# tpy001/VFMSeg

Measured on AMD Instinct MI355X. Metric: train images/sec @512x512 DINOv2-L+LoRA (dg_lora_dinov2_ms_masked, 1024^2 sample = LR+HR 512^2 passes), higher is better.
Workload: dtype bf16; 1 GPU; configs[1]: dg_lora_dinov2_ms_masked.py, synthetic 1024^2 19-class samples -> 2x512^2 passes, bs=2/GPU, full train step (fwd+bwd+allreduce+AdamW), LoRA dropout on; global_batch=2, parallelism=dp1

## Files before the change

include/vfmseg_hip.h:

```cpp
#ifndef VFMSEG_HIP_H
#define VFMSEG_HIP_H
#include <stdint.h>

#ifdef __cplusplus
extern "C" {
#endif

enum { VFM_F32 = 0, VFM_BF16 = 1, VFM_U8 = 2, VFM_I64 = 3,
       VFM_SPLIT3 = 4  };
enum { VFM_OK = 0, VFM_E_INVAL = -1, VFM_E_SHAPE = -2, VFM_E_ALIGN = -3, VFM_E_HIP = -4, VFM_E_UNSUPPORTED = -5 };
enum { VFM_EP_NONE = 0, VFM_EP_GELU = 1, VFM_EP_RELU = 2, VFM_EP_MUL_GELU_GRAD = 3, VFM_EP_MUL = 4,
       VFM_EP_QGELU = 5 , VFM_EP_MUL_QGELU_GRAD = 6,
       VFM_EP_GELU_DGELU = 7  };
enum { VFM_ACT_NONE = 0, VFM_ACT_GELU = 1, VFM_ACT_RELU = 2, VFM_ACT_QGELU = 3 };

const char* vfm_last_error(void);
int vfm_abi_version(void);
int vfm_half_kind(void);

int vfm_cast(const void* src, int src_dt, long ld_src, void* dst, int dst_dt, long ld_dst, long rows, long cols,
             const float* colscale, void* stream);
int vfm_split3(const float* src, long stride_r, long stride_c, void* dst, long ld_dst, long rows, long K, int pattern, void* stream);
int vfm_transpose(const void* src, int src_dt, long ld_src, void* dst, int dst_dt, long ld_dst, long rows, long cols,
                  long pad_rows, void* stream);
int vfm_strided_copy(const void* src, int src_dt, void* dst, int dst_dt, long n0, long n1, long n2, long n3, long s0,
                     long s1, long s2, long s3, long d0, long d1, long d2, long d3, int accumulate, void* stream);
typedef struct vfm_copy_job {
  const float* src; void* dst; long dst_dt; long accumulate;
  long n[4], s[4], d[4];
  long nsum, sum_stride;
} vfm_copy_job;
int vfm_strided_copy_batch(const vfm_copy_job* table_dev, int njobs, long max_elems, void* stream);
int vfm_axpby(const float* x, float a, float* y, float b, long n, void* stream);
int vfm_scale_by_device_scalar(float* y, const float* scalar, long n, void* stream);
int vfm_colsum(const void* x, int dt, long ld, long rows, long cols, float* out, int accumulate, float* ws, void* stream);
typedef struct vfm_lora_site {
  const float* A; const float* B;
  void* a; void* at; void* w; void* wt;
  long r, K, N, Kw, ld_a, ld_at, ld_w, ld_wt;
} vfm_lora_site;
int vfm_lora_pack(const vfm_lora_site* table_dev, int nsites, long max_elems, int dt, void* stream);
int vfm_slab_reduce(const float* slabs, int kch, long P, long Q, long rows_used, float alpha, float* dst, long sp, long sq,
                    int accumulate, void* stream);
int vfm_dropout_mask(void* out, int dt, long n, float p, uint64_t seed, uint64_t offset, void* stream);
int vfm_mul_mask(const void* src, int src_dt, long ld_src, const void* mask, int mask_dt, long mask_ld,
                 long rows_per_group, void* dst, int dst_dt, long ld_dst, long rows, long cols, void* stream);
int vfm_geglu_fwd(const void* h, int h_dt, long ld_h, void* out, int out_dt, long ld_out, long rows, long C, void* stream);
int vfm_geglu_bwd(const void* h, int h_dt, long ld_h, const void* dout, int do_dt, long ld_do, void* dh, int dh_dt,
                  long ld_dh, long rows, long C, void* stream);
int vfm_swiglu_fwd(const void* h, int h_dt, long ld_h, void* out, int out_dt, long ld_out, long rows, long C, void* stream);
int vfm_swiglu_bwd(const void* h, int h_dt, long ld_h, const void* dout, int do_dt, long ld_do, void* dh, int dh_dt,
                   long ld_dh, long rows, long C, void* stream);
int vfm_rope(void* x, int dt, long ld, long rows, int np, int ncols, int d, const float* cos_t, const float* sin_t,
             int inverse, void* stream);
int vfm_act_grad_mul(const void* dy, int dy_dt, long ld_dy, const void* pre, int pre_dt, long ld_pre, void* out, int out_dt,
                     long ld_out, long rows, long cols, int act, void* stream);
int vfm_mask_token_fwd(const float* x, const uint8_t* keep, const float* token, float* out, long rows, long C, void* stream);
int vfm_mask_token_bwd(const float* dout, const uint8_t* keep, float* dx, float* dtoken, float* ws ,
                       long rows, long C, void* stream);

int vfm_layernorm_fwd(const float* x, long ld_x, const float* w, const float* b, float eps, void* y, int y_dt, long ld_y,
                      float* stats, long rows, long C, void* stream);
int vfm_layernorm_fwd_split3(const float* x, long ld_x, const float* w, const float* b, float eps, float* y, long ld_y, void* y3, long ld3,
                             long plane, float* stats, long rows, long C, void* stream);
int vfm_layernorm_dropout_fwd(const float* x, long ld_x, const float* w, const float* b, float eps, void* y, long ld_y,
                              float* stats, void* y_drop, long ld_yd, void* mask, long ld_mask, float p, uint64_t seed,
                              uint64_t offset, long rows, long C, void* stream);
int vfm_layernorm_bwd_scaled(const void* dy, int dy_dt, long ld_dy, const float* x, long ld_x, const float* w,
                             const float* stats, float* dx, long ld_dx, int accumulate_dx, void* t_out, long ld_t,
                             const float* t_scale, long rows, long C, void* stream);
int vfm_layernorm_bwd(const void* dy, int dy_dt, long ld_dy, const float* x, long ld_x, const float* w,
                      const float* stats, float* dx, long ld_dx, int accumulate_dx, float* dw, float* db, float* ws,
                      long rows, long C, void* stream);
int vfm_groupnorm_fwd(const float* x, const float* w, const float* b, float eps, int G, int act, void* y, int y_dt,
                      float* stats, float* ws, long B, long P, long C, void* stream);
int vfm_groupnorm_bwd(const void* dy, int dy_dt, const float* x, const float* w, const float* b, const float* stats,
                      int G, int act, float* dx, float* dw, float* db, float* ws, long B, long P, long C, void* stream);
int vfm_groupnorm_tile_ok(long P, long C, int G);
int vfm_groupnorm_tile_fwd(const float* x, const float* w, const float* b, float eps, int G, int act, void* y, int y_dt,
                           float* stats, long B, long P, long C, void* stream);
int vfm_groupnorm_tile_bwd(const void* dy, int dy_dt, const float* x, const float* w, const float* b, const float* stats,
                           int G, int act, float* dx, float* dw, float* db, float* ws, long B, long P, long C, void* stream);
int vfm_bn_moments(const float* x, long rows, long C, float* sums, float* ws, void* stream);
int vfm_bn_finalize(const float* sums, float count, float* mean_var, float* running_mean, float* running_var,
                    float momentum, long C, void* stream);
int vfm_bn_apply(const float* x, const float* mean_var, const float* w, const float* b, float eps, int act, void* y,
                 int y_dt, long rows, long C, void* stream);
int vfm_bn_bwd_reduce(const void* dy, int dy_dt, const float* x, const float* mean_var, const float* w, const float* b,
                      float eps, int act, float* sums_dy, float* ws, long rows, long C, void* stream);
int vfm_bn_bwd_apply(const void* dy, int dy_dt, const float* x, const float* mean_var, const float* w, const float* b,
                     float eps, int act, const float* sums_dy, float total_rows, float* dx, long rows, long C,
                     void* stream);

typedef struct vfm_gemm_desc {
  const void* A; const void* B; void* C;
  int in_dt; int c_dt;
  long M, N, K;
  long sa_m, sa_k, sb_n, sb_k, ldc;
  float alpha;
  const float* bias; long bias_mod;
  const float* colscale;
  const void* residual; int r_dt; long ldr;
  int ep_mode; const void* aux; int aux_dt; long ld_aux;
  void* C2; int c2_dt; long ldc2;
  long batch, stride_a, stride_b, stride_c;
  long c_plane;
  long kb_rows;
} vfm_gemm_desc;
int vfm_gemm(const vfm_gemm_desc* d, void* stream);
int vfm_tune(const char* key, int value);

typedef struct vfm_attn_desc {
  const void* q; const void* k; const void* v; void* o;
  int dt; long ldq, ldk, ldv, ldo;
  int B, H, d;
  int nq_main, nq_extra, nk_main, nk_extra;
  float scale;
  float* lse;
  const void* dout; long ld_do;
  void* dq; void* dk; void* dv; long ld_dq, ld_dk, ld_dv;
  float* delta;
} vfm_attn_desc;
int vfm_attn_fwd(const vfm_attn_desc* d, void* stream);
int vfm_attn_bwd(const vfm_attn_desc* d, void* stream);
int vfm_attn_fwd_x3(const vfm_attn_desc* d, long lo_off, void* stream);
int vfm_attn_fwd_x3_split(const vfm_attn_desc* d, long lo_off, void* o3, long ld3, long plane, void* stream);
int vfm_attn_bwd_x3(const vfm_attn_desc* d, const void* q3, const void* k3, const void* v3, long ld3, long lo_off, const void* do3,
                    long ld_do3, long lo_off_do3, void* stream);

int vfm_sam_relpos_table(const float* rel_pos, int L, int d, int S, float* out, void* stream);
int vfm_sam_attn_prep(const void* qkv, int dt, long ld, const float* bias, const float* rh, const float* rw, void* q_aug,
                      void* k_aug, void* v_win, int nimg, int G, int S, int H, int d, int Dq, int NP,
                      int rows_per_batch , float scale, void* stream);
int vfm_softmax_rows(const float* scores, long ld_s, void* out, int out_dt, long ld_o, long rows, int n, int npad, void* stream);
int vfm_sam_attn_merge(const void* o_win, int dt, void* out, long ld, int nimg, int G, int S, int H, int d, int NP, void* stream);
int vfm_sam_attn_bwd_prep(const void* dao, long ld_dao, const void* qkv, long ld_qkv, const float* bias, int dt, void* dow,
                          void* dowT, void* vp, void* qsT, int nimg, int G, int S, int H, int d, int dp, int NP, float scale,
                          void* stream);
int vfm_softmax_rows_batched(const float* scores, long ld_s, void* out, int out_dt, long ld_o, long rows, int n, int npad,
                             int rows_per_batch, int valid_rows, void* stream);
int vfm_softmax_rows_bwd(const void* p, const float* dp, long ld_dp, void* ds, int dt, long ld_p, long rows, int n, int npad,
                         int rows_per_batch, int valid_rows, void* stream);
int vfm_sam_attn_bwd_merge(const void* dqa, const void* dkT, const void* dvT, int dt, const float* rh, const float* rw, void* dqkv,
                           long ld, int nimg, int G, int S, int H, int d, int dp, int NP, int Dq, float scale, void* stream);

int vfm_rein_mix_fwd(const float* x, long ld_x, const void* t, const void* vt, void* u, long ld_u, void* p, long ld_p, void* x16,
                     long ld_x16, long rows, int D, int m, float c, void* stream);
int vfm_rein_mix_bwd(const void* du, long ld_du, const void* p, long ld_p, const void* v, const void* tt, void* ds, long ld_ds,
                     float* dx, long ld_dx, long rows, int D, int m, float c, void* stream);

int vfm_sam_attn_flash_fwd(const void* qkv, long ld, const float* bias, const void* tbl_h, const void* tbl_w, void* out, long ldo,
                           int nimg, int G, int S, int H, int d, float scale, void* stream);
int vfm_sam_attn_flash_fwd_train(const void* qkv, long ld, const float* bias, const void* tbl_h, const void* tbl_w, void* out, long ldo,
                                 int nimg, int G, int S, int H, int d, float scale, float* lse, void* qext, void* stream);
long vfm_sam_attn_flash_stat_rows(int nimg, int G, int S, int H);
int vfm_sam_attn_flash_bwd(const void* qkv, long ld, const float* bias, const void* tbl_h, const void* tbl_w, const void* out,
                           const void* dout, long ldo, const float* lse, const void* qext, float* dsum, void* dqkv, long ldg,
                           int nimg, int G, int S, int H, int d, float scale, void* stream);

int vfm_patchify(const float* img, long stride_b, long stride_c, long stride_y, int y0, int x0, int h, int w, int P,
                 void* out, int out_dt, long ld_out, int B, void* stream);
int vfm_assemble_tokens(const float* patch_tok, const float* cls, const float* pos, float* x, int B, int np, int C,
                        void* stream);

int vfm_resize_bilinear(const void* in, int in_dt, int in_nchw, int B, int Hi, int Wi, int C, long in_ld_c, void* out,
                        int out_dt, int out_mode, long out_ld_c, int Hv, int Wv, int y0, int x0, int hc, int wc,
                        float scale_y, float scale_x, void* stream);
int vfm_resize_bicubic(const float* in, int Hi, int Wi, int C, float* out, int Ho, int Wo, double scale_y, double scale_x,
                       void* stream);
int vfm_label_resize(const int64_t* in, int B, int Hi, int Wi, int64_t* out, int Hv, int Wv, int y0, int x0, int hc,
                     int wc, void* stream);
int vfm_unblock(const float* x, float* y, int B, int H, int W, int C, int levels, int inverse, void* stream);
int vfm_upsample_ce(const float* logits_low, const int64_t* label, int B, int h, int w, int C, int H, int W,
                    int ignore_index, float* loss_parts, int32_t* counts, float* dlogits, void* stream);
int vfm_upsample_ce_w(const float* logits_low, const int64_t* label, const float* weight, int B, int h, int w, int C, int H, int W,
                      int ignore_index, float* loss_parts, int32_t* counts, float* dlogits, void* stream);
int vfm_pseudo_label(const float* logits_low, int B, int h, int w, int C, int H, int W, float thr, int64_t* pseudo_label,
                     float* pseudo_prob, int32_t* count, void* stream);
int vfm_class_presence(const int64_t* label, int B, long n, uint32_t* bits, void* stream);
int vfm_class_mix(const float* src_img, const float* tgt_img, const int64_t* src_label, const int64_t* pseudo_label,
                  const uint32_t* chosen, const int32_t* count, long total, int ignore_top, int ignore_bottom, int B, int H, int W,
                  float* mixed_img, int64_t* mixed_label, float* mix_weight, uint8_t* mask, void* stream);
#define VFM_OHEM_STATE_INTS 3080
#define VFM_OHEM_N 0
#define VFM_OHEM_NLT 1
#define VFM_OHEM_K 2
#define VFM_OHEM_T 6
#define VFM_LABEL_COUNT_INTS 33
int vfm_ohem_prob(const float* logits_low, const int64_t* label, int B, int h, int w, int C, int H, int W, int ignore_index,
                  float thresh, float* p, int32_t* state, void* stream);
int vfm_ohem_threshold(const float* p, long n_pix, long k_request, float thresh, int32_t* state, void* stream);
int vfm_label_weight(const int64_t* label, const float* p, const int32_t* state, const float* class_weight, const float* pix_weight,
                     int C, long n_pix, int ignore_index, int avg_non_ignore, float* weight, int32_t* counts, float* norm, void* stream);
int vfm_ce_finish(const float* loss_parts, long n, float scale, int32_t* counts, float eps, float* loss, float* acc, void* stream);
int vfm_hrda_fuse_fwd(const float* lr, const float* a, const float* hr, int B, int h, int w, int C, int ha, int wa, int hc, int wc,
                      int Y0, int X0, int my0, int my1, int mx0, int mx1, float* fused, float* att_out, float* lr_scaled_out,
                      void* stream);
int vfm_hrda_fuse_bwd(const float* d_fused, const float* lr, const float* a, const float* hr, const float* att, int B, int h, int w,
                      int C, int ha, int wa, int hc, int wc, int Y0, int X0, int my0, int my1, int mx0, int mx1, float* d_lr,
                      float* d_a, float* d_hr, float* d_att_ws, void* stream);
int vfm_reduce_sum(const float* x, long n, float scale, float* out, void* stream);

int vfm_preprocess_u8(const uint8_t* img, int H, int W, float* out, int Hp, int Wp, const float* mean3, const float* std3,
                      int bgr_to_rgb, float pad_val, void* stream);
typedef struct vfm_augment_plan {
  int resize_h, resize_w;
  int crop_y, crop_x, crop_h, crop_w;
  int flip;
  int wide;
  int brightness_on, contrast_on;
  int saturation_on, hue_on, hue_delta;
  double brightness_beta, contrast_alpha, saturation_alpha;
} vfm_augment_plan;
int vfm_augment_u8(const uint8_t* img, int Hs, int Ws, const vfm_augment_plan* plan, float* out, int Hp, int Wp, const float* mean3,
                   const float* std3, int bgr_to_rgb, float pad_val, void* stream);
int vfm_conf_gate(const float* logits, int B, int C, int H, int W, int y0, int x0, int hc, int wc, float thr,
                  int32_t* count, void* stream);
int vfm_slide_accumulate(const float* crop, int crop_nchw, int B, int h, int w, int C, float* preds, float* count,
                         int H, int W, int y0, int x0, int hc, int wc, void* stream);
typedef struct vfm_slide_win {
  const float* crop;
  int nchw, h, w;
  int y0, x0, hc, wc;
} vfm_slide_win;
int vfm_slide_gather(const vfm_slide_win* wins, int nwin, int B, int C, float* preds, int H, int W, void* stream);
int vfm_conf_gate_windows(const float* logits, int B, int C, int H, int W, const int* boxes, int nwin, float thr, int32_t* counts,
                          void* stream);
int vfm_slide_finalize(float* preds, const float* count, uint8_t* argmax, int B, int C, int H, int W, void* stream);

int vfm_confusion_hist(const uint8_t* pred, const void* label, int label_dt, long n, int num_classes, int ignore_index,
                       int64_t* hist, void* stream);
int vfm_postprocess_argmax(const float* logits, int C, long plane_stride, long row_stride, int Hm, int Wm, int y0, int x0,
                           int h, int w, int flip, uint8_t* pred, int oh, int ow, const void* label, int label_dt,
                           int num_classes, int ignore_index, int64_t* hist, void* stream);

int vfm_adamw(float* p, float* g, float* m, float* v, long n, const long* seg_start, const float* seg_lr_mult,
              const float* seg_wd, int n_seg, float lr, float beta1, float beta2, float eps, int step, float grad_scale,
              int zero_grad, int vec4, void* stream);
int vfm_adamw_guarded(float* p, float* g, float* m, float* v, long n, const long* seg_start, const float* seg_lr_mult,
                      const float* seg_wd, int n_seg, float lr, float beta1, float beta2, float eps, int step, float grad_scale,
                      int zero_grad, int vec4, const int* skip, const float* amp_state, void* stream);
int vfm_amp_update(const int* flag, float* amp_state, float growth, float backoff, int interval, int dynamic, void* stream);

enum { VFM_OP_GEMM = 0, VFM_OP_LN_FWD = 1, VFM_OP_LN_DROPOUT_FWD = 2, VFM_OP_LN_BWD_SCALED = 3, VFM_OP_ATTN_FWD = 4, VFM_OP_ATTN_BWD = 5,
       VFM_OP_CAST = 6, VFM_OP_STRIDED_COPY = 7 };
enum { VFM_PROF_NONE = 0, VFM_PROF_GEMM = 1, VFM_PROF_GEMM_TN = 2, VFM_PROF_ATTN_FWD = 3, VFM_PROF_ATTN_BWD = 4 };
typedef struct vfm_plan_op {
  int kind;
  int prof_kind;
  double flops;
  union {
    vfm_gemm_desc gemm;
    vfm_attn_desc attn;
    struct { const float* x; long ld_x; const float* w; const float* b; float eps; void* y; int y_dt; long ld_y; float* stats;
             long rows, C; } ln_fwd;
    struct { const float* x; long ld_x; const float* w; const float* b; float eps; void* y; long ld_y; float* stats; void* y_drop;
             long ld_yd; void* mask; long ld_mask; float p; uint64_t offset; long rows, C; } ln_drop;
    struct { const void* dy; int dy_dt; long ld_dy; const float* x; long ld_x; const float* w; const float* stats; float* dx;
             long ld_dx; int accumulate_dx; void* t_out; long ld_t; const float* t_scale; long rows, C; } ln_bwd;
    struct { const void* src; int src_dt; long ld_src; void* dst; int dst_dt; long ld_dst; long rows, cols; const float* colscale; } cast;
    struct { const void* src; int src_dt; void* dst; int dst_dt; long n[4]; long ss[4]; long ds[4]; int accumulate; } copy;
  } u;
} vfm_plan_op;
int vfm_run_plan(const vfm_plan_op* ops, int n, uint64_t seed, uint64_t rng_base, void* stream);
int vfm_prof_config(int every);
int vfm_prof_read(double* out, int cap);

#ifdef __cplusplus
}
#endif
#endif
```

vfmseg_amd/backbones.py:

```python
import math

import os

import torch
import torch.nn as nn

from .precision import is_half
from . import ops
from .precision import compute_dtype
from .registry import MODELS

R_PAD = 64

BACKWARD_EVENTS = {"heads_done": None, "block_done": None, "backbone_done": None}
_PENDING_BACKWARD = [0]


class _Lin(nn.Module):
    def __init__(self, i, o, bias=True):
        super().__init__()
        self.in_features, self.out_features = i, o
        self.weight = nn.Parameter(torch.empty(o, i))
        self.bias = nn.Parameter(torch.zeros(o)) if bias else None
        nn.init.trunc_normal_(self.weight, std=0.02)
# ... 169 lines not shown
        if ck is not None:
            if init_cfg.get("type", "Pretrained") != "Pretrained":
                raise NotImplementedError(f"init_cfg type {init_cfg.get('type')!r}: only dict(type='Pretrained', checkpoint=...) is read")
            self.load_pretrained_base(ck)

    def load_pretrained_base(self, checkpoint):
        sd = torch.load(checkpoint, map_location="cpu") if isinstance(checkpoint, (str, os.PathLike)) else checkpoint
        sd = sd.get("state_dict", sd) if isinstance(sd, dict) else sd
        missing, _ = self.load_state_dict(sd, strict=False)
        missing = [k for k in missing if not k.startswith("reins.")]
        if missing:
            raise RuntimeError(f"pretrained backbone {checkpoint if isinstance(checkpoint, (str, os.PathLike)) else '<state dict>'}: "
                               f"{len(missing)} base parameters not found (first: {missing[:3]}; the file holds e.g. {list(sd)[:3]})")
        self.pretrained = checkpoint if isinstance(checkpoint, (str, os.PathLike)) else "<state dict>"
        self.engine().invalidate()

    def train(self, mode=True):
        nn.Module.train(self, False)
        self._rein_train = bool(mode)
        if mode:
            for n, p in self.named_parameters():
                p.requires_grad = "reins" in n
            for p in self.reins.inert_params():
                p.requires_grad = False
            self.reins.train(True)
        return self

    def adapter_training(self):
        return self._rein_train

    def state_dict(self, *args, destination=None, prefix="", keep_vars=False):
        if args:
            args = list(args) + [None] * (3 - len(args))
            destination, prefix, keep_vars = args[0], args[1] or "", bool(args[2])
        state = super().state_dict(destination=destination, prefix=prefix, keep_vars=keep_vars)
        for k in [k for k in state.keys() if k.startswith(prefix) and "rein" not in k[len(prefix):]]:
            state.pop(k)
        return state

    def forward(self, x):
        xcat, (hp, wp) = self.forward_tokens([(x, None)], training=self._rein_train)
        b, d = x.shape[0], self.embed_dim
        v = xcat.view(b, hp, wp, len(self.out_indices), d)
        return tuple(v[:, :, :, i].permute(0, 3, 1, 2) for i in range(len(self.out_indices)))


class _Holder(nn.Module):
    def __init__(self, m):
        super().__init__()
        self.model = m


class _PeftModel(nn.Module):
    def __init__(self, m):
        super().__init__()
        self.base_model = _Holder(m)


@MODELS.register_module()
class LoRABackbone(nn.Module):

    def __init__(self, backbone, checkpoint=None, Lora_config=None, init_cfg=None, **kw):
        super().__init__()
        vit = MODELS.build(backbone)
        cfg = Lora_config or {}
        self.lora_targets = list(cfg.get("target_modules", ["qkv"]))
        for name, mod in list(vit.named_modules()):
            if isinstance(mod, _Lin) and any(name == t or name.endswith("." + t) for t in self.lora_targets):
                parent = vit
                parts = name.split(".")
                for p_ in parts[:-1]:
                    parent = getattr(parent, p_)
                setattr(parent, parts[-1], LoraLinear(mod, cfg.get("r", 32), cfg.get("lora_alpha", 32), cfg.get("lora_dropout", 0.0)))
        if not vit.engine().lora_on():
            raise NotImplementedError(f"target_modules={self.lora_targets}: no adapter site the {type(vit).__name__} HIP engine fuses")
        self.model = _PeftModel(vit)
        self._lora_train = False
        if checkpoint is not None:
            self.load_pretrained_backbone(checkpoint, self.lora_targets)
        self.train(True)

    @property
    def vit(self):
        return self.model.base_model.model

    def load_pretrained_backbone(self, checkpoint, target_modules):
        sd = torch.load(checkpoint, map_location="cpu") if isinstance(checkpoint, str) else checkpoint
        new = {}
        for name, w in sd.items():
            for t in target_modules:
                if t in name:
                    name = name.replace(t, t + ".base_layer")
            new[name] = w
        self.vit.load_state_dict(new, strict=False)
        self.vit.engine().invalidate()

    def train(self, mode=True):
        super().train(False)
        self._lora_train = bool(mode)
        for n, p in self.named_parameters():
            p.requires_grad = ("lora" in n) if mode else p.requires_grad
        if mode:
            for p in getattr(self.vit.engine(), "inert_params", lambda: [])():
                p.requires_grad = False
        return self

    def forward_tokens(self, jobs, seed=None):
        return self.vit.forward_tokens(jobs, training=self._lora_train, seed=seed)

    def forward(self, x):
        xcat, (hp, wp) = self.forward_tokens([(x, None)])
        b, d, nt = x.shape[0], self.vit.embed_dim, len(self.vit.out_indices)
        v = xcat.view(b, hp, wp, nt, d)
        return tuple(v[:, :, :, i].permute(0, 3, 1, 2) for i in range(nt))


class Packed:

    def __init__(self, w_f32, cd, k_pad=None):
        n, k = w_f32.shape
        k_pad = k_pad or k
        self.n, self.k = n, k_pad
        self.w = ops.empty_ld(n, k_pad, cd, w_f32.device, zero=True)
        ops.cast(w_f32, self.w[:, :k])
        self.wt = None
        if is_half(cd):
            self.wt = ops.empty_ld(k_pad, n, cd, w_f32.device, zero=True)
            ops.transpose(w_f32, self.wt[:k], pad_rows=n)

    def fwd(self, a, out, **epi):
        return ops.gemm(a, self.w, out, **epi)

    def dgrad(self, dy, out, **epi):
        if self.wt is not None:
            return ops.gemm(dy, self.wt, out, **epi)
        return ops.gemm(dy, self.w, out, trans_b=True, **epi)


def wgrad(dy, x, grad_out, alpha=1.0, n_rows=None, accumulate=True):
    M = dy.shape[0]
    res = grad_out if accumulate else None
    if is_half(dy.dtype):
        mp = (M + 63) // 64 * 64
        dyt = torch.empty(dy.shape[1], mp, dtype=dy.dtype, device=dy.device)
        xt = torch.empty(x.shape[1], mp, dtype=x.dtype, device=x.device)
        ops.transpose(dy, dyt, pad_rows=mp)
        ops.transpose(x, xt, pad_rows=mp)
        ops.gemm(dyt, xt, grad_out, alpha=alpha, residual=res)
    else:
        ops.gemm(dy, x, grad_out, alpha=alpha, residual=res, trans_a=True, trans_b=True)
    return grad_out


class _DinoTrainPlan:

    def __init__(self, eng, P, nimg, Np):
        v = eng.vit
        cd, dev = P["cd"], P["dev"]
        D, H = v.embed_dim, v.num_heads
        nL = len(v.blocks)
        M, Mp = nimg * Np + nimg, nimg * Np
        Lp0 = P["layers"][0]
        kq, hid = Lp0["qkv"].k, Lp0["fc1"].n
        q0 = v.blocks[0].attn.qkv
        self.eng, self.P, self.nimg, self.Np, self.M, self.Mp, self.nL, self.D, self.H = eng, P, nimg, Np, M, Mp, nL, D, H
        self.busy = False
        e = lambda *sh, dt=cd: torch.empty(*sh, dtype=dt, device=dev)
        f32 = torch.float32
        self.X = e(nL + 1, M, D, dt=f32)
        self.A1, self.XD, self.MASK = e(nL, M, kq), e(nL, M, D), e(nL, M, D)
        self.ST1, self.ST2 = e(nL, M, 2, dt=f32), e(nL, M, 2, dt=f32)
        self.QKV, self.AO = e(nL, M, 3 * D), e(nL, M, D)
        self.LSE = e(nL, nimg, H, Np + 1, dt=f32)
        self.XMID, self.A2 = e(nL, M, D, dt=f32), e(nL, M, D)
        hld = hid + ops.ld_pad(hid, cd)
        self.HPRE = e(nL, M, hld)[:, :, :hid]
        self.G = e(M, hld)[:, :hid]
        self.hid, self.kq = hid, kq
        hd = D // H
        scale = hd ** -0.5
        f = self.fwd = ops.Plan("backbone")
        self.tap_ops = []
        self.nt = len(v.out_indices)
        xcat0 = e(Mp, self.nt * D)
        for li, (blk, Lp) in enumerate(zip(v.blocks, P["layers"])):
            q = blk.attn.qkv
            x, a1 = self.X[li], self.A1[li]
            f.layernorm_dropout_fwd(x, Lp["n1w"], Lp["n1b"], 1e-6, a1[:, :D], self.ST1[li], self.XD[li], self.MASK[li], q.p, li * M * D)
            f.gemm(self.XD[li], Lp["a"], a1[:, D:D + R_PAD], alpha=q.scaling)
            f.gemm(a1, Lp["qkv"].w, self.QKV[li], bias=Lp["qkv_b"])
            qkv = self.QKV[li]
            f.attn_fwd(qkv[:, :D], qkv[:, D:2 * D], qkv[:, 2 * D:], self.AO[li], self.LSE[li], nimg, H, hd, Np, 1, Np, 1, scale)
            f.gemm(self.AO[li], Lp["proj"].w, self.XMID[li], bias=Lp["proj_b"], colscale=Lp["g1"], residual=x)
            f.layernorm_fwd(self.XMID[li], Lp["n2w"], Lp["n2b"], 1e-6, self.A2[li], self.ST2[li])
            f.gemm(self.A2[li], Lp["fc1"].w, self.G, bias=Lp["fc1_b"], ep_mode=ops.EP_GELU_DGELU, c2=self.HPRE[li])
            f.gemm(self.G, Lp["fc2"].w, self.X[li + 1], bias=Lp["fc2_b"], colscale=Lp["g2"], residual=self.XMID[li])
            for i, oi in enumerate(v.out_indices):
                if oi == li:
                    self.tap_ops.append((f.cast(self.X[li + 1][:Mp], xcat0[:, i * D:(i + 1) * D]), i * D))
        self.bwd = None

    def eligible_backward(self):
        from .functional import direct_grad_target
        v = self.eng.vit
        return (os.environ.get("VFMSEG_LORA_WGRAD_BATCHED", "1") != "0" and
                all(direct_grad_target(b.attn.qkv.lora_A["default"].weight) is not None and
                    direct_grad_target(b.attn.qkv.lora_B["default"].weight) is not None for b in v.blocks))

    def run_forward(self, xcat, seed, rng0):
        esz = xcat.element_size()
        for idx, col in self.tap_ops:
            self.fwd.entry(idx).u.cast.dst = xcat.data_ptr() + col * esz
        self.fwd.run(seed, rng0)

    def _build_backward(self, dxcat):
        v, P = self.eng.vit, self.P
        cd, dev = P["cd"], P["dev"]
        D, H, nL, M, Mp, nimg, Np = self.D, self.H, self.nL, self.M, self.Mp, self.nimg, self.Np
        hd = D // H
        scale = hd ** -0.5
        e = lambda *sh, dt=cd: torch.empty(*sh, dtype=dt, device=dev)
        self.DX = e(M, D, dt=torch.float32)
        self.T, self.DN, self.DAO = e(M, D), e(M, D), e(M, D)
        self.DH = e(M, self.hid + ops.ld_pad(self.hid, cd))[:, :self.hid]
        self.DQKV, self.DA1 = e(nL, M, 3 * D), e(nL, M, self.kq)
        half = nL // 2
        skip_l0 = os.environ.get("VFMSEG_PLAN_SKIP_L0", "1") != "0"
        self.half = half
        self.dx_sig = (tuple(dxcat.shape), tuple(dxcat.stride()), dxcat.dtype)
        plans, self.tap_src = [], []

        def add_tap(pl, pn, li):
            for i, oi in enumerate(v.out_indices):
                if oi == li:
                    src = dxcat[:, i * D:(i + 1) * D]
                    self.tap_src.append((pn, pl.strided_copy(src, self.DX, (Mp, D), (src.stride(0), 1), (D, 1), accumulate=True), i * D))

        for pn, (hi, lo) in enumerate(((nL, half), (half, 0)) if half > 0 else ((nL, 0),)):
            pl = ops.Plan("backbone")
            for li in range(hi - 1, lo - 1, -1):
                blk, Lp = v.blocks[li], P["layers"][li]
                q = blk.attn.qkv
                if li == nL - 1:
                    add_tap(pl, pn, li)
                    pl.cast(self.DX, self.T, Lp["g2"])
                pl.gemm(self.T, Lp["fc2"].wt, self.DH, ep_mode=ops.EP_MUL, aux=self.HPRE[li])
                pl.gemm(self.DH, Lp["fc1"].wt, self.DN)
                pl.layernorm_bwd_scaled(self.DN, self.XMID[li], Lp["n2w"], self.ST2[li], self.DX, self.T, Lp["g1"], accumulate_dx=True)
                pl.gemm(self.T, Lp["proj"].wt, self.DAO)
                qkv, dqkv, da1 = self.QKV[li], self.DQKV[li], self.DA1[li]
                pl.attn_bwd(qkv[:, :D], qkv[:, D:2 * D], qkv[:, 2 * D:], self.AO[li], self.LSE[li], self.DAO, dqkv[:, :D], dqkv[:, D:2 * D],
                            dqkv[:, 2 * D:], nimg, H, hd, Np, 1, Np, 1, scale)
                if li == 0 and skip_l0:
                    pl.gemm(dqkv, Lp["qkv"].wt[D:D + R_PAD], da1[:, D:D + R_PAD])
                    continue
                pl.gemm(dqkv, Lp["qkv"].wt, da1)
                pl.gemm(da1[:, D:D + R_PAD], Lp["at"], da1[:, :D], alpha=q.scaling, residual=da1[:, :D], ep_mode=ops.EP_MUL, aux=self.MASK[li])
                if li > 0:
                    add_tap(pl, pn, li - 1)
                    pl.layernorm_bwd_scaled(da1[:, :D], self.X[li], Lp["n1w"], self.ST1[li], self.DX, self.T, P["layers"][li - 1]["g2"],
                                            accumulate_dx=True)
                else:
                    pl.layernorm_bwd_scaled(da1[:, :D], self.X[li], Lp["n1w"], self.ST1[li], self.DX, self.T, Lp["g2"], accumulate_dx=True)
            plans.append((pl, lo, hi))
        self.bwd = plans

    def run_backward(self, ctx, dxcat):
        sig = (tuple(dxcat.shape), tuple(dxcat.stride()), dxcat.dtype)
        if self.bwd is None or self.dx_sig != sig:
            self._build_backward(dxcat)
        esz = dxcat.element_size()
        for pn, idx, col in self.tap_src:
            self.bwd[pn][0].entry(idx).u.copy.src = dxcat.data_ptr() + col * esz
        self.DX.zero_()
        for pl, lo, hi in self.bwd:
            pl.run()
            self.eng._lora_wgrads_batched(self.P, ctx, self.DA1, self.DQKV, lo, hi, self.M, self.D)
            if BACKWARD_EVENTS["block_done"] is not None:
                for lj in range(hi - 1, lo - 1, -1):
                    BACKWARD_EVENTS["block_done"](lj)


class DinoEngine:
    def __init__(self, vit):
        self.vit = vit
        self._packed = None
        self._pos_cache = {}

    def invalidate(self):
        self._packed = None
        self._pos_cache = {}

    def lora_on(self):
        return isinstance(self.vit.blocks[0].attn.qkv, LoraLinear)

    def rein_on(self):
        return getattr(self.vit, "reins", None) is not None

    def trainable(self):
        out = []
        if self.lora_on():
            for blk in self.vit.blocks:
                out += [blk.attn.qkv.lora_A["default"].weight, blk.attn.qkv.lora_B["default"].weight]
        if self.rein_on():
            out += self.vit.reins.live_params()
        return out

    def packed(self):
        cd = compute_dtype()
        dev = self.vit.pos_embed.device
        if self._packed is not None and self._packed["cd"] == cd and self._packed["dev"] == dev:
            return self._packed
        v = self.vit
        D = v.embed_dim
        P = dict(cd=cd, dev=dev, layers=[])
        with torch.no_grad():
            pw = v.patch_embed.proj.weight.detach().reshape(D, -1)
            P["pe"] = Packed(pw, cd)
            P["pe_b"] = v.patch_embed.proj.bias.detach().float().contiguous()
            P["cls"] = v.cls_token.detach().reshape(D).float().contiguous()
            for blk in v.blocks:
                qkv = blk.attn.qkv
                base = qkv.base_layer if isinstance(qkv, LoraLinear) else qkv
                kq = D + (R_PAD if isinstance(qkv, LoraLinear) else 0)
                Lp = dict(
                    qkv=Packed(base.weight.detach(), cd, k_pad=kq),
                    qkv_b=base.bias.detach().float().contiguous() if base.bias is not None else None,
                    proj=Packed(blk.attn.proj.weight.detach(), cd),
                    proj_b=blk.attn.proj.bias.detach().float().contiguous() if blk.attn.proj.bias is not None else None,
                    fc1=Packed(blk.mlp.fc1.weight.detach(), cd),
                    fc1_b=blk.mlp.fc1.bias.detach().float().contiguous() if blk.mlp.fc1.bias is not None else None,
                    fc2=Packed(blk.mlp.fc2.weight.detach(), cd),
                    fc2_b=blk.mlp.fc2.bias.detach().float().contiguous() if blk.mlp.fc2.bias is not None else None,
                    g1=blk.ls1.gamma.detach().float().contiguous(), g2=blk.ls2.gamma.detach().float().contiguous(),
                    n1w=blk.norm1.weight.detach().float().contiguous(), n1b=blk.norm1.bias.detach().float().contiguous(),
                    n2w=blk.norm2.weight.detach().float().contiguous(), n2b=blk.norm2.bias.detach().float().contiguous(),
                )
                if isinstance(qkv, LoraLinear):
                    Lp["a"] = torch.zeros(R_PAD, D, dtype=cd, device=dev)
                    Lp["at"] = torch.zeros(D, R_PAD, dtype=cd, device=dev)
                P["layers"].append(Lp)
        self._packed = P
        return P

    def refresh_lora(self, P):
        D = self.vit.embed_dim
        sites = []
        for blk, Lp in zip(self.vit.blocks, P["layers"]):
            q = blk.attn.qkv
            if isinstance(q, LoraLinear):
                A, Bm = q.lora_A["default"].weight.detach(), q.lora_B["default"].weight.detach()
                sites.append((A, Bm, Lp["a"], Lp["at"], Lp["qkv"].w, Lp["qkv"].wt, q.r, A.shape[1], Bm.shape[0], D))
        _refresh_sites(P, sites)

    def merged_qkv(self, P):
        from .optim import PARAM_EPOCH
        key = [PARAM_EPOCH[0]]
        for blk in self.vit.blocks:
            q = blk.attn.qkv
            A, Bm = q.lora_A["default"].weight, q.lora_B["default"].weight
            key += [A._version, Bm._version, A.data_ptr(), Bm.data_ptr()]
        key = tuple(key)
        if P.get("merged_key") == key:
            return P["merged"]
        D, cd, dev = self.vit.embed_dim, P["cd"], P["dev"]
        merged = []
        with torch.no_grad():
            for blk in self.vit.blocks:
                q = blk.attn.qkv
                A, Bm = q.lora_A["default"].weight.detach().float(), q.lora_B["default"].weight.detach().float()
                w = q.base_layer.weight.detach().float()
                weff = torch.empty_like(w)
                ops.gemm(Bm.contiguous(), A.contiguous(), weff, alpha=q.scaling, residual=w, trans_b=True)
                wp = ops.empty_ld(w.shape[0], D, cd, dev)
                ops.cast(weff, wp)
                merged.append(wp)
        P["merged"], P["merged_key"] = merged, key
        return merged

    def pos_tokens(self, hp, wp):
        v = self.vit
        n = v.pos_embed.shape[1] - 1
        s = int(math.sqrt(n))
        if hp == s and wp == s:
            return v.pos_embed.detach().reshape(n + 1, -1).float().contiguous()
        key = (hp, wp)
        if key not in self._pos_cache:
            D = v.embed_dim
            pe = v.pos_embed.detach().reshape(n + 1, D).float().contiguous()
            out = torch.empty(1 + hp * wp, D, dtype=torch.float32, device=pe.device)
            ops.cast(pe[:1], out[:1])
            sy, sx = s / (hp + 0.1), s / (wp + 0.1)
            assert int(s * ((hp + 0.1) / s)) == hp and int(s * ((wp + 0.1) / s)) == wp
            ops.resize_bicubic(pe[1:], s, s, D, out[1:], hp, wp, sy, sx)
            self._pos_cache[key] = out
        return self._pos_cache[key]

    def forward(self, jobs, training, seed, need_grad=False):
        v, P = self.vit, self.packed()
        cd = P["cd"]
        dev = P["dev"]
        D, H, ps = v.embed_dim, v.num_heads, v.patch_size
        lora = self.lora_on()
        rein = self._rein_pack(P) if self.rein_on() else None
        merged = None
        from .precision import split3 as _x3_mode
        x3 = _x3_mode() and not is_half(cd)
        if (lora and not training and not torch.is_grad_enabled() and (is_half(cd) or x3)
                and os.environ.get("VFMSEG_MERGE_LORA_EVAL", "1") != "0"):
            merged = self.merged_qkv(P)
        elif lora:
            self.refresh_lora(P)
        sizes = []
        for img, box in jobs:
            y0, y1, x0, x1 = box if box is not None else (0, img.shape[2], 0, img.shape[3])
            sizes.append(((y1 - y0) // ps, (x1 - x0) // ps))
        hp, wp = sizes[0]
        assert all(s == (hp, wp) for s in sizes), "all jobs of one backbone call must share the token grid"
        Np = hp * wp
        nimg = sum(j[0].shape[0] for j in jobs)
        Mp, M = nimg * Np, nimg * Np + nimg
        kpe = 3 * ps * ps
        A0 = torch.empty(Mp, kpe, dtype=cd, device=dev)
        r0 = 0
        for img, box in jobs:
            b = img.shape[0]
            ops.patchify(img, A0[r0 * Np:(r0 + b) * Np], box=box, patch=ps)
            r0 += b
        ptok = torch.empty(Mp, D, dtype=torch.float32, device=dev)
        P["pe"].fwd(A0, ptok, bias=P["pe_b"])
        plan = self._train_plan(P, nimg, Np, training, merged) if need_grad else None
        x = plan.X[0] if plan is not None else torch.empty(M, D, dtype=torch.float32, device=dev)
        ops.assemble_tokens(ptok, P["cls"], self.pos_tokens(hp, wp), x, nimg, Np, D)
        del ptok, A0
        nt = len(v.out_indices)
        from .precision import eval_heads_fp32
        tap_dt = torch.float32 if (not training and not need_grad and eval_heads_fp32()) else cd
        xcat = torch.empty(Mp, nt * D, dtype=tap_dt, device=dev)
        saved = []
        if lora and training:
            from .functional import draw_seed
            seed, rng0 = draw_seed(seed, len(v.blocks) * M * D)
        else:
            seed, rng0 = 0, 0
        if plan is not None:
            plan.run_forward(xcat, seed, rng0)
            plan.busy = True
            ctx = dict(saved=None, plan=plan, nimg=nimg, Np=Np, M=M, Mp=Mp, P=P, training=training, A1all=plan.A1, XDall=plan.XD)
            return xcat, (hp, wp), ctx
        nL = len(v.blocks)
        batched = lora and training and is_half(cd) and merged is None
        A1all = torch.empty(nL, M, P["layers"][0]["qkv"].k, dtype=cd, device=dev) if batched else None
        XDall = None
        hd = D // H
        scale = hd ** -0.5
        for li, (blk, Lp) in enumerate(zip(v.blocks, P["layers"])):
            S = {"x_in": x}
            kq = D if merged is not None else Lp["qkv"].k
            a1 = A1all[li] if batched else torch.empty(M, kq, dtype=cd, device=dev)
            st1 = torch.empty(M, 2, dtype=torch.float32, device=dev)
            q = blk.attn.qkv if lora else None
            fused_drop = lora and training and q.p > 0 and is_half(cd) and D % 256 == 0
            if fused_drop:
                mask = torch.empty(M, D, dtype=cd, device=dev)
                if batched and XDall is None:
                    XDall = torch.empty(nL, M, D, dtype=cd, device=dev)
                xd = XDall[li] if batched else torch.empty(M, D, dtype=cd, device=dev)
                ops.layernorm_dropout_fwd(x, Lp["n1w"], Lp["n1b"], 1e-6, a1[:, :D], st1, xd, mask, q.p, seed, offset=rng0 + li * M * D)
            else:
                so = "only" if (x3 and not training and not need_grad and kq == D) else None
                ops.layernorm_fwd(x, Lp["n1w"], Lp["n1b"], 1e-6, a1 if kq == D else a1[:, :D], st1, split_out=so)
            if lora and merged is None:
                if not fused_drop:
                    xd, mask = a1[:, :D], None
                    if training and q.p > 0:
                        mask = torch.empty(M, D, dtype=cd, device=dev)
                        ops.dropout_mask(mask, q.p, seed, offset=rng0 + li * M * D)
                        xd = torch.empty(M, D, dtype=cd, device=dev)
                        ops.mul_mask(a1[:, :D], mask, xd)
                ops.gemm(xd, Lp["a"], a1[:, D:D + R_PAD], alpha=q.scaling)
                S.update(xd=xd if mask is not None else None, mask=mask)
            qkv = torch.empty(M, 3 * D, dtype=cd, device=dev)
            if merged is not None:
                ops.gemm(a1, merged[li], qkv, bias=Lp["qkv_b"])
            else:
                Lp["qkv"].fwd(a1, qkv, bias=Lp["qkv_b"])
            ao = torch.empty(M, D, dtype=cd, device=dev)
            lse = torch.empty(nimg, H, Np + 1, dtype=torch.float32, device=dev)
            so = "only" if (x3 and not training and not need_grad) else None
            ops.attn_fwd(qkv[:, :D], qkv[:, D:2 * D], qkv[:, 2 * D:], ao, lse, nimg, H, hd, Np, 1, Np, 1, scale, keep_split=training, o_split=so)
            xm = torch.empty(M, D, dtype=torch.float32, device=dev)
            Lp["proj"].fwd(ao, xm, bias=Lp["proj_b"], colscale=Lp["g1"], residual=x)
            a2 = torch.empty(M, D, dtype=cd, device=dev)
            st2 = torch.empty(M, 2, dtype=torch.float32, device=dev)
            ops.layernorm_fwd(xm, Lp["n2w"], Lp["n2b"], 1e-6, a2, st2, split_out=so)
            hid = Lp["fc1"].n
            g = ops.empty_ld(M, hid, cd, dev)
            if training and (lora or (rein is not None and need_grad)):
                hpre = torch.empty(M, hid, dtype=cd, device=dev)
                Lp["fc1"].fwd(a2, g, bias=Lp["fc1_b"], ep_mode=ops.EP_GELU_DGELU, c2=hpre)
            else:
                hpre = None
                Lp["fc1"].fwd(a2, g, bias=Lp["fc1_b"], ep_mode=ops.EP_GELU, **({"c_split": so} if so else {}))
            xo = torch.empty(M, D, dtype=torch.float32, device=dev)
            Lp["fc2"].fwd(g, xo, bias=Lp["fc2_b"], colscale=Lp["g2"], residual=xm)
            S.update(a1=a1, st1=st1, qkv=qkv, ao=ao, lse=lse, x_mid=xm, a2=a2, st2=st2, hpre=hpre, g=g)
            saved.append(S)
            x = xo
            if rein is not None:
                x = self._rein_forward(rein, li, x, Mp, S if (training and need_grad) else None)
            for i, oi in enumerate(v.out_indices):
                if oi == li:
                    ops.cast(x[:Mp], xcat[:, i * D:(i + 1) * D])
        ctx = dict(saved=saved, nimg=nimg, Np=Np, M=M, Mp=Mp, P=P, training=training, A1all=A1all, XDall=XDall, rein=rein)
        return xcat, (hp, wp), ctx

    def _train_plan(self, P, nimg, Np, training, merged):
        v = self.vit
        if (not training or merged is not None or not self.lora_on() or self.rein_on() or not is_half(P["cd"])
                or os.environ.get("VFMSEG_PLAN", "1") == "0" or v.embed_dim % 256 != 0):
            return None
        q0 = v.blocks[0].attn.qkv
        if not all(isinstance(b.attn.qkv, LoraLinear) and b.attn.qkv.p > 0 and b.attn.qkv.p == q0.p and b.attn.qkv.scaling == q0.scaling
                   for b in v.blocks):
            return None
        plans = P.setdefault("plans", {})
        pl = plans.get((nimg, Np))
        if pl is None:
            pl = plans[(nimg, Np)] = _DinoTrainPlan(self, P, nimg, Np)
        if pl.busy or not pl.eligible_backward():
            return None
        return pl

    def backward(self, ctx, dxcat):
        if ctx.get("plan") is not None:
            plan = ctx["plan"]
            try:
                plan.run_backward(ctx, dxcat)
            finally:
                plan.busy = False
            return [None] * (2 * len(self.vit.blocks))
        v, P = self.vit, ctx["P"]
        cd, dev = P["cd"], P["dev"]
        D, H = v.embed_dim, v.num_heads
        hd = D // H
        scale = hd ** -0.5
        M, Mp, nimg, Np = ctx["M"], ctx["Mp"], ctx["nimg"], ctx["Np"]
        dx = torch.zeros(M, D, dtype=torch.float32, device=dev)
        grads = [None] * (2 * len(v.blocks) if self.lora_on() else 0)
        nL = len(v.blocks)
        rein = ctx.get("rein")
        rein_acc = self._rein_backward_begin(rein) if rein is not None else None
        from .functional import direct_grad_target
        wg_batched = (ctx.get("A1all") is not None and self.lora_on() and os.environ.get("VFMSEG_LORA_WGRAD_BATCHED", "1") != "0" and
                      all(direct_grad_target(b.attn.qkv.lora_A["default"].weight) is not None and
                          direct_grad_target(b.attn.qkv.lora_B["default"].weight) is not None for b in v.blocks) and
                      (ctx.get("XDall") is not None or all(S_["mask"] is None for S_ in ctx["saved"])))
        if wg_batched:
            kq_all = ctx["A1all"].shape[2]
            DA1all = torch.empty(nL, M, kq_all, dtype=cd, device=dev)
            DQKVall = torch.empty(nL, M, 3 * D, dtype=cd, device=dev)
        half = nL // 2
        fuse_t = is_half(cd) and D % 256 == 0
        fuse_t1 = fuse_t and rein is None
        def add_tap(li):
            for i, oi in enumerate(v.out_indices):
                if oi == li:
                    src = dxcat[:, i * D:(i + 1) * D]
                    ops.strided_copy(src, dx, (Mp, D), (src.stride(0), 1), (D, 1), accumulate=True)
        t = None
        for li in range(len(v.blocks) - 1, -1, -1):
            blk, Lp, S = v.blocks[li], P["layers"][li], ctx["saved"][li]
            q = blk.attn.qkv
            if t is None:
                add_tap(li)
                if rein is not None:
                    self._rein_backward(rein, rein_acc, li, dx, Mp, S)
                t = torch.empty(M, D, dtype=cd, device=dev)
                ops.cast(dx, t, Lp["g2"])
            hid = Lp["fc1"].n
            dh = ops.empty_ld(M, hid, cd, dev)
            Lp["fc2"].dgrad(t, dh, ep_mode=ops.EP_MUL, aux=S["hpre"])
            dn = torch.empty(M, D, dtype=cd, device=dev)
            Lp["fc1"].dgrad(dh, dn)
            if fuse_t:
                ops.layernorm_bwd_scaled(dn, S["x_mid"], Lp["n2w"], S["st2"], dx, t, Lp["g1"], accumulate_dx=True)
            else:
                ops.layernorm_bwd(dn, S["x_mid"], Lp["n2w"], S["st2"], dx, accumulate_dx=True)
                ops.cast(dx, t, Lp["g1"])
            del dh
            dao = torch.empty(M, D, dtype=cd, device=dev)
            Lp["proj"].dgrad(t, dao)
            dqkv = DQKVall[li] if wg_batched else torch.empty(M, 3 * D, dtype=cd, device=dev)
            qkv = S["qkv"]
            ops.attn_bwd(qkv[:, :D], qkv[:, D:2 * D], qkv[:, 2 * D:], S["ao"], S["lse"], dao, dqkv[:, :D], dqkv[:, D:2 * D],
                         dqkv[:, 2 * D:], nimg, H, hd, Np, 1, Np, 1, scale)
            kq = Lp["qkv"].k
            da1 = DA1all[li] if wg_batched else torch.empty(M, kq, dtype=cd, device=dev)
            Lp["qkv"].dgrad(dqkv, da1)
            if isinstance(q, LoraLinear) and wg_batched:
                ep = dict(ep_mode=ops.EP_MUL, aux=S["mask"]) if S["mask"] is not None else {}
                ops.gemm(da1[:, D:D + R_PAD], Lp["at"], da1[:, :D], alpha=q.scaling, residual=da1[:, :D], **ep)
            elif isinstance(q, LoraLinear):
                r = q.r
                A, Bm = q.lora_A["default"].weight, q.lora_B["default"].weight
                a1 = S["a1"]
                xd = S["xd"] if S["xd"] is not None else a1[:, :D]
                from .functional import direct_grad_target
                tB, tA = direct_grad_target(Bm), direct_grad_target(A)
                gBt = torch.empty(R_PAD, Bm.shape[0], dtype=torch.float32, device=dev)
                gAp = torch.empty(R_PAD, A.shape[1], dtype=torch.float32, device=dev)
                doneB = _wgrad_small_t(a1[:, D:D + R_PAD], dqkv, gBt, scatter=None if tB is None else (tB, r, 1, r))
                doneA = _wgrad_small_t(da1[:, D:D + R_PAD], xd, gAp, alpha=q.scaling,
                                       scatter=None if tA is None else (tA, r, A.shape[1], 1))
                if doneB is True:
                    pass
                elif tB is not None:
                    ops.strided_copy(gBt, tB, (Bm.shape[0], r), (1, gBt.stride(0)), (r, 1), accumulate=True)
                else:
                    gB = torch.empty_like(Bm, dtype=torch.float32)
                    ops.strided_copy(gBt, gB, (Bm.shape[0], r), (1, gBt.stride(0)), (r, 1))
                    grads[2 * li + 1] = gB
                if doneA is True:
                    pass
                elif tA is not None:
                    ops.axpby(gAp[:r].reshape(-1), 1.0, tA.view(-1), 1.0)
                else:
                    grads[2 * li] = gAp[:r]
                ep = dict(ep_mode=ops.EP_MUL, aux=S["mask"]) if S["mask"] is not None else {}
                ops.gemm(da1[:, D:D + R_PAD], Lp["at"], da1[:, :D], alpha=q.scaling, residual=da1[:, :D], **ep)
            if fuse_t1 and li > 0:
                add_tap(li - 1)
                ops.layernorm_bwd_scaled(da1[:, :D], S["x_in"], Lp["n1w"], S["st1"], dx, t, P["layers"][li - 1]["g2"],
                                         accumulate_dx=True)
            else:
                ops.layernorm_bwd(da1[:, :D], S["x_in"], Lp["n1w"], S["st1"], dx, accumulate_dx=True)
                t = None
            ctx["saved"][li] = None
            if wg_batched:
                if li == half or li == 0:
                    lo, hi = (half, nL) if li == half and half > 0 else (0, half if half > 0 else nL)
                    self._lora_wgrads_batched(P, ctx, DA1all, DQKVall, lo, hi, M, D)
                    if BACKWARD_EVENTS["block_done"] is not None:
                        for lj in range(hi - 1, lo - 1, -1):
                            BACKWARD_EVENTS["block_done"](lj)
            elif BACKWARD_EVENTS["block_done"] is not None:
                BACKWARD_EVENTS["block_done"](li)
        if rein is not None:
            grads += self._rein_backward_end(rein, rein_acc)
        return grads

    def _rein_fused(self, P):
        r = self.vit.reins
        return (is_half(P["cd"]) and os.environ.get("VFMSEG_REIN_FUSED", "0") == "1" and self.vit.embed_dim % 256 == 0
                and r.token_length <= ops.REIN_TOK)

    def _rein_pack(self, P):
        from .optim import PARAM_EPOCH
        r = self.vit.reins
        cd, dev = P["cd"], P["dev"]
        D, nL, m = self.vit.embed_dim, r.num_layers, r.token_length
        live = r.live_params()
        key = (PARAM_EPOCH[0], self._rein_fused(P)) + tuple(x for p_ in live for x in (p_._version, p_.data_ptr()))
        R = P.get("rein")
        if R is not None and R["key"] == key:
            return R
        TP = (max(m, ops.REIN_TOK) + 63) // 64 * 64
        if R is None or R["TP"] != TP:
            z = lambda *sh, dt=cd: torch.zeros(*sh, dtype=dt, device=dev)
            R = P["rein"] = dict(TP=TP, T32=z(nL, TP, D, dt=torch.float32), T=z(nL, TP, D), V=z(nL, TP, D), TT=None, VT=None,
                                 scalevec=torch.empty(D, dtype=torch.float32, device=dev))
        R["key"], R["m"], R["c"], R["fused"] = key, m, float(D) ** -0.5, self._rein_fused(P)
        with torch.no_grad():
            T32 = R["T32"]
            toks = [p_.detach() for p_ in r.token_params()]
            if len(toks) == 2:
                ops.gemm(toks[0], toks[1], T32[:, :m], trans_b=True)
            else:
                ops.strided_copy(toks[0], T32, (nL, m, D), (m * D, D, 1), (TP * D, D, 1))
            if cd != torch.float32:
                ops.cast(T32.view(nL * TP, D), R["T"].view(nL * TP, D))
            else:
                R["T"] = T32
            Wt, Wd = r.mlp_token2feat, r.mlp_delta_f
            R["wt"], R["wd"] = Packed(Wt.weight.detach(), cd), Packed(Wd.weight.detach(), cd)
            R["bt"], R["bd"] = Wt.bias.detach(), Wd.bias.detach()
            vtmp = torch.empty(nL * TP, D, dtype=torch.float32, device=dev)
            R["wt"].fwd(R["T"].view(nL * TP, D), vtmp, bias=R["bt"])
            vt3 = vtmp.view(nL, TP, D)
            ops.strided_copy(vt3[:, 1:m], R["V"][:, 1:m], (nL, m - 1, D), (TP * D, D, 1), (TP * D, D, 1))
            if R["fused"]:
                if R["TT"] is None:
                    R["TT"], R["VT"] = torch.zeros(nL, D, TP, dtype=cd, device=dev), torch.zeros(nL, D, TP, dtype=cd, device=dev)
                ops.strided_copy(T32, R["TT"], (nL, D, m), (TP * D, 1, D), (D * TP, TP, 1))
                ops.strided_copy(vt3[:, 1:m], R["VT"][:, :, 1:m], (nL, D, m - 1), (TP * D, 1, D), (D * TP, TP, 1))
            ops.strided_copy(r.scale.detach().reshape(1), R["scalevec"], (D,), (0,), (1,))
        return R

    def _rein_forward(self, R, li, x, Mp, S):
        cd, dev = R["T"].dtype, x.device
        D, m, TP = x.shape[1], R["m"], R["TP"]
        xp = x[:Mp]
        u = torch.empty(Mp, D, dtype=cd, device=dev)
        p = torch.empty(Mp, TP, dtype=cd, device=dev) if S is not None else None
        x16 = None
        if R["fused"]:
            x16 = torch.empty(Mp, D, dtype=cd, device=dev) if S is not None else None
            ops.rein_mix_fwd(xp, R["T"][li], R["VT"][li], u, m, R["c"], p=p, x16=x16)
        else:
            if cd != torch.float32:
                x16 = torch.empty(Mp, D, dtype=cd, device=dev)
                ops.cast(xp, x16)
            sc = torch.empty(Mp, TP, dtype=torch.float32, device=dev)
            ops.gemm(x16 if x16 is not None else xp, R["T"][li], sc, alpha=R["c"])
            if p is None:
                p = torch.empty(Mp, TP, dtype=cd, device=dev)
            ops.softmax_rows(sc, p, m)
            ops.gemm(p, R["V"][li], u, residual=xp, trans_b=True)
        if S is None:
            xn = x
        else:
            xn = torch.empty_like(x)
            ops.cast(x[Mp:], xn[Mp:])
            S.update(rein_u=u, rein_p=p, rein_x=x16 if x16 is not None else xp)
        R["wd"].fwd(u, xn[:Mp], bias=R["bd"], colscale=R["scalevec"], residual=xp)
        return xn

    def _rein_backward_begin(self, R):
        dev = R["T"].device
        nL, TP, D = R["T"].shape
        z = lambda *sh: torch.zeros(*sh, dtype=torch.float32, device=dev)
        return dict(dT=z(nL, TP, D), dV=z(nL, TP, D), Gm=z(D, D), gb=z(D))

    @staticmethod
    def _tn(xs, y, out, alpha=1.0, accumulate=False):
        if is_half(xs.dtype):
            ops.gemm_tn_batched(xs.unsqueeze(0), y.unsqueeze(0), out.unsqueeze(0), xs.shape[0], alpha=alpha, accumulate=accumulate)
        else:
            ops.gemm(xs, y, out, alpha=alpha, residual=out if accumulate else None, trans_a=True, trans_b=True)

    def _rein_backward(self, R, acc, li, dx, Mp, S):
        cd, dev = R["T"].dtype, dx.device
        D, m, TP, c = dx.shape[1], R["m"], R["TP"], R["c"]
        u, p, xs = S["rein_u"], S["rein_p"], S["rein_x"]
        g = torch.empty(Mp, D, dtype=cd, device=dev)
        ops.cast(dx[:Mp], g)
        self._tn(g, u, acc["Gm"], accumulate=True)
        ops.colsum(g, acc["gb"], accumulate=True)
        du = torch.empty(Mp, D, dtype=cd, device=dev)
        R["wd"].dgrad(g, du, colscale=R["scalevec"])
        ds = torch.empty(Mp, TP, dtype=cd, device=dev)
        if R["fused"]:
            ops.rein_mix_bwd(du, p, R["V"][li], R["TT"][li], ds, dx[:Mp], m, c)
            a = 1.0
        else:
            dp = torch.empty(Mp, TP, dtype=torch.float32, device=dev)
            ops.gemm(du, R["V"][li], dp)
            ops.softmax_rows_bwd(p, dp, ds, m, 1, 1)
            ops.gemm(ds, R["T"][li], dx[:Mp], alpha=c, residual=dx[:Mp], trans_b=True)
            ops.strided_copy(du, dx[:Mp], (Mp, D), (du.stride(0), 1), (dx.stride(0), 1), accumulate=True)
            a = c
        self._tn(ds, xs, acc["dT"][li], alpha=a)
        self._tn(p, du, acc["dV"][li])
        S["rein_u"] = S["rein_p"] = S["rein_x"] = None

    def _rein_backward_end(self, R, acc):
        from .functional import direct_grad_target
        r = self.vit.reins
        cd, dev = R["T"].dtype, R["T"].device
        nL, TP, D = R["T"].shape
        m = R["m"]
        z = lambda *sh, dt=torch.float32: torch.zeros(*sh, dtype=dt, device=dev)
        dvz = z(nL, TP, D, dt=cd)
        ops.strided_copy(acc["dV"][:, 1:m], dvz[:, 1:m], (nL, m - 1, D), (TP * D, D, 1), (TP * D, D, 1))
        dvz2, T2 = dvz.view(nL * TP, D), R["T"].view(nL * TP, D)
        gWt, gbt = z(D, D), z(D)
        self._tn(dvz2, T2, gWt)
        ops.colsum(dvz2, gbt)
        back = torch.empty(nL * TP, D, dtype=torch.float32, device=dev)
        R["wt"].dgrad(dvz2, back)
        dT = acc["dT"]
        ops.strided_copy(back.view(nL, TP, D)[:, 1:m], dT[:, 1:m], (nL, m - 1, D), (TP * D, D, 1), (TP * D, D, 1), accumulate=True)
        toks = r.token_params()
# ... 169 lines not shown
```

vfmseg_amd/csrc/elementwise.hip:

```cpp
#include "common.h"

thread_local char g_vfm_err[512] = {0};

extern "C" const char* vfm_last_error(void) { return g_vfm_err; }
extern "C" int vfm_abi_version(void) { return 9; }
extern "C" int vfm_half_kind(void) { return VFM_HALF_KIND; }

template <typename TI, typename TO>
__global__ void k_cast(const TI* __restrict__ src, long ld_src, TO* __restrict__ dst, long ld_dst, long rows, long cols,
                       const float* __restrict__ colscale) {
  const long cols4 = cols >> 2;
  const long total = rows * cols4;
  for (long i = blockIdx.x * (long)blockDim.x + threadIdx.x; i < total; i += (long)gridDim.x * blockDim.x) {
    const long r = i / cols4, c = (i - r * cols4) << 2;
    float v[4];
#pragma unroll
    for (int j = 0; j < 4; ++j) v[j] = ld_f32(src + r * ld_src + c + j);
    if (colscale) {
#pragma unroll
      for (int j = 0; j < 4; ++j) v[j] *= colscale[c + j];
    }
#pragma unroll
    for (int j = 0; j < 4; ++j) st_f32(dst + r * ld_dst + c + j, v[j]);
  }
  const long tail0 = cols4 << 2;
  const long ntail = cols - tail0;
  if (ntail) {
    for (long i = blockIdx.x * (long)blockDim.x + threadIdx.x; i < rows * ntail; i += (long)gridDim.x * blockDim.x) {
      const long r = i / ntail, c = tail0 + (i - r * ntail);
      float v = ld_f32(src + r * ld_src + c);
      if (colscale) v *= colscale[c];
      st_f32(dst + r * ld_dst + c, v);
    }
  }
}

extern "C" int vfm_cast(const void* src, int src_dt, long ld_src, void* dst, int dst_dt, long ld_dst, long rows, long cols,
                        const float* colscale, void* stream) {
  VFM_CHECK(rows >= 0 && cols >= 0 && ld_src >= cols && ld_dst >= cols, VFM_E_SHAPE, "vfm_cast: bad shape");
  if (rows == 0 || cols == 0) return VFM_OK;
  hipStream_t s = (hipStream_t)stream;
  const long total = rows * ((cols + 3) / 4);
  const int grid = (int)((total + 255) / 256 > 4096 ? 4096 : (total + 255) / 256);
#define L(TI, TO) hipLaunchKernelGGL((k_cast<TI, TO>), dim3(grid), dim3(256), 0, s, (const TI*)src, ld_src, (TO*)dst, ld_dst, rows, cols, colscale)
  if (src_dt == VFM_F32 && dst_dt == VFM_F32) L(float, float);
  else if (src_dt == VFM_F32 && dst_dt == VFM_BF16) L(float, bf16_t);
  else if (src_dt == VFM_BF16 && dst_dt == VFM_F32) L(bf16_t, float);
  else if (src_dt == VFM_BF16 && dst_dt == VFM_BF16) L(bf16_t, bf16_t);
  else VFM_FAIL(VFM_E_INVAL, "vfm_cast: dtype");
#undef L
  VFM_LAUNCH_CHECK();
  return VFM_OK;
}

__global__ void k_split3(const float* __restrict__ src, long sr, long sc, bf16_t* __restrict__ dst, long ld_dst, long rows, long K, long Kp,
                         int pattern) {
  const long per_row = Kp / 4;
  const long total = rows * per_row;
  for (long i = (long)blockIdx.x * blockDim.x + threadIdx.x; i < total; i += (long)gridDim.x * blockDim.x) {
    const long r = i / per_row, c = (i % per_row) * 4;
    float v[4];
    if (sc == 1 && c + 3 < K && ((reinterpret_cast<uintptr_t>(src + r * sr + c) & 15) == 0)) {
      const float4 f = *reinterpret_cast<const float4*>(src + r * sr + c);
      v[0] = f.x, v[1] = f.y, v[2] = f.z, v[3] = f.w;
    } else {
#pragma unroll
      for (int e = 0; e < 4; ++e) v[e] = (c + e < K) ? src[r * sr + (c + e) * sc] : 0.f;
    }
    ushort4 hi, lo;
    bf16_t* ph = &hi.x;
    bf16_t* pl = &lo.x;
#pragma unroll
    for (int e = 0; e < 4; ++e) {
      ph[e] = f32_to_bf16(v[e]);
      pl[e] = f32_to_bf16(v[e] - bf16_to_f32(ph[e]));
    }
    bf16_t* d = dst + r * ld_dst + c;
    *reinterpret_cast<ushort4*>(d) = hi;
    *reinterpret_cast<ushort4*>(d + Kp) = pattern == 0 ? hi : lo;
    *reinterpret_cast<ushort4*>(d + 2 * Kp) = pattern == 0 ? lo : hi;
  }
}

extern "C" int vfm_split3(const float* src, long stride_r, long stride_c, void* dst, long ld_dst, long rows, long K, int pattern, void* stream) {
  const long Kp = (K + 63) / 64 * 64;
  VFM_CHECK(rows >= 0 && K > 0 && ld_dst >= 3 * Kp && ld_dst % 4 == 0 && ((uintptr_t)dst % 8) == 0 && (pattern == 0 || pattern == 1), VFM_E_SHAPE,
            "vfm_split3: dst must hold rows x 3 ceil64(K) bf16 (ld %% 4 == 0, 8-byte aligned)");
  if (rows == 0) return VFM_OK;
  const long total = rows * (Kp / 4);
  const int grid = (int)((total + 255) / 256 > 8192 ? 8192 : (total + 255) / 256);
  hipLaunchKernelGGL(k_split3, dim3(grid), dim3(256), 0, (hipStream_t)stream, src, stride_r, stride_c, (bf16_t*)dst, ld_dst, rows, K, Kp, pattern);
  VFM_LAUNCH_CHECK();
  return VFM_OK;
}

template <typename TI, typename TO>
__global__ void k_transpose(const TI* __restrict__ src, long ld_src, TO* __restrict__ dst, long ld_dst, long rows, long cols,
                            long pad_rows) {
  __shared__ float tile[64][65];
  const long r0 = (long)blockIdx.y * 64, c0 = (long)blockIdx.x * 64;
  const int tx = threadIdx.x & 63, ty = threadIdx.x >> 6;
  for (int i = ty; i < 64; i += 4) {
    const long r = r0 + i, c = c0 + tx;
    tile[i][tx] = (r < rows && c < cols) ? ld_f32(src + r * ld_src + c) : 0.f;
  }
  __syncthreads();
  for (int i = ty; i < 64; i += 4) {
    const long c = c0 + i, r = r0 + tx;
    if (c < cols && r < pad_rows) st_f32(dst + c * ld_dst + r, tile[tx][i]);
  }
}

extern "C" int vfm_transpose(const void* src, int src_dt, long ld_src, void* dst, int dst_dt, long ld_dst, long rows, long cols,
                             long pad_rows, void* stream) {
  VFM_CHECK(pad_rows >= rows && ld_dst >= pad_rows && ld_src >= cols, VFM_E_SHAPE, "vfm_transpose: bad shape");
  if (cols == 0 || pad_rows == 0) return VFM_OK;
  hipStream_t s = (hipStream_t)stream;
  dim3 grid(cdiv(cols, 64), cdiv(pad_rows, 64));
#define L(TI, TO) hipLaunchKernelGGL((k_transpose<TI, TO>), grid, dim3(256), 0, s, (const TI*)src, ld_src, (TO*)dst, ld_dst, rows, cols, pad_rows)
  if (src_dt == VFM_F32 && dst_dt == VFM_F32) L(float, float);
  else if (src_dt == VFM_F32 && dst_dt == VFM_BF16) L(float, bf16_t);
  else if (src_dt == VFM_BF16 && dst_dt == VFM_F32) L(bf16_t, float);
  else if (src_dt == VFM_BF16 && dst_dt == VFM_BF16) L(bf16_t, bf16_t);
  else VFM_FAIL(VFM_E_INVAL, "vfm_transpose: dtype");
#undef L
  VFM_LAUNCH_CHECK();
  return VFM_OK;
}

template <typename TI, typename TO>
__global__ void k_strided_copy(const TI* __restrict__ src, TO* __restrict__ dst, long n0, long n1, long n2, long n3, long s0,
                               long s1, long s2, long s3, long d0, long d1, long d2, long d3, int accumulate) {
  const long total = n0 * n1 * n2 * n3;
  for (long i = blockIdx.x * (long)blockDim.x + threadIdx.x; i < total; i += (long)gridDim.x * blockDim.x) {
    long t = i;
    const long i3 = t % n3; t /= n3;
    const long i2 = t % n2; t /= n2;
    const long i1 = t % n1; t /= n1;
    const float v = ld_f32(src + t * s0 + i1 * s1 + i2 * s2 + i3 * s3);
    TO* q = dst + t * d0 + i1 * d1 + i2 * d2 + i3 * d3;
    st_f32(q, accumulate ? ld_f32(q) + v : v);
  }
}

extern "C" int vfm_strided_copy(const void* src, int src_dt, void* dst, int dst_dt, long n0, long n1, long n2, long n3,
                                long s0, long s1, long s2, long s3, long d0, long d1, long d2, long d3, int accumulate,
                                void* stream) {
  const long total = n0 * n1 * n2 * n3;
  if (total == 0) return VFM_OK;
  hipStream_t s = (hipStream_t)stream;
  const int grid = (int)((total + 255) / 256 > 4096 ? 4096 : (total + 255) / 256);
#define L(TI, TO) hipLaunchKernelGGL((k_strided_copy<TI, TO>), dim3(grid), dim3(256), 0, s, (const TI*)src, (TO*)dst, n0, n1, n2, n3, s0, s1, s2, s3, d0, d1, d2, d3, accumulate)
  if (src_dt == VFM_F32 && dst_dt == VFM_F32) L(float, float);
  else if (src_dt == VFM_F32 && dst_dt == VFM_BF16) L(float, bf16_t);
  else if (src_dt == VFM_BF16 && dst_dt == VFM_F32) L(bf16_t, float);
  else if (src_dt == VFM_BF16 && dst_dt == VFM_BF16) L(bf16_t, bf16_t);
  else VFM_FAIL(VFM_E_INVAL, "vfm_strided_copy: dtype");
#undef L
// ... 674 lines not shown
```

vfmseg_amd/csrc/norm.hip:

```cpp
#include "common.h"

__device__ __forceinline__ float act_f(float v, int act) {
  return act == VFM_ACT_GELU ? gelu_f(v) : (act == VFM_ACT_RELU ? fmaxf(v, 0.f) : v);
}
__device__ __forceinline__ float act_grad_f(float v, int act) {
  return act == VFM_ACT_GELU ? gelu_grad_f(v) : (act == VFM_ACT_RELU ? (v > 0.f ? 1.f : 0.f) : 1.f);
}

template <typename TO, int MAXPL>
__global__ void k_ln_fwd(const float* __restrict__ x, long ld_x, const float* __restrict__ w, const float* __restrict__ b,
                         float eps, TO* __restrict__ y, long ld_y, float* __restrict__ stats, long rows, int C) {
  const int lane = threadIdx.x & 63;
  const long row = (long)blockIdx.x * (blockDim.x >> 6) + (threadIdx.x >> 6);
  if (row >= rows) return;
  const float* xr = x + row * ld_x;
  float v[MAXPL];
  float s = 0.f;
#pragma unroll
  for (int i = 0; i < MAXPL; ++i) {
    const int c = i * 64 + lane;
    v[i] = c < C ? xr[c] : 0.f;
    s += v[i];
  }
  const float mean = wave_sum(s) / C;
  float q = 0.f;
#pragma unroll
  for (int i = 0; i < MAXPL; ++i) {
    const int c = i * 64 + lane;
    const float d = c < C ? v[i] - mean : 0.f;
    q += d * d;
  }
  const float rstd = rsqrtf(wave_sum(q) / C + eps);
  if (stats && lane == 0) {
    stats[row * 2] = mean;
    stats[row * 2 + 1] = rstd;
  }
#pragma unroll
  for (int i = 0; i < MAXPL; ++i) {
    const int c = i * 64 + lane;
    if (c < C) st_f32(y + row * ld_y + c, (v[i] - mean) * rstd * w[c] + b[c]);
  }
}


struct LnDrop {
  void* yd; long ld_yd; void* mask; long ld_mask; float p, keep_scale; uint64_t seed, offset;
};
struct Split3Out {
  bf16_t* y3; long ld3; long plane;
};
__device__ __forceinline__ void store_split4(const Split3Out& so, long row, int c0, float4 o) {
  const bf16_t h0 = f32_to_bf16(o.x), h1 = f32_to_bf16(o.y), h2 = f32_to_bf16(o.z), h3 = f32_to_bf16(o.w);
  const ushort4 hi = {h0, h1, h2, h3};
  const ushort4 lo = {f32_to_bf16(o.x - bf16_to_f32(h0)), f32_to_bf16(o.y - bf16_to_f32(h1)), f32_to_bf16(o.z - bf16_to_f32(h2)),
                      f32_to_bf16(o.w - bf16_to_f32(h3))};
  bf16_t* p = so.y3 + row * so.ld3 + c0;
  *reinterpret_cast<ushort4*>(p) = hi;
  *reinterpret_cast<ushort4*>(p + so.plane) = hi;
  *reinterpret_cast<ushort4*>(p + 2 * so.plane) = lo;
}
template <typename TO, int NV, bool DROP = false, bool SPLIT = false>
__global__ void k_ln_fwd_v4(const float* __restrict__ x, long ld_x, const float* __restrict__ w, const float* __restrict__ b,
                            float eps, TO* __restrict__ y, long ld_y, float* __restrict__ stats, long rows, int C, LnDrop dr = LnDrop(),
                            Split3Out so = Split3Out()) {
  const int lane = threadIdx.x & 63;
  const long row = (long)blockIdx.x * (blockDim.x >> 6) + (threadIdx.x >> 6);
  if (row >= rows) return;
  const float* xr = x + row * ld_x;
  float4 v[NV];
  float s = 0.f;
#pragma unroll
  for (int i = 0; i < NV; ++i) {
    v[i] = *reinterpret_cast<const float4*>(xr + (i * 64 + lane) * 4);
    s += (v[i].x + v[i].y) + (v[i].z + v[i].w);
  }
  const float mean = wave_sum(s) / C;
  float q = 0.f;
#pragma unroll
  for (int i = 0; i < NV; ++i) {
    const float a = v[i].x - mean, bb = v[i].y - mean, c = v[i].z - mean, d = v[i].w - mean;
    q += (a * a + bb * bb) + (c * c + d * d);
  }
  const float rstd = rsqrtf(wave_sum(q) / C + eps);
  if (stats && lane == 0) {
    stats[row * 2] = mean;
    stats[row * 2 + 1] = rstd;
  }
#pragma unroll
  for (int i = 0; i < NV; ++i) {
    const int c0 = (i * 64 + lane) * 4;
    const float4 ww = *reinterpret_cast<const float4*>(w + c0);
    const float4 bv = *reinterpret_cast<const float4*>(b + c0);
    float4 o;
    o.x = (v[i].x - mean) * rstd * ww.x + bv.x;
    o.y = (v[i].y - mean) * rstd * ww.y + bv.y;
    o.z = (v[i].z - mean) * rstd * ww.z + bv.z;
    o.w = (v[i].w - mean) * rstd * ww.w + bv.w;
    if constexpr (sizeof(TO) == 2) {
      ushort4 p = {f32_to_bf16(o.x), f32_to_bf16(o.y), f32_to_bf16(o.z), f32_to_bf16(o.w)};
      *reinterpret_cast<ushort4*>(y + row * ld_y + c0) = p;
      if constexpr (DROP) {
        const uint64_t e0 = dr.offset + (uint64_t)row * C + c0;
        const bf16_t ks = f32_to_bf16(dr.keep_scale);
        const float ksf = bf16_to_f32(ks);
        ushort4 mk, yd;
        const bool k0 = (hash_u32(dr.seed, e0) >> 8) * (1.0f / 16777216.0f) >= dr.p;
        const bool k1 = (hash_u32(dr.seed, e0 + 1) >> 8) * (1.0f / 16777216.0f) >= dr.p;
        const bool k2 = (hash_u32(dr.seed, e0 + 2) >> 8) * (1.0f / 16777216.0f) >= dr.p;
        const bool k3 = (hash_u32(dr.seed, e0 + 3) >> 8) * (1.0f / 16777216.0f) >= dr.p;
        mk.x = k0 ? ks : 0, mk.y = k1 ? ks : 0, mk.z = k2 ? ks : 0, mk.w = k3 ? ks : 0;
        yd.x = k0 ? f32_to_bf16(bf16_to_f32(p.x) * ksf) : f32_to_bf16(bf16_to_f32(p.x) * 0.f);
        yd.y = k1 ? f32_to_bf16(bf16_to_f32(p.y) * ksf) : f32_to_bf16(bf16_to_f32(p.y) * 0.f);
        yd.z = k2 ? f32_to_bf16(bf16_to_f32(p.z) * ksf) : f32_to_bf16(bf16_to_f32(p.z) * 0.f);
        yd.w = k3 ? f32_to_bf16(bf16_to_f32(p.w) * ksf) : f32_to_bf16(bf16_to_f32(p.w) * 0.f);
        *reinterpret_cast<ushort4*>((bf16_t*)dr.mask + row * dr.ld_mask + c0) = mk;
        *reinterpret_cast<ushort4*>((bf16_t*)dr.yd + row * dr.ld_yd + c0) = yd;
      }
    } else {
      if (!SPLIT || y != nullptr) *reinterpret_cast<float4*>(y + row * ld_y + c0) = o;
      if constexpr (SPLIT) store_split4(so, row, c0, o);
    }
  }
}

template <typename TD, int NV>
__global__ void k_ln_bwd_v4(const TD* __restrict__ dy, long ld_dy, const float* __restrict__ x, long ld_x,
                            const float* __restrict__ w, const float* __restrict__ stats, float* __restrict__ dx, long ld_dx,
                            int accumulate_dx, long rows, int C, bf16_t* __restrict__ t_out = nullptr, long ld_t = 0,
                            const float* __restrict__ t_scale = nullptr) {
  const int lane = threadIdx.x & 63;
  const long row = (long)blockIdx.x * (blockDim.x >> 6) + (threadIdx.x >> 6);
  if (row >= rows) return;
  const float mean = stats[row * 2], rstd = stats[row * 2 + 1];
  float4 g[NV], xh[NV];
  float s1 = 0.f, s2 = 0.f;
#pragma unroll
  for (int i = 0; i < NV; ++i) {
    const int c0 = (i * 64 + lane) * 4;
    float4 d;
    if constexpr (sizeof(TD) == 2) {
      const ushort4 p = *reinterpret_cast<const ushort4*>(dy + row * ld_dy + c0);
      d = make_float4(bf16_to_f32(p.x), bf16_to_f32(p.y), bf16_to_f32(p.z), bf16_to_f32(p.w));
    } else {
      d = *reinterpret_cast<const float4*>(dy + row * ld_dy + c0);
    }
    const float4 xv = *reinterpret_cast<const float4*>(x + row * ld_x + c0);
    const float4 ww = *reinterpret_cast<const float4*>(w + c0);
    xh[i] = make_float4((xv.x - mean) * rstd, (xv.y - mean) * rstd, (xv.z - mean) * rstd, (xv.w - mean) * rstd);
    g[i] = make_float4(d.x * ww.x, d.y * ww.y, d.z * ww.z, d.w * ww.w);
    s1 += (g[i].x + g[i].y) + (g[i].z + g[i].w);
    s2 += (g[i].x * xh[i].x + g[i].y * xh[i].y) + (g[i].z * xh[i].z + g[i].w * xh[i].w);
  }
  s1 = wave_sum(s1) / C;
  s2 = wave_sum(s2) / C;
#pragma unroll
  for (int i = 0; i < NV; ++i) {
    const int c0 = (i * 64 + lane) * 4;
    float4 o = make_float4(rstd * (g[i].x - s1 - xh[i].x * s2), rstd * (g[i].y - s1 - xh[i].y * s2),
                           rstd * (g[i].z - s1 - xh[i].z * s2), rstd * (g[i].w - s1 - xh[i].w * s2));
    float4* p = reinterpret_cast<float4*>(dx + row * ld_dx + c0);
    if (accumulate_dx) {
      const float4 old = *p;
      o.x += old.x, o.y += old.y, o.z += old.z, o.w += old.w;
    }
    *p = o;
    if (t_out) {
      const float4 ts = *reinterpret_cast<const float4*>(t_scale + c0);
      const ushort4 tv = {f32_to_bf16(o.x * ts.x), f32_to_bf16(o.y * ts.y), f32_to_bf16(o.z * ts.z), f32_to_bf16(o.w * ts.w)};
      *reinterpret_cast<ushort4*>(t_out + row * ld_t + c0) = tv;
    }
  }
}

template <typename TO, int MAXP2>
__global__ void k_ln_fwd_v2(const float* __restrict__ x, long ld_x, const float* __restrict__ w, const float* __restrict__ b, float eps,
                            TO* __restrict__ y, long ld_y, float* __restrict__ stats, long rows, int C) {
  const int lane = threadIdx.x & 63;
  const long row = (long)blockIdx.x * (blockDim.x >> 6) + (threadIdx.x >> 6);
  if (row >= rows) return;
  const float* xr = x + row * ld_x;
  float2 v[MAXP2];
  float s = 0.f;
#pragma unroll
  for (int i = 0; i < MAXP2; ++i) {
    const int c = (i * 64 + lane) * 2;
    v[i] = c < C ? *reinterpret_cast<const float2*>(xr + c) : make_float2(0.f, 0.f);
    s += v[i].x + v[i].y;
  }
  const float mean = wave_sum(s) / C;
  float q = 0.f;
#pragma unroll
  for (int i = 0; i < MAXP2; ++i) {
    const int c = (i * 64 + lane) * 2;
    if (c < C) {
      const float a = v[i].x - mean, bb = v[i].y - mean;
      q += a * a + bb * bb;
    }
  }
  const float rstd = rsqrtf(wave_sum(q) / C + eps);
  if (stats && lane == 0) {
    stats[row * 2] = mean;
    stats[row * 2 + 1] = rstd;
  }
#pragma unroll
  for (int i = 0; i < MAXP2; ++i) {
    const int c = (i * 64 + lane) * 2;
    if (c < C) {
      const float2 ww = *reinterpret_cast<const float2*>(w + c), bv = *reinterpret_cast<const float2*>(b + c);
      const float o0 = (v[i].x - mean) * rstd * ww.x + bv.x, o1 = (v[i].y - mean) * rstd * ww.y + bv.y;
      if constexpr (sizeof(TO) == 2) {
        const ushort2 pk = {f32_to_bf16(o0), f32_to_bf16(o1)};
        *reinterpret_cast<ushort2*>(y + row * ld_y + c) = pk;
      } else {
        *reinterpret_cast<float2*>(y + row * ld_y + c) = make_float2(o0, o1);
      }
    }
  }
}

template <typename TO, int MAXP4>
__global__ void k_ln_fwd_v4t(const float* __restrict__ x, long ld_x, const float* __restrict__ w, const float* __restrict__ b, float eps,
                             TO* __restrict__ y, long ld_y, float* __restrict__ stats, long rows, int C) {
  const int lane = threadIdx.x & 63;
  const long row = (long)blockIdx.x * (blockDim.x >> 6) + (threadIdx.x >> 6);
  if (row >= rows) return;
  const float* xr = x + row * ld_x;
  float v[MAXP4][4];
  float s = 0.f;
#pragma unroll
  for (int i = 0; i < MAXP4; ++i) {
    const int c = (i * 64 + lane) * 4;
    const float4 t = c < C ? *reinterpret_cast<const float4*>(xr + c) : make_float4(0.f, 0.f, 0.f, 0.f);
    v[i][0] = t.x, v[i][1] = t.y, v[i][2] = t.z, v[i][3] = t.w;
#pragma unroll
    for (int e = 0; e < 4; ++e)
      if (c + e < C) s += v[i][e];
  }
  const float mean = wave_sum(s) / C;
  float q = 0.f;
#pragma unroll
  for (int i = 0; i < MAXP4; ++i) {
    const int c = (i * 64 + lane) * 4;
#pragma unroll
    for (int e = 0; e < 4; ++e)
      if (c + e < C) q += (v[i][e] - mean) * (v[i][e] - mean);
  }
  const float rstd = rsqrtf(wave_sum(q) / C + eps);
  if (stats && lane == 0) {
    stats[row * 2] = mean;
    stats[row * 2 + 1] = rstd;
  }
#pragma unroll
  for (int i = 0; i < MAXP4; ++i) {
    const int c = (i * 64 + lane) * 4;
    if (c < C) {
      if (c + 4 <= C) {
        const float4 ww = *reinterpret_cast<const float4*>(w + c), bv = *reinterpret_cast<const float4*>(b + c);
        const float o0 = (v[i][0] - mean) * rstd * ww.x + bv.x, o1 = (v[i][1] - mean) * rstd * ww.y + bv.y;
        const float o2 = (v[i][2] - mean) * rstd * ww.z + bv.z, o3 = (v[i][3] - mean) * rstd * ww.w + bv.w;
        if constexpr (sizeof(TO) == 2) {
          const ushort4 pk = {f32_to_bf16(o0), f32_to_bf16(o1), f32_to_bf16(o2), f32_to_bf16(o3)};
          *reinterpret_cast<ushort4*>(y + row * ld_y + c) = pk;
        } else {
          *reinterpret_cast<float4*>(y + row * ld_y + c) = make_float4(o0, o1, o2, o3);
        }
      } else {
#pragma unroll
        for (int e = 0; e < 4; ++e)
          if (c + e < C) {
            const float o = (v[i][e] - mean) * rstd * w[c + e] + b[c + e];
            if constexpr (sizeof(TO) == 2) y[row * ld_y + c + e] = f32_to_bf16(o);
            else y[row * ld_y + c + e] = o;
          }
      }
    }
  }
}

extern "C" int vfm_layernorm_fwd_split3(const float* x, long ld_x, const float* w, const float* b, float eps, float* y, long ld_y, void* y3,
                                        long ld3, long plane, float* stats, long rows, long C, void* stream) {
  const int nv = (int)(C / 256);
  VFM_CHECK(C > 0 && C % 256 == 0 && (nv == 1 || nv == 2 || nv == 4 || nv == 5 || nv == 8) && ld_x >= C && ld_x % 4 == 0 && (uintptr_t)x % 16 == 0 &&
                (uintptr_t)w % 16 == 0 && (uintptr_t)b % 16 == 0,
            VFM_E_SHAPE, "vfm_layernorm_fwd_split3: C=%ld must be 256, 512, 1024, 1280 or 2048 with 16-byte aligned rows", C);
  VFM_CHECK(y3 && (uintptr_t)y3 % 8 == 0 && plane >= C && plane % 4 == 0 && ld3 >= 3 * plane && ld3 % 4 == 0 && (!y || (ld_y >= C && ld_y % 4 == 0 && (uintptr_t)y % 16 == 0)),
            VFM_E_ALIGN, "vfm_layernorm_fwd_split3: y3 [rows, >= 3 plane] bf16 with plane >= C, 8-byte aligned; y (optional fp32 copy) 16-byte aligned");
  if (rows == 0) return VFM_OK;
  hipStream_t s = (hipStream_t)stream;
  dim3 grid(cdiv(rows, 4)), blk(256);
  Split3Out so;
  so.y3 = (bf16_t*)y3, so.ld3 = ld3, so.plane = plane;
#define LVS(NV) hipLaunchKernelGGL((k_ln_fwd_v4<float, NV, false, true>), grid, blk, 0, s, x, ld_x, w, b, eps, y, ld_y, stats, rows, (int)C, LnDrop(), so)
  if (nv == 1) LVS(1); else if (nv == 2) LVS(2); else if (nv == 4) LVS(4); else if (nv == 5) LVS(5); else LVS(8);
#undef LVS
  VFM_LAUNCH_CHECK();
  return VFM_OK;
}

extern "C" int vfm_layernorm_fwd(const float* x, long ld_x, const float* w, const float* b, float eps, void* y, int y_dt,
                                 long ld_y, float* stats, long rows, long C, void* stream) {
  VFM_CHECK(C > 0 && C <= 3072 && ld_x >= C && ld_y >= C, VFM_E_SHAPE, "vfm_layernorm_fwd: C=%ld unsupported", C);
  if (rows == 0) return VFM_OK;
  hipStream_t s = (hipStream_t)stream;
  dim3 grid(cdiv(rows, 4)), blk(256);
  const int nvq = (int)(C / 256);
  const bool v4 = (C % 256 == 0) && (nvq == 1 || nvq == 2 || nvq == 4 || nvq == 5 || nvq == 8) && (ld_x % 4 == 0) && (ld_y % 4 == 0) && ((uintptr_t)x % 16 == 0) &&
                  ((uintptr_t)y % 8 == 0) && ((uintptr_t)w % 16 == 0) && ((uintptr_t)b % 16 == 0);
  if (v4) {
#define LV(TO, NV) hipLaunchKernelGGL((k_ln_fwd_v4<TO, NV>), grid, blk, 0, s, x, ld_x, w, b, eps, (TO*)y, ld_y, stats, rows, (int)C)
    const int nv = (int)(C / 256);
    if (y_dt == VFM_BF16) { if (nv == 1) LV(bf16_t, 1); else if (nv == 4) LV(bf16_t, 4); else if (nv == 5) LV(bf16_t, 5); else if (nv == 2) LV(bf16_t, 2); else LV(bf16_t, 8); }
    else if (y_dt == VFM_F32) { if (nv == 1) LV(float, 1); else if (nv == 4) LV(float, 4); else if (nv == 5) LV(float, 5); else if (nv == 2) LV(float, 2); else LV(float, 8); }
    else VFM_FAIL(VFM_E_INVAL, "vfm_layernorm_fwd: dtype");
#undef LV
    if (!(nv == 1 || nv == 2 || nv == 4 || nv == 5 || nv == 8)) VFM_FAIL(VFM_E_SHAPE, "vfm_layernorm_fwd: C=%ld", C);
    VFM_LAUNCH_CHECK();
    return VFM_OK;
  }
  if (C > 1024 && C <= 2816 && ld_x % 4 == 0 && ld_y % 4 == 0 && ld_x >= (C + 3) / 4 * 4 && ld_y >= (C + 3) / 4 * 4 && (uintptr_t)x % 16 == 0 &&
      (uintptr_t)y % 16 == 0 && (uintptr_t)w % 16 == 0 && (uintptr_t)b % 16 == 0) {
    if (y_dt == VFM_BF16) hipLaunchKernelGGL((k_ln_fwd_v4t<bf16_t, 11>), grid, blk, 0, s, x, ld_x, w, b, eps, (bf16_t*)y, ld_y, stats, rows, (int)C);
    else if (y_dt == VFM_F32) hipLaunchKernelGGL((k_ln_fwd_v4t<float, 11>), grid, blk, 0, s, x, ld_x, w, b, eps, (float*)y, ld_y, stats, rows, (int)C);
    else VFM_FAIL(VFM_E_INVAL, "vfm_layernorm_fwd: dtype");
    VFM_LAUNCH_CHECK();
    return VFM_OK;
  }
  if (C > 1024 && C % 2 == 0 && ld_x % 2 == 0 && ld_y % 2 == 0 && (uintptr_t)x % 8 == 0 && (uintptr_t)y % 8 == 0 && (uintptr_t)w % 8 == 0 &&
      (uintptr_t)b % 8 == 0) {
    if (y_dt == VFM_BF16) hipLaunchKernelGGL((k_ln_fwd_v2<bf16_t, 24>), grid, blk, 0, s, x, ld_x, w, b, eps, (bf16_t*)y, ld_y, stats, rows, (int)C);
    else if (y_dt == VFM_F32) hipLaunchKernelGGL((k_ln_fwd_v2<float, 24>), grid, blk, 0, s, x, ld_x, w, b, eps, (float*)y, ld_y, stats, rows, (int)C);
    else VFM_FAIL(VFM_E_INVAL, "vfm_layernorm_fwd: dtype");
    VFM_LAUNCH_CHECK();
    return VFM_OK;
  }
#define L(TO, PL) hipLaunchKernelGGL((k_ln_fwd<TO, PL>), grid, blk, 0, s, x, ld_x, w, b, eps, (TO*)y, ld_y, stats, rows, (int)C)
  const int pl = (int)((C + 63) / 64);
  if (y_dt == VFM_BF16) { if (pl <= 4) L(bf16_t, 4); else if (pl <= 16) L(bf16_t, 16); else if (pl <= 32) L(bf16_t, 32); else L(bf16_t, 48); }
  else if (y_dt == VFM_F32) { if (pl <= 4) L(float, 4); else if (pl <= 16) L(float, 16); else if (pl <= 32) L(float, 32); else L(float, 48); }
  else VFM_FAIL(VFM_E_INVAL, "vfm_layernorm_fwd: dtype");
#undef L
  VFM_LAUNCH_CHECK();
  return VFM_OK;
}

extern "C" int vfm_layernorm_dropout_fwd(const float* x, long ld_x, const float* w, const float* b, float eps, void* y, long ld_y,
                                         float* stats, void* y_drop, long ld_yd, void* mask, long ld_mask, float p, uint64_t seed,
                                         uint64_t offset, long rows, long C, void* stream) {
  VFM_CHECK(p >= 0.f && p < 1.f, VFM_E_INVAL, "vfm_layernorm_dropout_fwd: p");
  const long nv = C / 256;
  VFM_CHECK(C % 256 == 0 && (nv == 1 || nv == 2 || nv == 4 || nv == 5 || nv == 8), VFM_E_SHAPE, "vfm_layernorm_dropout_fwd: C=%ld", C);
  VFM_CHECK(ld_x % 4 == 0 && ld_y % 4 == 0 && ld_yd % 4 == 0 && ld_mask % 4 == 0 && (uintptr_t)x % 16 == 0 && (uintptr_t)y % 8 == 0 &&
                (uintptr_t)y_drop % 8 == 0 && (uintptr_t)mask % 8 == 0 && (uintptr_t)w % 16 == 0 && (uintptr_t)b % 16 == 0,
            VFM_E_ALIGN, "vfm_layernorm_dropout_fwd: alignment");
  if (rows == 0) return VFM_OK;
  hipStream_t s = (hipStream_t)stream;
  dim3 blk(256), grid(cdiv(rows, 4));
  LnDrop dr{y_drop, ld_yd, mask, ld_mask, p, 1.0f / (1.0f - p), seed, offset};
#define LVD(NV) hipLaunchKernelGGL((k_ln_fwd_v4<bf16_t, NV, true>), grid, blk, 0, s, x, ld_x, w, b, eps, (bf16_t*)y, ld_y, stats, rows, (int)C, dr)
  if (nv == 1) LVD(1); else if (nv == 2) LVD(2); else if (nv == 4) LVD(4); else if (nv == 5) LVD(5); else LVD(8);
#undef LVD
  VFM_LAUNCH_CHECK();
  return VFM_OK;
}

template <typename TD, int MAXPL, bool NEED_W>
__global__ void k_ln_bwd(const TD* __restrict__ dy, long ld_dy, const float* __restrict__ x, long ld_x,
                         const float* __restrict__ w, const float* __restrict__ stats, float* __restrict__ dx, long ld_dx,
                         int accumulate_dx, float* __restrict__ ws, long rows, int C) {
  const int lane = threadIdx.x & 63, wv = threadIdx.x >> 6, nw = blockDim.x >> 6;
  float pdw[NEED_W ? MAXPL : 1], pdb[NEED_W ? MAXPL : 1];
#pragma unroll
  for (int i = 0; i < (NEED_W ? MAXPL : 1); ++i) pdw[i] = pdb[i] = 0.f;
  for (long row = (long)blockIdx.x * nw + wv; row < rows; row += (long)gridDim.x * nw) {
    const float mean = stats[row * 2], rstd = stats[row * 2 + 1];
    float g[MAXPL], xh[MAXPL];
    float s1 = 0.f, s2 = 0.f;
#pragma unroll
    for (int i = 0; i < MAXPL; ++i) {
      const int c = i * 64 + lane;
      if (c < C) {
        const float d = ld_f32(dy + row * ld_dy + c);
        xh[i] = (x[row * ld_x + c] - mean) * rstd;
        g[i] = d * w[c];
        s1 += g[i];
        s2 += g[i] * xh[i];
        if constexpr (NEED_W) {
          pdw[i] += d * xh[i];
          pdb[i] += d;
        }
      } else {
        g[i] = xh[i] = 0.f;
      }
    }
    s1 = wave_sum(s1) / C;
    s2 = wave_sum(s2) / C;
#pragma unroll
    for (int i = 0; i < MAXPL; ++i) {
      const int c = i * 64 + lane;
      if (c < C) {
        const float v = rstd * (g[i] - s1 - xh[i] * s2);
        float* p = dx + row * ld_dx + c;
        *p = accumulate_dx ? *p + v : v;
      }
    }
  }
  if constexpr (NEED_W) {
    extern __shared__ float sh[];
#pragma unroll
    for (int i = 0; i < MAXPL; ++i) {
      const int c = i * 64 + lane;
      if (c < C) {
        sh[(wv * 2 + 0) * C + c] = pdw[i];
        sh[(wv * 2 + 1) * C + c] = pdb[i];
      }
    }
    __syncthreads();
    for (int c = threadIdx.x; c < 2 * C; c += blockDim.x) {
      const int which = c / C, cc = c - which * C;
      float a = 0.f;
      for (int k = 0; k < nw; ++k) a += sh[(k * 2 + which) * C + cc];
      ws[((long)blockIdx.x * 2 + which) * C + cc] = a;
    }
  }
}
__global__ void k_ln_bwd_fin(const float* __restrict__ ws, int parts, int C, float* __restrict__ dw, float* __restrict__ db) {
  __shared__ float sh[2][4][64];
  const int tx = threadIdx.x & 63, ty = threadIdx.x >> 6;
  const int c = blockIdx.x * 64 + tx;
  float a = 0.f, b = 0.f;
  if (c < C) {
#pragma unroll 8
    for (int p = ty; p < parts; p += 4) {
      a += ws[((long)p * 2 + 0) * C + c];
      b += ws[((long)p * 2 + 1) * C + c];
    }
  }
  sh[0][ty][tx] = a, sh[1][ty][tx] = b;
  __syncthreads();
  if (ty == 0 && c < C) {
    if (dw) dw[c] += (sh[0][0][tx] + sh[0][1][tx]) + (sh[0][2][tx] + sh[0][3][tx]);
    if (db) db[c] += (sh[1][0][tx] + sh[1][1][tx]) + (sh[1][2][tx] + sh[1][3][tx]);
  }
}

template <typename TD, int MAXP4>
__global__ void k_ln_bwd_v4t(const TD* __restrict__ dy, long ld_dy, const float* __restrict__ x, long ld_x, const float* __restrict__ w,
                             const float* __restrict__ stats, float* __restrict__ dx, long ld_dx, int accumulate_dx, long rows, int C) {
  const int lane = threadIdx.x & 63;
  const long row = (long)blockIdx.x * (blockDim.x >> 6) + (threadIdx.x >> 6);
  if (row >= rows) return;
  const float mean = stats[row * 2], rstd = stats[row * 2 + 1];
  float g[MAXP4][4], xh[MAXP4][4];
  float s1 = 0.f, s2 = 0.f;
#pragma unroll
  for (int i = 0; i < MAXP4; ++i) {
    const int c = (i * 64 + lane) * 4;
#pragma unroll
    for (int e = 0; e < 4; ++e) g[i][e] = xh[i][e] = 0.f;
    if (c < C) {
      float d[4];
      if constexpr (sizeof(TD) == 2) {
        const ushort4 pp = *reinterpret_cast<const ushort4*>(dy + row * ld_dy + c);
        d[0] = bf16_to_f32(pp.x), d[1] = bf16_to_f32(pp.y), d[2] = bf16_to_f32(pp.z), d[3] = bf16_to_f32(pp.w);
      } else {
        const float4 t = *reinterpret_cast<const float4*>(dy + row * ld_dy + c);
        d[0] = t.x, d[1] = t.y, d[2] = t.z, d[3] = t.w;
      }
      const float4 xv4 = *reinterpret_cast<const float4*>(x + row * ld_x + c);
      const float xv[4] = {xv4.x, xv4.y, xv4.z, xv4.w};
      float wv[4] = {0.f, 0.f, 0.f, 0.f};
      if (c + 4 <= C) {
        const float4 ww = *reinterpret_cast<const float4*>(w + c);
        wv[0] = ww.x, wv[1] = ww.y, wv[2] = ww.z, wv[3] = ww.w;
      } else {
#pragma unroll
        for (int e = 0; e < 4; ++e)
          if (c + e < C) wv[e] = w[c + e];
      }
#pragma unroll
      for (int e = 0; e < 4; ++e)
        if (c + e < C) {
          xh[i][e] = (xv[e] - mean) * rstd;
          g[i][e] = d[e] * wv[e];
          s1 += g[i][e];
          s2 += g[i][e] * xh[i][e];
        }
    }
  }
  s1 = wave_sum(s1) / C;
  s2 = wave_sum(s2) / C;
#pragma unroll
  for (int i = 0; i < MAXP4; ++i) {
    const int c = (i * 64 + lane) * 4;
    if (c < C) {
      float o[4];
#pragma unroll
      for (int e = 0; e < 4; ++e) o[e] = rstd * (g[i][e] - s1 - xh[i][e] * s2);
      if (c + 4 <= C) {
        float4* pp = reinterpret_cast<float4*>(dx + row * ld_dx + c);
        if (accumulate_dx) {
          const float4 old = *pp;
          o[0] += old.x, o[1] += old.y, o[2] += old.z, o[3] += old.w;
        }
        *pp = make_float4(o[0], o[1], o[2], o[3]);
      } else {
#pragma unroll
        for (int e = 0; e < 4; ++e)
          if (c + e < C) dx[row * ld_dx + c + e] = accumulate_dx ? dx[row * ld_dx + c + e] + o[e] : o[e];
      }
    }
  }
// ... 615 lines not shown
```

vfmseg_amd/csrc/plan.hip:

```cpp
#include <vector>

#include "common.h"

namespace {
struct ProfRec {
  int kind;
  double flops;
  hipEvent_t e0, e1;
};
int g_prof_every = 0;
long g_prof_count = 0;
std::vector<ProfRec> g_prof_recs;
std::vector<hipEvent_t> g_prof_pool;

hipEvent_t prof_event() {
  if (!g_prof_pool.empty()) {
    hipEvent_t e = g_prof_pool.back();
    g_prof_pool.pop_back();
    return e;
  }
  hipEvent_t e = nullptr;
  if (hipEventCreate(&e) != hipSuccess) return nullptr;
  return e;
}

int run_one(const vfm_plan_op& o, uint64_t seed, uint64_t rng_base, void* s) {
  switch (o.kind) {
    case VFM_OP_GEMM: return vfm_gemm(&o.u.gemm, s);
    case VFM_OP_ATTN_FWD: return vfm_attn_fwd(&o.u.attn, s);
    case VFM_OP_ATTN_BWD: return vfm_attn_bwd(&o.u.attn, s);
    case VFM_OP_LN_FWD: {
      const auto& a = o.u.ln_fwd;
      return vfm_layernorm_fwd(a.x, a.ld_x, a.w, a.b, a.eps, a.y, a.y_dt, a.ld_y, a.stats, a.rows, a.C, s);
    }
    case VFM_OP_LN_DROPOUT_FWD: {
      const auto& a = o.u.ln_drop;
      return vfm_layernorm_dropout_fwd(a.x, a.ld_x, a.w, a.b, a.eps, a.y, a.ld_y, a.stats, a.y_drop, a.ld_yd, a.mask, a.ld_mask, a.p, seed,
                                       rng_base + a.offset, a.rows, a.C, s);
    }
    case VFM_OP_LN_BWD_SCALED: {
      const auto& a = o.u.ln_bwd;
      return vfm_layernorm_bwd_scaled(a.dy, a.dy_dt, a.ld_dy, a.x, a.ld_x, a.w, a.stats, a.dx, a.ld_dx, a.accumulate_dx, a.t_out, a.ld_t,
                                      a.t_scale, a.rows, a.C, s);
    }
    case VFM_OP_CAST: {
      const auto& a = o.u.cast;
      return vfm_cast(a.src, a.src_dt, a.ld_src, a.dst, a.dst_dt, a.ld_dst, a.rows, a.cols, a.colscale, s);
    }
    case VFM_OP_STRIDED_COPY: {
      const auto& a = o.u.copy;
      return vfm_strided_copy(a.src, a.src_dt, a.dst, a.dst_dt, a.n[0], a.n[1], a.n[2], a.n[3], a.ss[0], a.ss[1], a.ss[2], a.ss[3], a.ds[0],
                              a.ds[1], a.ds[2], a.ds[3], a.accumulate, s);
    }
    default: VFM_FAIL(VFM_E_INVAL, "vfm_run_plan: unknown op kind %d", o.kind);
  }
}
}

extern "C" int vfm_run_plan(const vfm_plan_op* ops, int n, uint64_t seed, uint64_t rng_base, void* stream) {
  VFM_CHECK(ops != nullptr || n == 0, VFM_E_INVAL, "vfm_run_plan: null plan");
  hipStream_t hs = (hipStream_t)stream;
  for (int i = 0; i < n; ++i) {
    const vfm_plan_op& o = ops[i];
    bool timed = false;
    ProfRec rec;
    if (g_prof_every > 0 && o.prof_kind != VFM_PROF_NONE && (++g_prof_count % g_prof_every) == 0 && g_prof_recs.size() < 65536) {
      rec.kind = o.prof_kind, rec.flops = o.flops, rec.e0 = prof_event(), rec.e1 = prof_event();
      timed = rec.e0 && rec.e1 && hipEventRecord(rec.e0, hs) == hipSuccess;
    }
    const int rc = run_one(o, seed, rng_base, stream);
    if (timed) {
      if (hipEventRecord(rec.e1, hs) == hipSuccess) g_prof_recs.push_back(rec);
    }
    if (rc != VFM_OK) {
      char msg[400];
      snprintf(msg, sizeof(msg), "%s", g_vfm_err);
      VFM_FAIL(rc, "vfm_run_plan: entry %d (kind %d) failed: %s", i, o.kind, msg);
    }
  }
  return VFM_OK;
}

extern "C" int vfm_prof_config(int every) {
  VFM_CHECK(every >= 0, VFM_E_INVAL, "vfm_prof_config: every >= 0");
  g_prof_every = every;
  g_prof_count = 0;
  return VFM_OK;
}

extern "C" int vfm_prof_read(double* out, int cap) {
  VFM_CHECK(out != nullptr || cap == 0, VFM_E_INVAL, "vfm_prof_read: null buffer");
  int n = 0;
  for (const ProfRec& r : g_prof_recs) {
    float ms = 0.f;
    if (hipEventSynchronize(r.e1) == hipSuccess && hipEventElapsedTime(&ms, r.e0, r.e1) == hipSuccess && n < cap) {
      out[3 * n] = (double)r.kind, out[3 * n + 1] = r.flops, out[3 * n + 2] = (double)ms;
      ++n;
    }
    g_prof_pool.push_back(r.e0), g_prof_pool.push_back(r.e1);
  }
  g_prof_recs.clear();
  return n;
}
```

vfmseg_amd/lib.py:

```python
import ctypes as C
import os

import torch

_HERE = os.path.dirname(os.path.abspath(__file__))
LIB_PATH = os.path.join(_HERE, "csrc", "libvfmseg_hip.so")
LIB_PATH_F16 = os.path.join(_HERE, "csrc", "libvfmseg_hip_f16.so")

F32, BF16, U8, I64, SPLIT3 = 0, 1, 2, 3, 4
ABI_VERSION = 9
EP_NONE, EP_GELU, EP_RELU, EP_MUL_GELU_GRAD, EP_MUL, EP_QGELU, EP_MUL_QGELU_GRAD, EP_GELU_DGELU = 0, 1, 2, 3, 4, 5, 6, 7
ACT_NONE, ACT_GELU, ACT_RELU, ACT_QGELU = 0, 1, 2, 3

vp, ci, cl, cf, u64 = C.c_void_p, C.c_int, C.c_long, C.c_float, C.c_uint64


class GemmDesc(C.Structure):
    _fields_ = [
        ("A", vp), ("B", vp), ("C", vp),
        ("in_dt", ci), ("c_dt", ci),
        ("M", cl), ("N", cl), ("K", cl),
        ("sa_m", cl), ("sa_k", cl), ("sb_n", cl), ("sb_k", cl), ("ldc", cl),
        ("alpha", cf),
        ("bias", vp), ("bias_mod", cl),
        ("colscale", vp),
        ("residual", vp), ("r_dt", ci), ("ldr", cl),
        ("ep_mode", ci), ("aux", vp), ("aux_dt", ci), ("ld_aux", cl),
        ("C2", vp), ("c2_dt", ci), ("ldc2", cl),
        ("batch", cl), ("stride_a", cl), ("stride_b", cl), ("stride_c", cl),
        ("c_plane", cl),
        ("kb_rows", cl),
    ]


class AttnDesc(C.Structure):
    _fields_ = [
        ("q", vp), ("k", vp), ("v", vp), ("o", vp),
        ("dt", ci), ("ldq", cl), ("ldk", cl), ("ldv", cl), ("ldo", cl),
        ("B", ci), ("H", ci), ("d", ci),
        ("nq_main", ci), ("nq_extra", ci), ("nk_main", ci), ("nk_extra", ci),
        ("scale", cf),
        ("lse", vp),
        ("dout", vp), ("ld_do", cl),
        ("dq", vp), ("dk", vp), ("dv", vp), ("ld_dq", cl), ("ld_dk", cl), ("ld_dv", cl),
        ("delta", vp),
    ]


class _LnFwd(C.Structure):
    _fields_ = [("x", vp), ("ld_x", cl), ("w", vp), ("b", vp), ("eps", cf), ("y", vp), ("y_dt", ci), ("ld_y", cl), ("stats", vp),
                ("rows", cl), ("C", cl)]


class _LnDrop(C.Structure):
    _fields_ = [("x", vp), ("ld_x", cl), ("w", vp), ("b", vp), ("eps", cf), ("y", vp), ("ld_y", cl), ("stats", vp), ("y_drop", vp),
                ("ld_yd", cl), ("mask", vp), ("ld_mask", cl), ("p", cf), ("offset", u64), ("rows", cl), ("C", cl)]


class _LnBwd(C.Structure):
    _fields_ = [("dy", vp), ("dy_dt", ci), ("ld_dy", cl), ("x", vp), ("ld_x", cl), ("w", vp), ("stats", vp), ("dx", vp), ("ld_dx", cl),
                ("accumulate_dx", ci), ("t_out", vp), ("ld_t", cl), ("t_scale", vp), ("rows", cl), ("C", cl)]


class _CastOp(C.Structure):
    _fields_ = [("src", vp), ("src_dt", ci), ("ld_src", cl), ("dst", vp), ("dst_dt", ci), ("ld_dst", cl), ("rows", cl), ("cols", cl),
                ("colscale", vp)]


class _CopyOp(C.Structure):
    _fields_ = [("src", vp), ("src_dt", ci), ("dst", vp), ("dst_dt", ci), ("n", cl * 4), ("ss", cl * 4), ("ds", cl * 4), ("accumulate", ci)]


class _PlanU(C.Union):
    _fields_ = [("gemm", GemmDesc), ("attn", AttnDesc), ("ln_fwd", _LnFwd), ("ln_drop", _LnDrop), ("ln_bwd", _LnBwd), ("cast", _CastOp),
                ("copy", _CopyOp)]


class PlanOp(C.Structure):
    _fields_ = [("kind", ci), ("prof_kind", ci), ("flops", C.c_double), ("u", _PlanU)]


OP_GEMM, OP_LN_FWD, OP_LN_DROPOUT_FWD, OP_LN_BWD_SCALED, OP_ATTN_FWD, OP_ATTN_BWD, OP_CAST, OP_STRIDED_COPY = range(8)
PROF_NONE, PROF_GEMM, PROF_GEMM_TN, PROF_ATTN_FWD, PROF_ATTN_BWD = range(5)
PROF_NAMES = {PROF_GEMM: "gemm", PROF_GEMM_TN: "gemm_tn", PROF_ATTN_FWD: "attn_fwd", PROF_ATTN_BWD: "attn_bwd"}


class SlideWin(C.Structure):
    _fields_ = [("crop", vp), ("nchw", ci), ("h", ci), ("w", ci), ("y0", ci), ("x0", ci), ("hc", ci), ("wc", ci)]


class AugmentPlan(C.Structure):
    _fields_ = [("resize_h", ci), ("resize_w", ci), ("crop_y", ci), ("crop_x", ci), ("crop_h", ci), ("crop_w", ci), ("flip", ci), ("wide", ci),
                ("brightness_on", ci), ("contrast_on", ci), ("saturation_on", ci), ("hue_on", ci), ("hue_delta", ci),
                ("brightness_beta", C.c_double), ("contrast_alpha", C.c_double), ("saturation_alpha", C.c_double)]


SIGNATURES = {
    "vfm_cast": [vp, ci, cl, vp, ci, cl, cl, cl, vp, vp],
    "vfm_split3": [vp, cl, cl, vp, cl, cl, cl, ci, vp],
    "vfm_transpose": [vp, ci, cl, vp, ci, cl, cl, cl, cl, vp],
    "vfm_strided_copy": [vp, ci, vp, ci] + [cl] * 12 + [ci, vp],
    "vfm_strided_copy_batch": [vp, ci, cl, vp],
    "vfm_axpby": [vp, cf, vp, cf, cl, vp],
    "vfm_scale_by_device_scalar": [vp, vp, cl, vp],
    "vfm_colsum": [vp, ci, cl, cl, cl, vp, ci, vp, vp],
    "vfm_preprocess_u8": [vp, ci, ci, vp, ci, ci, C.POINTER(C.c_float), C.POINTER(C.c_float), ci, cf, vp],
    "vfm_augment_u8": [vp, ci, ci, C.POINTER(AugmentPlan), vp, ci, ci, C.POINTER(C.c_float), C.POINTER(C.c_float), ci, cf, vp],
    "vfm_lora_pack": [vp, ci, cl, ci, vp],
    "vfm_slab_reduce": [vp, ci, cl, cl, cl, cf, vp, cl, cl, ci, vp],
    "vfm_dropout_mask": [vp, ci, cl, cf, u64, u64, vp],
    "vfm_mul_mask": [vp, ci, cl, vp, ci, cl, cl, vp, ci, cl, cl, cl, vp],
    "vfm_geglu_fwd": [vp, ci, cl, vp, ci, cl, cl, cl, vp],
    "vfm_geglu_bwd": [vp, ci, cl, vp, ci, cl, vp, ci, cl, cl, cl, vp],
    "vfm_swiglu_fwd": [vp, ci, cl, vp, ci, cl, cl, cl, vp],
    "vfm_swiglu_bwd": [vp, ci, cl, vp, ci, cl, vp, ci, cl, cl, cl, vp],
    "vfm_rope": [vp, ci, cl, cl, ci, ci, ci, vp, vp, ci, vp],
    "vfm_act_grad_mul": [vp, ci, cl, vp, ci, cl, vp, ci, cl, cl, cl, ci, vp],
    "vfm_mask_token_fwd": [vp, vp, vp, vp, cl, cl, vp],
    "vfm_mask_token_bwd": [vp, vp, vp, vp, vp, cl, cl, vp],
    "vfm_layernorm_fwd": [vp, cl, vp, vp, cf, vp, ci, cl, vp, cl, cl, vp],
    "vfm_layernorm_fwd_split3": [vp, cl, vp, vp, cf, vp, cl, vp, cl, cl, vp, cl, cl, vp],
    "vfm_layernorm_dropout_fwd": [vp, cl, vp, vp, cf, vp, cl, vp, vp, cl, vp, cl, cf, u64, u64, cl, cl, vp],
    "vfm_layernorm_bwd_scaled": [vp, ci, cl, vp, cl, vp, vp, vp, cl, ci, vp, cl, vp, cl, cl, vp],
    "vfm_layernorm_bwd": [vp, ci, cl, vp, cl, vp, vp, vp, cl, ci, vp, vp, vp, cl, cl, vp],
    "vfm_groupnorm_fwd": [vp, vp, vp, cf, ci, ci, vp, ci, vp, vp, cl, cl, cl, vp],
    "vfm_groupnorm_bwd": [vp, ci, vp, vp, vp, vp, ci, ci, vp, vp, vp, vp, cl, cl, cl, vp],
    "vfm_groupnorm_tile_ok": [cl, cl, ci],
    "vfm_groupnorm_tile_fwd": [vp, vp, vp, cf, ci, ci, vp, ci, vp, cl, cl, cl, vp],
    "vfm_groupnorm_tile_bwd": [vp, ci, vp, vp, vp, vp, ci, ci, vp, vp, vp, vp, cl, cl, cl, vp],
    "vfm_bn_moments": [vp, cl, cl, vp, vp, vp],
    "vfm_bn_finalize": [vp, cf, vp, vp, vp, cf, cl, vp],
    "vfm_bn_apply": [vp, vp, vp, vp, cf, ci, vp, ci, cl, cl, vp],
    "vfm_bn_bwd_reduce": [vp, ci, vp, vp, vp, vp, cf, ci, vp, vp, cl, cl, vp],
    "vfm_bn_bwd_apply": [vp, ci, vp, vp, vp, vp, cf, ci, vp, cf, vp, cl, cl, vp],
    "vfm_gemm": [C.POINTER(GemmDesc), vp],
    "vfm_tune": [C.c_char_p, ci],
    "vfm_attn_fwd": [C.POINTER(AttnDesc), vp],
    "vfm_attn_fwd_x3": [C.POINTER(AttnDesc), cl, vp],
    "vfm_attn_fwd_x3_split": [C.POINTER(AttnDesc), cl, vp, cl, cl, vp],
    "vfm_attn_bwd": [C.POINTER(AttnDesc), vp],
    "vfm_attn_bwd_x3": [C.POINTER(AttnDesc), vp, vp, vp, cl, cl, vp, cl, cl, vp],
    "vfm_sam_relpos_table": [vp, ci, ci, ci, vp, vp],
    "vfm_sam_attn_prep": [vp, ci, cl, vp, vp, vp, vp, vp, vp, ci, ci, ci, ci, ci, ci, ci, ci, cf, vp],
    "vfm_softmax_rows": [vp, cl, vp, ci, cl, cl, ci, ci, vp],
    "vfm_sam_attn_merge": [vp, ci, vp, cl, ci, ci, ci, ci, ci, ci, vp],
    "vfm_sam_attn_bwd_prep": [vp, cl, vp, cl, vp, ci, vp, vp, vp, vp, ci, ci, ci, ci, ci, ci, ci, cf, vp],
    "vfm_softmax_rows_batched": [vp, cl, vp, ci, cl, cl, ci, ci, ci, ci, vp],
    "vfm_softmax_rows_bwd": [vp, vp, cl, vp, ci, cl, cl, ci, ci, ci, ci, vp],
    "vfm_rein_mix_fwd": [vp, cl, vp, vp, vp, cl, vp, cl, vp, cl, cl, ci, ci, cf, vp],
    "vfm_rein_mix_bwd": [vp, cl, vp, cl, vp, vp, vp, cl, vp, cl, cl, ci, ci, cf, vp],
    "vfm_sam_attn_bwd_merge": [vp, vp, vp, ci, vp, vp, vp, cl, ci, ci, ci, ci, ci, ci, ci, ci, cf, vp],
    "vfm_sam_attn_flash_fwd": [vp, cl, vp, vp, vp, vp, cl, ci, ci, ci, ci, ci, cf, vp],
    "vfm_sam_attn_flash_fwd_train": [vp, cl, vp, vp, vp, vp, cl, ci, ci, ci, ci, ci, cf, vp, vp, vp],
    "vfm_sam_attn_flash_bwd": [vp, cl, vp, vp, vp, vp, vp, cl, vp, vp, vp, vp, cl, ci, ci, ci, ci, ci, cf, vp],
    "vfm_patchify": [vp, cl, cl, cl, ci, ci, ci, ci, ci, vp, ci, cl, ci, vp],
    "vfm_assemble_tokens": [vp, vp, vp, vp, ci, ci, ci, vp],
    "vfm_resize_bilinear": [vp, ci, ci, ci, ci, ci, ci, cl, vp, ci, ci, cl, ci, ci, ci, ci, ci, ci, cf, cf, vp],
    "vfm_resize_bicubic": [vp, ci, ci, ci, vp, ci, ci, C.c_double, C.c_double, vp],
    "vfm_label_resize": [vp, ci, ci, ci, vp, ci, ci, ci, ci, ci, ci, vp],
    "vfm_unblock": [vp, vp, ci, ci, ci, ci, ci, ci, vp],
    "vfm_upsample_ce": [vp, vp, ci, ci, ci, ci, ci, ci, ci, vp, vp, vp, vp],
    "vfm_upsample_ce_w": [vp, vp, vp, ci, ci, ci, ci, ci, ci, ci, vp, vp, vp, vp],
    "vfm_pseudo_label": [vp, ci, ci, ci, ci, ci, ci, cf, vp, vp, vp, vp],
    "vfm_ohem_prob": [vp, vp, ci, ci, ci, ci, ci, ci, ci, cf, vp, vp, vp],
    "vfm_ohem_threshold": [vp, cl, cl, cf, vp, vp],
    "vfm_label_weight": [vp, vp, vp, vp, vp, ci, cl, ci, ci, vp, vp, vp, vp],
    "vfm_class_presence": [vp, ci, cl, vp, vp],
    "vfm_class_mix": [vp, vp, vp, vp, vp, vp, cl, ci, ci, ci, ci, ci, vp, vp, vp, vp, vp],
    "vfm_hrda_fuse_fwd": [vp, vp, vp] + [ci] * 14 + [vp, vp, vp, vp],
    "vfm_hrda_fuse_bwd": [vp, vp, vp, vp, vp] + [ci] * 14 + [vp, vp, vp, vp, vp],
    "vfm_reduce_sum": [vp, cl, cf, vp, vp],
    "vfm_ce_finish": [vp, cl, cf, vp, cf, vp, vp, vp],
    "vfm_conf_gate": [vp, ci, ci, ci, ci, ci, ci, ci, ci, cf, vp, vp],
    "vfm_slide_accumulate": [vp, ci, ci, ci, ci, ci, vp, vp, ci, ci, ci, ci, ci, ci, vp],
    "vfm_slide_finalize": [vp, vp, vp, ci, ci, ci, ci, vp],
    "vfm_slide_gather": [vp, ci, ci, ci, vp, ci, ci, vp],
    "vfm_conf_gate_windows": [vp, ci, ci, ci, ci, vp, ci, cf, vp, vp],
    "vfm_confusion_hist": [vp, vp, ci, cl, ci, ci, vp, vp],
    "vfm_postprocess_argmax": [vp, ci, cl, cl] + [ci] * 7 + [vp, ci, ci, vp, ci, ci, ci, vp, vp],
    "vfm_adamw": [vp, vp, vp, vp, cl, vp, vp, vp, ci, cf, cf, cf, cf, ci, cf, ci, ci, vp],
    "vfm_adamw_guarded": [vp, vp, vp, vp, cl, vp, vp, vp, ci, cf, cf, cf, cf, ci, cf, ci, ci, vp, vp, vp],
    "vfm_amp_update": [vp, vp, cf, cf, ci, ci, vp],
    "vfm_run_plan": [C.POINTER(PlanOp), ci, u64, u64, vp],
    "vfm_prof_config": [ci],
    "vfm_prof_read": [C.POINTER(C.c_double), ci],
}

_lib = None
_libs = {}
_half = 0
HALF_DTYPES = (torch.bfloat16, torch.float16)


class HipLibraryMissing(RuntimeError):
    pass


def _open(kind):
    path = LIB_PATH_F16 if kind else LIB_PATH
    if not os.path.exists(path):
        raise HipLibraryMissing(
            f"{path} not found: build it with `python -m vfmseg_amd.csrc.build` (hipcc --offload-arch=gfx950)")
    lib = C.CDLL(path)
    lib.vfm_last_error.restype = C.c_char_p
    lib.vfm_abi_version.restype = ci
    lib.vfm_half_kind.restype = ci
    if lib.vfm_abi_version() < ABI_VERSION:
        raise HipLibraryMissing(f"{path} has ABI version {lib.vfm_abi_version()}, this binding needs {ABI_VERSION}: rebuild (python -m vfmseg_amd.csrc.build)")
    if lib.vfm_half_kind() != kind:
        raise HipLibraryMissing(f"{path} reports half kind {lib.vfm_half_kind()}, expected {kind}: stale build")
    for name, args in SIGNATURES.items():
        fn = getattr(lib, name)
        fn.argtypes = args
        fn.restype = ci
    return lib


def load():
    global _lib
    if _lib is not None:
        return _lib
    if _half not in _libs:
        _libs[_half] = _open(_half)
    _lib = _libs[_half]
    return _lib


def set_half(kind):
    global _half, _lib
    kind = {torch.bfloat16: 0, torch.float16: 1, "bf16": 0, "fp16": 1, "f16": 1}.get(kind, kind)
    assert kind in (0, 1)
    if kind != _half:
        _half, _lib = kind, None


def half_dtype():
    return torch.float16 if _half else torch.bfloat16


class HipError(RuntimeError):
    pass


def check(rc, name):
    if rc != 0:
        raise HipError(f"{name} failed ({rc}): {load().vfm_last_error().decode()}")


_raw_stream = getattr(torch._C, "_cuda_getCurrentRawStream", None)
_dev_index = None


def stream():
    global _dev_index
    if _raw_stream is not None:
        if _dev_index is None:
            _dev_index = torch.cuda.current_device()
        return _raw_stream(_dev_index)
    return torch.cuda.current_stream().cuda_stream


def set_device_index(i):
    global _dev_index
    _dev_index = i


def dt_of(t):
    if t.dtype == torch.float32:
        return F32
    if t.dtype == torch.bfloat16 or t.dtype == torch.float16:
        if (t.dtype == torch.float16) != bool(_half):
            raise TypeError(f"{t.dtype} tensor handed to the {'fp16' if _half else 'bf16'} library (precision mode and tensors disagree)")
        return BF16
    if t.dtype == torch.uint8 or t.dtype == torch.bool:
        return U8
# ... 16 lines not shown
```

vfmseg_amd/ops.py:

```python
import ctypes as C
import os

import torch

from .precision import is_half
from . import lib as L
from .lib import (ACT_GELU, ACT_NONE, ACT_QGELU, ACT_RELU, BF16, EP_GELU, EP_GELU_DGELU, EP_MUL, EP_MUL_GELU_GRAD,
                  EP_MUL_QGELU_GRAD, EP_NONE, EP_QGELU, EP_RELU, F32)

_ws_cache = {}

PROFILE = None
REGION = ["heads"]


class region:
    def __init__(self, name):
        self.name = name

    def __enter__(self):
        REGION.append(self.name)

    def __exit__(self, *a):
        REGION.pop()
# ... 64 lines not shown
        self.keep, self.max_elems, self.n = [], 0, len(jobs)
        for job in jobs:
            src, dst, shape, sstr, dstr = job[:5]
            acc = int(bool(job[5])) if len(job) > 5 else 0
            nsum, sstride = (int(job[6]), int(job[7])) if len(job) > 7 else (1, 0)
            assert src.dtype == torch.float32 and src.is_cuda and dst.is_cuda and (not acc or dst.dtype == torch.float32)
            k = 4 - len(shape)
            n, s_, d_ = [1] * k + list(shape), [0] * k + list(sstr), [0] * k + list(dstr)
            buf += struct.pack("2Q16q", src.data_ptr(), dst.data_ptr(), L.dt_of(dst), acc, *n, *s_, *d_, nsum, sstride)
            self.keep += [src, dst]
            e = 1
            for v in shape:
                e *= v
            self.max_elems = max(self.max_elems, e)
        self.table = torch.frombuffer(buf, dtype=torch.uint8).clone().to(jobs[0][1].device) if jobs else None

    def run(self):
        if self.n:
            lib = L.load()
            L.check(lib.vfm_strided_copy_batch(L.ptr(self.table), self.n, self.max_elems, L.stream()), "vfm_strided_copy_batch")


def permute_copy(src, perm, dst):
    v = src.permute(*perm)
    strided_copy(src, dst, list(v.shape), list(v.stride()), list(torch.empty(v.shape, device="meta").stride()))
    return dst


def axpby(x, a, y, b):
    lib = L.load()
    assert x.is_contiguous() and y.is_contiguous() and x.dtype == y.dtype == torch.float32 and x.numel() == y.numel()
    L.check(lib.vfm_axpby(L.ptr(x), float(a), L.ptr(y), float(b), x.numel(), L.stream()), "vfm_axpby")
    return y


def scale_by_device_scalar(y, scalar):
    lib = L.load()
    assert y.is_contiguous() and y.dtype == torch.float32
    L.check(lib.vfm_scale_by_device_scalar(L.ptr(y), L.ptr(scalar), y.numel(), L.stream()), "vfm_scale_by_device_scalar")
    return y


def colsum(x, out, accumulate=False):
    lib = L.load()
    rows, cols = x.shape
    ws = workspace(64 * cols, x.device)
    L.check(lib.vfm_colsum(L.ptr(x), L.dt_of(x), _ld(x), rows, cols, L.ptr(out), int(accumulate), L.ptr(ws), L.stream()),
            "vfm_colsum")
    return out


def dropout_mask(out, p, seed, offset=0):
    lib = L.load()
    assert out.is_contiguous()
    L.check(lib.vfm_dropout_mask(L.ptr(out), L.dt_of(out), out.numel(), float(p), int(seed), int(offset), L.stream()),
            "vfm_dropout_mask")
    return out


def mul_mask(src, mask, dst, rows_per_group=1):
    lib = L.load()
    L.check(lib.vfm_mul_mask(L.ptr(src), L.dt_of(src), _ld(src), L.ptr(mask), L.dt_of(mask), _ld(mask), rows_per_group,
                             L.ptr(dst), L.dt_of(dst), _ld(dst), src.shape[0], src.shape[1], L.stream()), "vfm_mul_mask")
    return dst


def geglu_fwd(h, out):
    lib = L.load()
    rows, c2 = h.shape
    L.check(lib.vfm_geglu_fwd(L.ptr(h), L.dt_of(h), _ld(h), L.ptr(out), L.dt_of(out), _ld(out), rows, c2 // 2, L.stream()),
            "vfm_geglu_fwd")
    return out


def geglu_bwd(h, dout, dh):
    lib = L.load()
    rows, c2 = h.shape
    L.check(lib.vfm_geglu_bwd(L.ptr(h), L.dt_of(h), _ld(h), L.ptr(dout), L.dt_of(dout), _ld(dout), L.ptr(dh), L.dt_of(dh),
                              _ld(dh), rows, c2 // 2, L.stream()), "vfm_geglu_bwd")
    return dh


def swiglu_fwd(h, out, C_):
    lib = L.load()
    L.check(lib.vfm_swiglu_fwd(L.ptr(h), L.dt_of(h), _ld(h), L.ptr(out), L.dt_of(out), _ld(out), h.shape[0], C_, L.stream()),
            "vfm_swiglu_fwd")
    return out


def swiglu_bwd(h, dout, dh, C_):
    lib = L.load()
    L.check(lib.vfm_swiglu_bwd(L.ptr(h), L.dt_of(h), _ld(h), L.ptr(dout), L.dt_of(dout), _ld(dout), L.ptr(dh), L.dt_of(dh),
                               _ld(dh), h.shape[0], C_, L.stream()), "vfm_swiglu_bwd")
    return dh


def rope(x, rows, np_, ncols, d, cos_t, sin_t, inverse=False):
    lib = L.load()
    L.check(lib.vfm_rope(L.ptr(x), L.dt_of(x), _ld(x), rows, np_, ncols, d, L.ptr(cos_t), L.ptr(sin_t), int(inverse), L.stream()),
            "vfm_rope")
    return x


def act_grad_mul(dy, pre, out, act):
    lib = L.load()
    L.check(lib.vfm_act_grad_mul(L.ptr(dy), L.dt_of(dy), _ld(dy), L.ptr(pre), L.dt_of(pre), _ld(pre), L.ptr(out),
                                 L.dt_of(out), _ld(out), dy.shape[0], dy.shape[1], act, L.stream()), "vfm_act_grad_mul")
    return out


def mask_token_fwd(x, keep, token, out):
    lib = L.load()
    L.check(lib.vfm_mask_token_fwd(L.ptr(x), L.ptr(keep), L.ptr(token), L.ptr(out), x.shape[0], x.shape[1], L.stream()),
            "vfm_mask_token_fwd")
    return out


def mask_token_bwd(dout, keep, dx, dtoken):
    lib = L.load()
    ws = workspace(64 * dout.shape[1], dout.device)
    L.check(lib.vfm_mask_token_bwd(L.ptr(dout), L.ptr(keep), L.ptr(dx), L.ptr(dtoken), L.ptr(ws), dout.shape[0], dout.shape[1],
                                   L.stream()), "vfm_mask_token_bwd")


def _split_key(t):
    return (t.data_ptr(), tuple(t.shape), tuple(t.stride()), t._version)


def _register_split_out(t, t3):
    try:
        t._vfm_split3_out = (_split_key(t), t3)
    except AttributeError:
        pass


def layernorm_fwd(x, w, b, eps, y, stats=None, split_out=None):
    lib = L.load()
    rows, c = x.shape
    if split_out and _split3_on() and y.dtype == torch.float32 and c % 256 == 0 and c // 256 in (1, 2, 4, 5, 8) and y.shape[1] == c:
        kp = (c + 63) // 64 * 64
        y3 = torch.empty(rows, 3 * kp, dtype=L.half_dtype(), device=x.device)
        L.check(lib.vfm_layernorm_fwd_split3(L.ptr(x), _ld(x), L.ptr(w), L.ptr(b), float(eps), None if split_out == "only" else L.ptr(y), _ld(y),
                                             L.ptr(y3), y3.stride(0), kp, L.ptr(stats), rows, c, L.stream()), "vfm_layernorm_fwd_split3")
        _register_split_out(y, y3)
        return y
    L.check(lib.vfm_layernorm_fwd(L.ptr(x), _ld(x), L.ptr(w), L.ptr(b), float(eps), L.ptr(y), L.dt_of(y), _ld(y),
                                  L.ptr(stats), rows, c, L.stream()), "vfm_layernorm_fwd")
    return y


def layernorm_dropout_fwd(x, w, b, eps, y, stats, y_drop, mask, p, seed, offset=0):
    lib = L.load()
    rows, c = x.shape
    assert is_half(y.dtype) and is_half(y_drop.dtype) and is_half(mask.dtype)
    L.check(lib.vfm_layernorm_dropout_fwd(L.ptr(x), _ld(x), L.ptr(w), L.ptr(b), float(eps), L.ptr(y), _ld(y), L.ptr(stats),
                                          L.ptr(y_drop), _ld(y_drop), L.ptr(mask), _ld(mask), float(p), int(seed), int(offset),
                                          rows, c, L.stream()), "vfm_layernorm_dropout_fwd")
    return y


def layernorm_bwd_scaled(dy, x, w, stats, dx, t_out, t_scale, accumulate_dx=False):
    lib = L.load()
    rows, c = x.shape
    assert is_half(t_out.dtype) and t_scale.dtype == torch.float32
    L.check(lib.vfm_layernorm_bwd_scaled(L.ptr(dy), L.dt_of(dy), _ld(dy), L.ptr(x), _ld(x), L.ptr(w), L.ptr(stats), L.ptr(dx),
                                         _ld(dx), int(accumulate_dx), L.ptr(t_out), _ld(t_out), L.ptr(t_scale), rows, c,
                                         L.stream()), "vfm_layernorm_bwd_scaled")
    return dx


def layernorm_bwd(dy, x, w, stats, dx, accumulate_dx=False, dw=None, db=None):
    lib = L.load()
    rows, c = x.shape
    ws = workspace(2 * 128 * c, x.device) if (dw is not None or db is not None) else None
    L.check(lib.vfm_layernorm_bwd(L.ptr(dy), L.dt_of(dy), _ld(dy), L.ptr(x), _ld(x), L.ptr(w), L.ptr(stats), L.ptr(dx),
                                  _ld(dx), int(accumulate_dx), L.ptr(dw), L.ptr(db), L.ptr(ws), rows, c, L.stream()),
            "vfm_layernorm_bwd")
    return dx


def groupnorm_fwd(x, w, b, eps, groups, act, y, stats, B, P):
    lib = L.load()
    c = x.shape[1]
    ws = workspace(B * groups * 2 + B * 64 * 2 * c, x.device)
    L.check(lib.vfm_groupnorm_fwd(L.ptr(x), L.ptr(w), L.ptr(b), float(eps), groups, act, L.ptr(y), L.dt_of(y), L.ptr(stats),
                                  L.ptr(ws), B, P, c, L.stream()), "vfm_groupnorm_fwd")
    return y


def groupnorm_bwd(dy, x, w, b, stats, groups, act, dx, dw, db, B, P):
    lib = L.load()
    c = x.shape[1]
    ws = workspace(B * groups * 2 + B * 64 * 2 * c, x.device)
    L.check(lib.vfm_groupnorm_bwd(L.ptr(dy), L.dt_of(dy), L.ptr(x), L.ptr(w), L.ptr(b), L.ptr(stats), groups, act, L.ptr(dx),
                                  L.ptr(dw), L.ptr(db), L.ptr(ws), B, P, c, L.stream()), "vfm_groupnorm_bwd")
    return dx


def groupnorm_tile_ok(P, C, groups):
    return bool(L.load().vfm_groupnorm_tile_ok(int(P), int(C), int(groups)))


def groupnorm_tile_fwd(x, w, b, eps, groups, act, y, stats, B, P):
    lib = L.load()
    L.check(lib.vfm_groupnorm_tile_fwd(L.ptr(x), L.ptr(w), L.ptr(b), float(eps), groups, act, L.ptr(y), L.dt_of(y), L.ptr(stats),
                                       B, P, x.shape[1], L.stream()), "vfm_groupnorm_tile_fwd")
    return y


def groupnorm_tile_bwd(dy, x, w, b, stats, groups, act, dx, dw, db, B, P):
    lib = L.load()
    c = x.shape[1]
    ws = workspace(B * 2 * c, x.device)
    L.check(lib.vfm_groupnorm_tile_bwd(L.ptr(dy), L.dt_of(dy), L.ptr(x), L.ptr(w), L.ptr(b), L.ptr(stats), groups, act, L.ptr(dx),
                                       L.ptr(dw), L.ptr(db), L.ptr(ws), B, P, c, L.stream()), "vfm_groupnorm_tile_bwd")
    return dx


def bn_moments(x, sums):
    lib = L.load()
    rows, c = x.shape
    ws = workspace(64 * 2 * c, x.device)
    L.check(lib.vfm_bn_moments(L.ptr(x), rows, c, L.ptr(sums), L.ptr(ws), L.stream()), "vfm_bn_moments")
    return sums


def bn_finalize(sums, count, mean_var, running_mean=None, running_var=None, momentum=0.1):
    lib = L.load()
    L.check(lib.vfm_bn_finalize(L.ptr(sums), float(count), L.ptr(mean_var), L.ptr(running_mean), L.ptr(running_var),
                                float(momentum), sums.shape[1], L.stream()), "vfm_bn_finalize")
    return mean_var


def bn_apply(x, mean_var, w, b, eps, act, y):
    lib = L.load()
    rows, c = x.shape
    L.check(lib.vfm_bn_apply(L.ptr(x), L.ptr(mean_var), L.ptr(w), L.ptr(b), float(eps), act, L.ptr(y), L.dt_of(y), rows, c,
                             L.stream()), "vfm_bn_apply")
    return y


def bn_bwd_reduce(dy, x, mean_var, w, b, eps, act, sums_dy):
    lib = L.load()
    rows, c = x.shape
    ws = workspace(64 * 2 * c, x.device)
    L.check(lib.vfm_bn_bwd_reduce(L.ptr(dy), L.dt_of(dy), L.ptr(x), L.ptr(mean_var), L.ptr(w), L.ptr(b), float(eps), act,
                                  L.ptr(sums_dy), L.ptr(ws), rows, c, L.stream()), "vfm_bn_bwd_reduce")
    return sums_dy


def bn_bwd_apply(dy, x, mean_var, w, b, eps, act, sums_dy, total_rows, dx):
    lib = L.load()
    rows, c = x.shape
    L.check(lib.vfm_bn_bwd_apply(L.ptr(dy), L.dt_of(dy), L.ptr(x), L.ptr(mean_var), L.ptr(w), L.ptr(b), float(eps), act,
                                 L.ptr(sums_dy), float(total_rows), L.ptr(dx), rows, c, L.stream()), "vfm_bn_bwd_apply")
    return dx


def split3(x, pattern, trans=False, cache=False):
    if pattern == 0 and not trans:
        hit = getattr(x, "_vfm_split3_out", None)
        if hit is not None and hit[0] == _split_key(x):
            return hit[1]
    if cache:
        from .optim import PARAM_EPOCH
        key = (PARAM_EPOCH[0], x._version, x.data_ptr(), pattern, trans, tuple(x.shape), tuple(x.stride()))
        hit = getattr(x, "_vfm_split3", None)
        if hit is not None and hit[0] == key:
            return hit[1]
    rows, K = (x.shape[1], x.shape[0]) if trans else (x.shape[0], x.shape[1])
    sr, sc = (x.stride(1), x.stride(0)) if trans else (x.stride(0), x.stride(1))
    kp = (K + 63) // 64 * 64
    out = torch.empty(rows, 3 * kp, dtype=L.half_dtype(), device=x.device)
    L.check(L.load().vfm_split3(L.ptr(x), sr, sc, L.ptr(out), out.stride(0), rows, K, pattern, L.stream()), "vfm_split3")
    if cache:
        try:
            x._vfm_split3 = (key, out)
        except AttributeError:
            pass
    return out


def gemm(a, b, c, *, alpha=1.0, bias=None, bias_mod=0, colscale=None, residual=None, ep_mode=EP_NONE, aux=None, c2=None,
         trans_a=False, trans_b=False, kb_rows=0, c_split=None):
    if a.dtype == torch.float32 and b.dtype == torch.float32 and a.dim() == 2 and not kb_rows and _split3_on():
        a3 = split3(a, 0, trans=trans_a)
        b3 = split3(b, 1, trans=trans_b, cache=not b.requires_grad)
        c3 = None
        if (c_split == "only" and c.dtype == torch.float32 and c.dim() == 2 and c.shape[1] % 64 == 0 and residual is None and c2 is None
                and ep_mode in (EP_NONE, EP_GELU)):
            c3 = torch.empty(c.shape[0], 3 * c.shape[1], dtype=L.half_dtype(), device=c.device)
        gemm(a3, b3, c, alpha=alpha, bias=bias, bias_mod=bias_mod, colscale=colscale, residual=residual, ep_mode=ep_mode, aux=aux, c2=c2, c_split=c3)
        if c3 is not None:
            _register_split_out(c, c3)
        return c
    lib = L.load()
    d = gemm_desc(a, b, c, alpha=alpha, bias=bias, bias_mod=bias_mod, colscale=colscale, residual=residual, ep_mode=ep_mode, aux=aux, c2=c2,
                  trans_a=trans_a, trans_b=trans_b, kb_rows=kb_rows)
    if torch.is_tensor(c_split):
        d.C, d.c_dt, d.ldc, d.c_plane = L.ptr(c_split), L.SPLIT3, c_split.stride(0), c.shape[1]
    fin = PROFILE("gemm", 2.0 * d.M * d.N * d.K * d.batch, REGION[-1]) if (PROFILE is not None and is_half(a.dtype)) else None
    L.check(lib.vfm_gemm(C.byref(d), L.stream()), "vfm_gemm")
    if fin is not None:
        fin()
    return c


def gemm_desc(a, b, c, *, alpha=1.0, bias=None, bias_mod=0, colscale=None, residual=None, ep_mode=EP_NONE, aux=None, c2=None,
              trans_a=False, trans_b=False, kb_rows=0, d=None):
    d = L.GemmDesc() if d is None else d
    batched = a.dim() == 3
    a2 = a[0] if batched else a
    b2 = b[0] if batched else b
    c2d = c[0] if batched else c
    if trans_a:
        K, M = a2.shape
        d.sa_m, d.sa_k = a2.stride(1), a2.stride(0)
    else:
        M, K = a2.shape
        d.sa_m, d.sa_k = a2.stride(0), a2.stride(1)
    if trans_b:
        Kb, N = b2.shape
        d.sb_n, d.sb_k = b2.stride(1), b2.stride(0)
    else:
        N, Kb = b2.shape
        d.sb_n, d.sb_k = b2.stride(0), b2.stride(1)
    if kb_rows:
        assert trans_b and Kb == kb_rows and K >= Kb, "kb_rows: b holds the first kb_rows of the K (token) dimension"
        d.kb_rows = int(kb_rows)
    else:
        assert K == Kb, f"gemm K mismatch {K} vs {Kb}"
    assert a.dtype == b.dtype
    assert c2d.shape[0] == M and c2d.shape[1] == N and c2d.stride(1) == 1
    d.A, d.B, d.C = L.ptr(a), L.ptr(b), L.ptr(c)
    d.in_dt, d.c_dt = L.dt_of(a), L.dt_of(c)
    d.M, d.N, d.K = M, N, K
    d.ldc = c2d.stride(0)
    d.alpha = float(alpha)
    d.bias, d.bias_mod = L.ptr(bias), int(bias_mod)
    d.colscale = L.ptr(colscale)
    if residual is not None:
        r2 = residual[0] if batched else residual
        d.residual, d.r_dt, d.ldr = L.ptr(residual), L.dt_of(residual), r2.stride(0)
    d.ep_mode = ep_mode
    if aux is not None:
        d.aux, d.aux_dt, d.ld_aux = L.ptr(aux), L.dt_of(aux), aux.stride(0)
    if c2 is not None:
        d.C2, d.c2_dt, d.ldc2 = L.ptr(c2), L.dt_of(c2), c2.stride(0)
    if batched:
        d.batch, d.stride_a, d.stride_b, d.stride_c = a.shape[0], a.stride(0), b.stride(0), c.stride(0)
    else:
        d.batch = 1
    return d


class Plan:

    def __init__(self, region="backbone"):
        self.ops, self.keep, self.arr, self.region = [], [], None, region

    def _new(self, kind, prof=L.PROF_NONE, flops=0.0, *tensors):
        op = L.PlanOp()
        op.kind, op.prof_kind, op.flops = kind, prof, float(flops)
        self.ops.append(op)
        self.keep.extend(t for t in tensors if t is not None)
        self.arr = None
        return op

    def gemm(self, a, b, c, **kw):
        op = self._new(L.OP_GEMM, L.PROF_GEMM if is_half(a.dtype) else L.PROF_NONE, 0.0, a, b, c, kw.get("bias"), kw.get("colscale"),
                       kw.get("residual"), kw.get("aux"), kw.get("c2"))
        d = gemm_desc(a, b, c, d=op.u.gemm, **kw)
        op.flops = 2.0 * d.M * d.N * d.K * d.batch
        return len(self.ops) - 1

    def layernorm_fwd(self, x, w, b, eps, y, stats):
        op = self._new(L.OP_LN_FWD, L.PROF_NONE, 0.0, x, w, b, y, stats)
        u = op.u.ln_fwd
        u.x, u.ld_x, u.w, u.b, u.eps, u.y, u.y_dt, u.ld_y, u.stats = L.ptr(x), _ld(x), L.ptr(w), L.ptr(b), float(eps), L.ptr(y), L.dt_of(y), _ld(y), L.ptr(stats)
        u.rows, u.C = x.shape
        return len(self.ops) - 1

    def layernorm_dropout_fwd(self, x, w, b, eps, y, stats, y_drop, mask, p, offset):
        assert is_half(y.dtype) and is_half(y_drop.dtype) and is_half(mask.dtype)
        op = self._new(L.OP_LN_DROPOUT_FWD, L.PROF_NONE, 0.0, x, w, b, y, stats, y_drop, mask)
        u = op.u.ln_drop
        u.x, u.ld_x, u.w, u.b, u.eps, u.y, u.ld_y, u.stats = L.ptr(x), _ld(x), L.ptr(w), L.ptr(b), float(eps), L.ptr(y), _ld(y), L.ptr(stats)
        u.y_drop, u.ld_yd, u.mask, u.ld_mask, u.p, u.offset = L.ptr(y_drop), _ld(y_drop), L.ptr(mask), _ld(mask), float(p), int(offset)
        u.rows, u.C = x.shape
        return len(self.ops) - 1

    def layernorm_bwd_scaled(self, dy, x, w, stats, dx, t_out, t_scale, accumulate_dx=False):
        assert is_half(t_out.dtype) and t_scale.dtype == torch.float32
        op = self._new(L.OP_LN_BWD_SCALED, L.PROF_NONE, 0.0, dy, x, w, stats, dx, t_out, t_scale)
        u = op.u.ln_bwd
        u.dy, u.dy_dt, u.ld_dy, u.x, u.ld_x, u.w, u.stats = L.ptr(dy), L.dt_of(dy), _ld(dy), L.ptr(x), _ld(x), L.ptr(w), L.ptr(stats)
        u.dx, u.ld_dx, u.accumulate_dx, u.t_out, u.ld_t, u.t_scale = L.ptr(dx), _ld(dx), int(accumulate_dx), L.ptr(t_out), _ld(t_out), L.ptr(t_scale)
        u.rows, u.C = x.shape
        return len(self.ops) - 1

    def attn_fwd(self, q, k, v, o, lse, B, H, d, nq_main, nq_extra, nk_main, nk_extra, scale):
        fl = 4.0 * B * H * (nq_main + nq_extra) * (nk_main + nk_extra) * d
        op = self._new(L.OP_ATTN_FWD, L.PROF_ATTN_FWD if is_half(q.dtype) else L.PROF_NONE, fl, q, k, v, o, lse)
        C.memmove(C.byref(op.u.attn), C.byref(_attn_desc(q, k, v, o, B, H, d, nq_main, nq_extra, nk_main, nk_extra, scale, lse)), C.sizeof(L.AttnDesc))
        return len(self.ops) - 1

    def attn_bwd(self, q, k, v, o, lse, dout, dq, dk, dv, B, H, d, nq_main, nq_extra, nk_main, nk_extra, scale):
        fl = 10.0 * B * H * (nq_main + nq_extra) * (nk_main + nk_extra) * d
        delta = _attn_bwd_delta(q, B, H, nq_main + nq_extra)
        op = self._new(L.OP_ATTN_BWD, L.PROF_ATTN_BWD if is_half(q.dtype) else L.PROF_NONE, fl, q, k, v, o, lse, dout, dq, dk, dv, delta)
        a = _attn_desc(q, k, v, o, B, H, d, nq_main, nq_extra, nk_main, nk_extra, scale, lse)
        a.dout, a.ld_do = L.ptr(dout), dout.stride(0)
        a.dq, a.dk, a.dv = L.ptr(dq), L.ptr(dk), L.ptr(dv)
        a.ld_dq, a.ld_dk, a.ld_dv = dq.stride(0), dk.stride(0), dv.stride(0)
        a.delta = L.ptr(delta)
        C.memmove(C.byref(op.u.attn), C.byref(a), C.sizeof(L.AttnDesc))
        return len(self.ops) - 1

    def cast(self, src, dst, colscale=None):
        op = self._new(L.OP_CAST, L.PROF_NONE, 0.0, src, dst, colscale)
        u = op.u.cast
        u.src, u.src_dt, u.ld_src, u.dst, u.dst_dt, u.ld_dst = L.ptr(src), L.dt_of(src), _ld(src), L.ptr(dst), L.dt_of(dst), _ld(dst)
        u.rows, u.cols = src.shape
        u.colscale = L.ptr(colscale)
        return len(self.ops) - 1

    def strided_copy(self, src, dst, shape, sstr, dstr, accumulate=False):
        op = self._new(L.OP_STRIDED_COPY, L.PROF_NONE, 0.0, src, dst)
        u = op.u.copy
        k = 4 - len(shape)
        u.src, u.src_dt, u.dst, u.dst_dt = L.ptr(src), L.dt_of(src), L.ptr(dst), L.dt_of(dst)
        for i, (n, s_, d_) in enumerate(zip([1] * k + list(shape), [0] * k + list(sstr), [0] * k + list(dstr))):
            u.n[i], u.ss[i], u.ds[i] = n, s_, d_
        u.accumulate = int(accumulate)
        return len(self.ops) - 1

    def _array(self):
        if self.arr is None:
            self.arr = (L.PlanOp * len(self.ops))()
            for i, op in enumerate(self.ops):
                C.memmove(C.byref(self.arr[i]), C.byref(op), C.sizeof(L.PlanOp))
        return self.arr

    def entry(self, i):
        return self._array()[i]

    def run(self, seed=0, rng_base=0, start=0, count=None):
        arr = self._array()
        n = len(self.ops) - start if count is None else count
        first = C.cast(C.byref(arr, start * C.sizeof(L.PlanOp)), C.POINTER(L.PlanOp))
        L.check(L.load().vfm_run_plan(first, n, int(seed), int(rng_base), L.stream()), "vfm_run_plan")

    def __len__(self):
        return len(self.ops)


def prof_config(every):
    L.check(L.load().vfm_prof_config(int(every)), "vfm_prof_config")


def prof_read(cap=65536):
    buf = (C.c_double * (3 * cap))()
    n = L.load().vfm_prof_read(buf, cap)
    if n < 0:
        L.check(n, "vfm_prof_read")
    return [(L.PROF_NAMES.get(int(buf[3 * i]), "other"), buf[3 * i + 1], buf[3 * i + 2]) for i in range(n)]


class LoraPackTable:

    def __init__(self, sites, dt_tensor):
        import struct
        buf = bytearray()
        self.max_elems = 0
        self.keep = []
        for (A, B, a, at, w, wt, r, K, N, Kw) in sites:
            assert A.dtype == torch.float32 and B.dtype == torch.float32 and A.is_contiguous() and B.is_contiguous()
            self.keep += [A, B, a, at, w, wt]
            buf += struct.pack("6Q8q", A.data_ptr(), B.data_ptr(), a.data_ptr(), at.data_ptr(), w.data_ptr(),
                               wt.data_ptr() if wt is not None else 0, r, K, N, Kw, a.stride(0), at.stride(0), w.stride(0),
                               wt.stride(0) if wt is not None else 0)
            self.max_elems = max(self.max_elems, r * (K + N))
        self.n = len(sites)
        self.dt = L.dt_of(dt_tensor)
        dev = sites[0][2].device
        self.table = torch.frombuffer(buf, dtype=torch.uint8).clone().to(dev)
        self.ptrs = [s_[0].data_ptr() for s_ in sites] + [s_[1].data_ptr() for s_ in sites]

    def valid_for(self, sites):
        return self.n == len(sites) and self.ptrs == [s_[0].data_ptr() for s_ in sites] + [s_[1].data_ptr() for s_ in sites]

    def run(self):
        lib = L.load()
        L.check(lib.vfm_lora_pack(L.ptr(self.table), self.n, self.max_elems, self.dt, L.stream()), "vfm_lora_pack")


def slab_reduce(slabs, rows_used, dst, sp, sq, alpha=1.0, accumulate=False):
    lib = L.load()
    kch, P, Q = slabs.shape
    assert slabs.is_contiguous() and slabs.dtype == torch.float32 and dst.dtype == torch.float32
    L.check(lib.vfm_slab_reduce(L.ptr(slabs), kch, P, Q, int(rows_used), float(alpha), L.ptr(dst), int(sp), int(sq), int(accumulate),
                                L.stream()), "vfm_slab_reduce")
    return dst


def gemm_splitk_bt(at, y, slabs, kch):
    lib = L.load()
    d = L.GemmDesc()
    P, mp = at.shape
    M, Q = y.shape
    ck = mp // kch
    assert ck * kch == mp and ck % 64 == 0 and slabs.shape == (kch, P, Q)
    d.A, d.B, d.C = L.ptr(at), L.ptr(y), L.ptr(slabs)
    d.in_dt, d.c_dt = L.dt_of(at), L.dt_of(slabs)
    d.M, d.N, d.K = P, Q, ck
    d.sa_m, d.sa_k = at.stride(0), 1
    d.sb_n, d.sb_k = 1, y.stride(0)
    d.ldc = slabs.stride(1)
    d.alpha = 1.0
    d.batch, d.stride_a, d.stride_b, d.stride_c = kch, ck, ck * y.stride(0), slabs.stride(0)
    d.kb_rows = int(M)
    fin = PROFILE("gemm_tn", 2.0 * P * Q * mp, REGION[-1]) if PROFILE is not None else None
    L.check(lib.vfm_gemm(C.byref(d), L.stream()), "vfm_gemm")
    if fin is not None:
        fin()
    return slabs


def gemm_splitk_tn(xs, y, slabs, kch):
    lib = L.load()
    d = L.GemmDesc()
    M, P = xs.shape
    M2, Q = y.shape
    assert M == M2 and xs.stride(1) == 1 and y.stride(1) == 1
    mp = (M + 63) // 64 * 64
    ck = mp // kch
    assert ck * kch == mp and ck % 64 == 0 and slabs.shape == (kch, P, Q)
    d.A, d.B, d.C = L.ptr(xs), L.ptr(y), L.ptr(slabs)
    d.in_dt, d.c_dt = L.dt_of(xs), L.dt_of(slabs)
    d.M, d.N, d.K = P, Q, ck
    d.sa_m, d.sa_k = 1, xs.stride(0)
    d.sb_n, d.sb_k = 1, y.stride(0)
# ... 667 lines not shown
```

Baseline: 137.4 images/s.

## Add specialized LoRA down/up kernels with dropout mask regeneration

Adds dedicated HIP kernels for the rank-64 LoRA down-projection (split-K across waves with an LDS reduction) and the up-projection. The up-projection fuses the dropout mask, scaling and residual add, and can rebuild the dropout mask from the hash RNG instead of reading a stored one. Mode 1, the default, routes only the down-projection to the new kernel in place of the generic GEMM. Mode 2 also skips storing the per-layer M×D dropout mask and regenerates it in backward, trading extra hash work for less memory traffic and footprint.

```diff
diff --git a/include/vfmseg_hip.h b/include/vfmseg_hip.h
--- a/include/vfmseg_hip.h
+++ b/include/vfmseg_hip.h
@@ -66,6 +66,10 @@
 int vfm_layernorm_dropout_fwd(const float* x, long ld_x, const float* w, const float* b, float eps, void* y, long ld_y,
                               float* stats, void* y_drop, long ld_yd, void* mask, long ld_mask, float p, uint64_t seed,
                               uint64_t offset, long rows, long C, void* stream);
+int vfm_lora_down(const void* x, long ld_x, const void* a, long ld_a, void* t, long ld_t, float alpha, long M, long K, int r_live,
+                  void* stream);
+int vfm_lora_up_masked(const void* g, long ld_g, const void* at, long ld_at, const void* residual, long ld_r, void* out, long ld_o,
+                       float alpha, float p, uint64_t seed, uint64_t offset, long M, long N, void* stream);
 int vfm_layernorm_bwd_scaled(const void* dy, int dy_dt, long ld_dy, const float* x, long ld_x, const float* w,
                              const float* stats, float* dx, long ld_dx, int accumulate_dx, void* t_out, long ld_t,
                              const float* t_scale, long rows, long C, void* stream);
@@ -243,7 +247,7 @@
 int vfm_amp_update(const int* flag, float* amp_state, float growth, float backoff, int interval, int dynamic, void* stream);
 
 enum { VFM_OP_GEMM = 0, VFM_OP_LN_FWD = 1, VFM_OP_LN_DROPOUT_FWD = 2, VFM_OP_LN_BWD_SCALED = 3, VFM_OP_ATTN_FWD = 4, VFM_OP_ATTN_BWD = 5,
-       VFM_OP_CAST = 6, VFM_OP_STRIDED_COPY = 7 };
+       VFM_OP_CAST = 6, VFM_OP_STRIDED_COPY = 7, VFM_OP_LORA_DOWN = 8, VFM_OP_LORA_UP = 9 };
 enum { VFM_PROF_NONE = 0, VFM_PROF_GEMM = 1, VFM_PROF_GEMM_TN = 2, VFM_PROF_ATTN_FWD = 3, VFM_PROF_ATTN_BWD = 4 };
 typedef struct vfm_plan_op {
   int kind;
@@ -260,6 +264,9 @@
              long ld_dx; int accumulate_dx; void* t_out; long ld_t; const float* t_scale; long rows, C; } ln_bwd;
     struct { const void* src; int src_dt; long ld_src; void* dst; int dst_dt; long ld_dst; long rows, cols; const float* colscale; } cast;
     struct { const void* src; int src_dt; void* dst; int dst_dt; long n[4]; long ss[4]; long ds[4]; int accumulate; } copy;
+    struct { const void* x; long ld_x; const void* a; long ld_a; void* t; long ld_t; float alpha; int r_live; long M, K; } lora_down;
+    struct { const void* g; long ld_g; const void* at; long ld_at; const void* residual; long ld_r; void* out; long ld_o; float alpha;
+             float p; uint64_t offset; long M, N; } lora_up;
   } u;
 } vfm_plan_op;
 int vfm_run_plan(const vfm_plan_op* ops, int n, uint64_t seed, uint64_t rng_base, void* stream);
diff --git a/vfmseg_amd/backbones.py b/vfmseg_amd/backbones.py
--- a/vfmseg_amd/backbones.py
+++ b/vfmseg_amd/backbones.py
@@ -345,6 +345,15 @@
     return grad_out
 
 
+def lora_side_mode():
+    v = os.environ.get("VFMSEG_LORA_SIDE", "1")
+    return 0 if v == "0" else (2 if v == "2" else 1)
+
+
+def lora_side_on():
+    return lora_side_mode() != 0
+
+
 class _DinoTrainPlan:
 
     def __init__(self, eng, P, nimg, Np):
@@ -361,7 +370,10 @@
         e = lambda *sh, dt=cd: torch.empty(*sh, dtype=dt, device=dev)
         f32 = torch.float32
         self.X = e(nL + 1, M, D, dt=f32)
-        self.A1, self.XD, self.MASK = e(nL, M, kq), e(nL, M, D), e(nL, M, D)
+        self.side, self.regen = lora_side_mode() >= 1, lora_side_mode() == 2
+        self.A1, self.XD = e(nL, M, kq), e(nL, M, D)
+        if not self.regen:
+            self.MASK = e(nL, M, D)
         self.ST1, self.ST2 = e(nL, M, 2, dt=f32), e(nL, M, 2, dt=f32)
         self.QKV, self.AO = e(nL, M, 3 * D), e(nL, M, D)
         self.LSE = e(nL, nimg, H, Np + 1, dt=f32)
@@ -379,8 +391,12 @@
         for li, (blk, Lp) in enumerate(zip(v.blocks, P["layers"])):
             q = blk.attn.qkv
             x, a1 = self.X[li], self.A1[li]
-            f.layernorm_dropout_fwd(x, Lp["n1w"], Lp["n1b"], 1e-6, a1[:, :D], self.ST1[li], self.XD[li], self.MASK[li], q.p, li * M * D)
-            f.gemm(self.XD[li], Lp["a"], a1[:, D:D + R_PAD], alpha=q.scaling)
+            f.layernorm_dropout_fwd(x, Lp["n1w"], Lp["n1b"], 1e-6, a1[:, :D], self.ST1[li], self.XD[li], None if self.regen else self.MASK[li],
+                                    q.p, li * M * D)
+            if self.side:
+                f.lora_down(self.XD[li], Lp["a"], a1[:, D:D + R_PAD], alpha=q.scaling, r_live=min(q.r, R_PAD))
+            else:
+                f.gemm(self.XD[li], Lp["a"], a1[:, D:D + R_PAD], alpha=q.scaling)
             f.gemm(a1, Lp["qkv"].w, self.QKV[li], bias=Lp["qkv_b"])
             qkv = self.QKV[li]
             f.attn_fwd(qkv[:, :D], qkv[:, D:2 * D], qkv[:, 2 * D:], self.AO[li], self.LSE[li], nimg, H, hd, Np, 1, Np, 1, scale)
@@ -448,7 +464,10 @@
                     pl.gemm(dqkv, Lp["qkv"].wt[D:D + R_PAD], da1[:, D:D + R_PAD])
                     continue
                 pl.gemm(dqkv, Lp["qkv"].wt, da1)
-                pl.gemm(da1[:, D:D + R_PAD], Lp["at"], da1[:, :D], alpha=q.scaling, residual=da1[:, :D], ep_mode=ops.EP_MUL, aux=self.MASK[li])
+                if self.regen:
+                    pl.lora_up_masked(da1[:, D:D + R_PAD], Lp["at"], da1[:, :D], da1[:, :D], alpha=q.scaling, p=q.p, offset=li * M * D)
+                else:
+                    pl.gemm(da1[:, D:D + R_PAD], Lp["at"], da1[:, :D], alpha=q.scaling, residual=da1[:, :D], ep_mode=ops.EP_MUL, aux=self.MASK[li])
                 if li > 0:
                     add_tap(pl, pn, li - 1)
                     pl.layernorm_bwd_scaled(da1[:, :D], self.X[li], Lp["n1w"], self.ST1[li], self.DX, self.T, P["layers"][li - 1]["g2"],
@@ -467,7 +486,7 @@
             self.bwd[pn][0].entry(idx).u.copy.src = dxcat.data_ptr() + col * esz
         self.DX.zero_()
         for pl, lo, hi in self.bwd:
-            pl.run()
+            pl.run(ctx["seed"], ctx["rng0"])
             self.eng._lora_wgrads_batched(self.P, ctx, self.DA1, self.DQKV, lo, hi, self.M, self.D)
             if BACKWARD_EVENTS["block_done"] is not None:
                 for lj in range(hi - 1, lo - 1, -1):
@@ -639,9 +658,11 @@
         if plan is not None:
             plan.run_forward(xcat, seed, rng0)
             plan.busy = True
-            ctx = dict(saved=None, plan=plan, nimg=nimg, Np=Np, M=M, Mp=Mp, P=P, training=training, A1all=plan.A1, XDall=plan.XD)
+            ctx = dict(saved=None, plan=plan, nimg=nimg, Np=Np, M=M, Mp=Mp, P=P, training=training, A1all=plan.A1, XDall=plan.XD,
+                       seed=seed, rng0=rng0)
             return xcat, (hp, wp), ctx
         nL = len(v.blocks)
+        side = lora_side_mode()
         batched = lora and training and is_half(cd) and merged is None
         A1all = torch.empty(nL, M, P["layers"][0]["qkv"].k, dtype=cd, device=dev) if batched else None
         XDall = None
@@ -654,8 +675,12 @@
             st1 = torch.empty(M, 2, dtype=torch.float32, device=dev)
             q = blk.attn.qkv if lora else None
             fused_drop = lora and training and q.p > 0 and is_half(cd) and D % 256 == 0
+            regen = None
             if fused_drop:
-                mask = torch.empty(M, D, dtype=cd, device=dev)
+                if side == 2:
+                    mask, regen = None, (q.p, seed, rng0 + li * M * D)
+                else:
+                    mask = torch.empty(M, D, dtype=cd, device=dev)
                 if batched and XDall is None:
                     XDall = torch.empty(nL, M, D, dtype=cd, device=dev)
                 xd = XDall[li] if batched else torch.empty(M, D, dtype=cd, device=dev)
@@ -671,8 +696,11 @@
                         ops.dropout_mask(mask, q.p, seed, offset=rng0 + li * M * D)
                         xd = torch.empty(M, D, dtype=cd, device=dev)
                         ops.mul_mask(a1[:, :D], mask, xd)
-                ops.gemm(xd, Lp["a"], a1[:, D:D + R_PAD], alpha=q.scaling)
-                S.update(xd=xd if mask is not None else None, mask=mask)
+                if fused_drop and side:
+                    ops.lora_down(xd, Lp["a"], a1[:, D:D + R_PAD], alpha=q.scaling, r_live=min(q.r, R_PAD))
+                else:
+                    ops.gemm(xd, Lp["a"], a1[:, D:D + R_PAD], alpha=q.scaling)
+                S.update(xd=xd if (mask is not None or regen is not None) else None, mask=mask, regen=regen)
             qkv = torch.empty(M, 3 * D, dtype=cd, device=dev)
             if merged is not None:
                 ops.gemm(a1, merged[li], qkv, bias=Lp["qkv_b"])
@@ -724,6 +752,15 @@
         if pl.busy or not pl.eligible_backward():
             return None
         return pl
+
+    @staticmethod
+    def _lora_dgrad(S, Lp, da1, D, scaling):
+        if S.get("regen") is not None:
+            p, seed, offset = S["regen"]
+            ops.lora_up_masked(da1[:, D:D + R_PAD], Lp["at"], da1[:, :D], da1[:, :D], alpha=scaling, p=p, seed=seed, offset=offset)
+            return
+        ep = dict(ep_mode=ops.EP_MUL, aux=S["mask"]) if S["mask"] is not None else {}
+        ops.gemm(da1[:, D:D + R_PAD], Lp["at"], da1[:, :D], alpha=scaling, residual=da1[:, :D], **ep)
 
     def backward(self, ctx, dxcat):
         if ctx.get("plan") is not None:
@@ -792,8 +829,7 @@
             da1 = DA1all[li] if wg_batched else torch.empty(M, kq, dtype=cd, device=dev)
             Lp["qkv"].dgrad(dqkv, da1)
             if isinstance(q, LoraLinear) and wg_batched:
-                ep = dict(ep_mode=ops.EP_MUL, aux=S["mask"]) if S["mask"] is not None else {}
-                ops.gemm(da1[:, D:D + R_PAD], Lp["at"], da1[:, :D], alpha=q.scaling, residual=da1[:, :D], **ep)
+                self._lora_dgrad(S, Lp, da1, D, q.scaling)
             elif isinstance(q, LoraLinear):
                 r = q.r
                 A, Bm = q.lora_A["default"].weight, q.lora_B["default"].weight
@@ -820,8 +856,7 @@
                     ops.axpby(gAp[:r].reshape(-1), 1.0, tA.view(-1), 1.0)
                 else:
                     grads[2 * li] = gAp[:r]
-                ep = dict(ep_mode=ops.EP_MUL, aux=S["mask"]) if S["mask"] is not None else {}
-                ops.gemm(da1[:, D:D + R_PAD], Lp["at"], da1[:, :D], alpha=q.scaling, residual=da1[:, :D], **ep)
+                self._lora_dgrad(S, Lp, da1, D, q.scaling)
             if fuse_t1 and li > 0:
                 add_tap(li - 1)
                 ops.layernorm_bwd_scaled(da1[:, :D], S["x_in"], Lp["n1w"], S["st1"], dx, t, P["layers"][li - 1]["g2"],
diff --git a/vfmseg_amd/csrc/elementwise.hip b/vfmseg_amd/csrc/elementwise.hip
--- a/vfmseg_amd/csrc/elementwise.hip
+++ b/vfmseg_amd/csrc/elementwise.hip
@@ -3,7 +3,7 @@
 thread_local char g_vfm_err[512] = {0};
 
 extern "C" const char* vfm_last_error(void) { return g_vfm_err; }
-extern "C" int vfm_abi_version(void) { return 9; }
+extern "C" int vfm_abi_version(void) { return 10; }
 extern "C" int vfm_half_kind(void) { return VFM_HALF_KIND; }
 
 template <typename TI, typename TO>
diff --git a/vfmseg_amd/csrc/lora_side.hip b/vfmseg_amd/csrc/lora_side.hip
--- /dev/null
+++ b/vfmseg_amd/csrc/lora_side.hip
@@ -0,0 +1,177 @@
+#include "common.h"
+
+namespace {
+typedef float f32x4 __attribute__((ext_vector_type(4)));
+typedef vfm_h h16x8 __attribute__((ext_vector_type(8)));
+
+constexpr int LS_ROWS = 16;
+constexpr int LS_R = 64;
+constexpr int DOWN_WAVES = 8;
+constexpr int DOWN_PITCH = LS_R + 4;
+constexpr int UP_WAVES = 16;
+constexpr int UP_COLS = 512;
+constexpr int UP_PITCH = UP_COLS + 4;
+
+__device__ __forceinline__ h16x8 ld_frag(const bf16_t* p) { return *reinterpret_cast<const h16x8*>(p); }
+
+template <int NT>
+__global__ __launch_bounds__(DOWN_WAVES * 64) void k_lora_down(const bf16_t* __restrict__ X, long ld_x, const bf16_t* __restrict__ A, long ld_a,
+                                                               bf16_t* __restrict__ T, long ld_t, float alpha, long M, int K) {
+  __shared__ float red[DOWN_WAVES * LS_ROWS * DOWN_PITCH];
+  const int lane = threadIdx.x & 63, w = threadIdx.x >> 6;
+  const int r = lane & 15, kq = (lane >> 4) * 8;
+  const long row0 = (long)blockIdx.x * LS_ROWS;
+  const bf16_t* xp = X + (row0 + r < M ? row0 + r : row0) * ld_x + kq;
+  const bf16_t* ap = A + (long)r * ld_a + kq;
+  f32x4 acc[NT];
+#pragma unroll
+  for (int j = 0; j < NT; ++j) acc[j] = f32x4{0.f, 0.f, 0.f, 0.f};
+  const int S = K >> 5;
+  int k0 = ((w * S) / DOWN_WAVES) * 32;
+  const int k1 = (((w + 1) * S) / DOWN_WAVES) * 32;
+  for (; k0 + 3 * 32 < k1; k0 += 4 * 32) {
+    h16x8 fx[4];
+#pragma unroll
+    for (int u = 0; u < 4; ++u) fx[u] = ld_frag(xp + k0 + u * 32);
+#pragma unroll
+    for (int u = 0; u < 4; ++u) {
+#pragma unroll
+      for (int j = 0; j < NT; ++j) acc[j] = VFM_MFMA16S(fx[u], ld_frag(ap + (long)j * 16 * ld_a + k0 + u * 32), acc[j]);
+    }
+  }
+  for (; k0 < k1; k0 += 32) {
+    const h16x8 fx = ld_frag(xp + k0);
+#pragma unroll
+    for (int j = 0; j < NT; ++j) acc[j] = VFM_MFMA16S(fx, ld_frag(ap + (long)j * 16 * ld_a + k0), acc[j]);
+  }
+  float* mine = red + (w * LS_ROWS + (lane >> 4) * 4) * DOWN_PITCH + r;
+#pragma unroll
+  for (int j = 0; j < NT; ++j) {
+#pragma unroll
+    for (int i = 0; i < 4; ++i) mine[i * DOWN_PITCH + j * 16] = acc[j][i];
+  }
+  __syncthreads();
+  if (threadIdx.x >= LS_ROWS * 16) return;
+  const int orow = threadIdx.x >> 4, oc = (threadIdx.x & 15) * 4;
+  if (row0 + orow >= M) return;
+  ushort4 o = {0, 0, 0, 0};
+  if ((oc >> 4) < NT) {
+    float4 s = *reinterpret_cast<const float4*>(red + orow * DOWN_PITCH + oc);
+#pragma unroll
+    for (int v = 1; v < DOWN_WAVES; ++v) {
+      const float4 q = *reinterpret_cast<const float4*>(red + (v * LS_ROWS + orow) * DOWN_PITCH + oc);
+      s.x += q.x, s.y += q.y, s.z += q.z, s.w += q.w;
+    }
+    o = ushort4{f32_to_bf16(alpha * s.x), f32_to_bf16(alpha * s.y), f32_to_bf16(alpha * s.z), f32_to_bf16(alpha * s.w)};
+  }
+  *reinterpret_cast<ushort4*>(T + (row0 + orow) * ld_t + oc) = o;
+}
+
+template <bool DROP>
+__global__ __launch_bounds__(UP_WAVES * 64) void k_lora_up(const bf16_t* __restrict__ G, long ld_g, const bf16_t* __restrict__ At, long ld_at,
+                                                           const bf16_t* R, long ld_r, bf16_t* O, long ld_o, float alpha, float p,
+                                                           float keep_scale, uint64_t seed, uint64_t offset, long M, int N) {
+  __shared__ float tile[LS_ROWS * UP_PITCH];
+  const int lane = threadIdx.x & 63, w = threadIdx.x >> 6;
+  const int r = lane & 15, kq = (lane >> 4) * 8;
+  const long row0 = (long)blockIdx.x * LS_ROWS;
+  const bf16_t* gp = G + (row0 + r < M ? row0 + r : row0) * ld_g + kq;
+  const h16x8 g0 = ld_frag(gp), g1 = ld_frag(gp + 32);
+  const long erow = row0 + w;
+  const int ec = lane * 8;
+  const bool elive = erow < M;
+  const float ksf = bf16_to_f32(f32_to_bf16(keep_scale));
+  float* mine = tile + (lane >> 4) * 4 * UP_PITCH + w * 32 + r;
+  const float* fin = tile + w * UP_PITCH + ec;
+  for (int c0 = 0; c0 < N; c0 += UP_COLS) {
+    const int ncol = N - c0 < UP_COLS ? N - c0 : UP_COLS;
+    const bool mlive = w * 32 < ncol, flive = elive && ec < ncol;
+    uint4 rv = {};
+    if (flive) rv = *reinterpret_cast<const uint4*>(R + erow * ld_r + c0 + ec);
+    f32x4 acc[2];
+    if (mlive) {
+#pragma unroll
+      for (int j = 0; j < 2; ++j) {
+        const bf16_t* bp = At + (long)(c0 + w * 32 + j * 16 + r) * ld_at + kq;
+        acc[j] = VFM_MFMA16S(g0, ld_frag(bp), (f32x4{0.f, 0.f, 0.f, 0.f}));
+        acc[j] = VFM_MFMA16S(g1, ld_frag(bp + 32), acc[j]);
+      }
+    }
+    __syncthreads();
+    if (mlive) {
+#pragma unroll
+      for (int j = 0; j < 2; ++j) {
+#pragma unroll
+        for (int i = 0; i < 4; ++i) mine[i * UP_PITCH + j * 16] = acc[j][i];
+      }
+    }
+    __syncthreads();
+    if (!flive) continue;
+    const float4 a0 = *reinterpret_cast<const float4*>(fin), a1 = *reinterpret_cast<const float4*>(fin + 4);
+    const float a[8] = {a0.x, a0.y, a0.z, a0.w, a1.x, a1.y, a1.z, a1.w};
+    const uint32_t rw[4] = {rv.x, rv.y, rv.z, rv.w};
+    const int col = c0 + ec;
+    const uint64_t e0 = offset + (uint64_t)erow * (uint64_t)N + (uint64_t)col;
+    uint32_t ow[4];
+#pragma unroll
+    for (int h = 0; h < 4; ++h) {
+      float v0 = alpha * a[2 * h], v1 = alpha * a[2 * h + 1];
+      if constexpr (DROP) {
+        const bool k0 = (hash_u32(seed, e0 + 2 * h) >> 8) * (1.0f / 16777216.0f) >= p;
+        const bool k1 = (hash_u32(seed, e0 + 2 * h + 1) >> 8) * (1.0f / 16777216.0f) >= p;
+        v0 *= k0 ? ksf : 0.f;
+        v1 *= k1 ? ksf : 0.f;
+      }
+      v0 += h16_lo(rw[h]);
+      v1 += h16_hi(rw[h]);
+      ow[h] = (uint32_t)f32_to_bf16(v0) | ((uint32_t)f32_to_bf16(v1) << 16);
+    }
+    *reinterpret_cast<uint4*>(O + erow * ld_o + col) = uint4{ow[0], ow[1], ow[2], ow[3]};
+  }
+}
+
+inline bool al16(const void* p) { return (uintptr_t)p % 16 == 0; }
+}
+
+extern "C" int vfm_lora_down(const void* x, long ld_x, const void* a, long ld_a, void* t, long ld_t, float alpha, long M, long K, int r_live,
+                             void* stream) {
+  VFM_CHECK(x != nullptr && a != nullptr && t != nullptr, VFM_E_INVAL, "vfm_lora_down: null operand");
+  VFM_CHECK(M >= 0 && r_live >= 1 && r_live <= LS_R, VFM_E_INVAL, "vfm_lora_down: M=%ld r_live=%d", M, r_live);
+  VFM_CHECK(K > 0 && K % 32 == 0 && K <= (1L << 24), VFM_E_SHAPE, "vfm_lora_down: K=%ld (K %% 32 == 0)", K);
+  VFM_CHECK(al16(x) && al16(a) && al16(t) && ld_x % 8 == 0 && ld_a % 8 == 0 && ld_t % 8 == 0, VFM_E_ALIGN,
+            "vfm_lora_down: pointers and pitches must be 16-byte aligned");
+  VFM_CHECK(ld_x >= K && ld_a >= K && ld_t >= LS_R, VFM_E_SHAPE, "vfm_lora_down: pitch shorter than a row");
+  if (M == 0) return VFM_OK;
+#define LDN(NT)                                                                                                                              \
+  hipLaunchKernelGGL((k_lora_down<NT>), dim3(cdiv(M, LS_ROWS)), dim3(DOWN_WAVES * 64), 0, (hipStream_t)stream, (const bf16_t*)x, ld_x,       \
+                     (const bf16_t*)a, ld_a, (bf16_t*)t, ld_t, alpha, M, (int)K)
+  switch ((r_live + 15) / 16) {
+    case 1: LDN(1); break;
+    case 2: LDN(2); break;
+    case 3: LDN(3); break;
+    default: LDN(4); break;
+  }
+#undef LDN
+  VFM_LAUNCH_CHECK();
+  return VFM_OK;
+}
+
+extern "C" int vfm_lora_up_masked(const void* g, long ld_g, const void* at, long ld_at, const void* residual, long ld_r, void* out, long ld_o,
+                                  float alpha, float p, uint64_t seed, uint64_t offset, long M, long N, void* stream) {
+  VFM_CHECK(g != nullptr && at != nullptr && residual != nullptr && out != nullptr, VFM_E_INVAL, "vfm_lora_up_masked: null operand");
+  VFM_CHECK(M >= 0 && p >= 0.f && p < 1.f, VFM_E_INVAL, "vfm_lora_up_masked: M=%ld p=%g", M, (double)p);
+  VFM_CHECK(N > 0 && N % 256 == 0 && N <= (1L << 24), VFM_E_SHAPE, "vfm_lora_up_masked: N=%ld (N %% 256 == 0)", N);
+  VFM_CHECK(al16(g) && al16(at) && al16(residual) && al16(out) && ld_g % 8 == 0 && ld_at % 8 == 0 && ld_r % 8 == 0 && ld_o % 8 == 0,
+            VFM_E_ALIGN, "vfm_lora_up_masked: pointers and pitches must be 16-byte aligned");
+  VFM_CHECK(ld_g >= LS_R && ld_at >= LS_R && ld_r >= N && ld_o >= N, VFM_E_SHAPE, "vfm_lora_up_masked: pitch shorter than a row");
+  if (M == 0) return VFM_OK;
+  const dim3 grid(cdiv(M, LS_ROWS)), blk(UP_WAVES * 64);
+  hipStream_t s = (hipStream_t)stream;
+#define LUP(DROP)                                                                                                                      \
+  hipLaunchKernelGGL((k_lora_up<DROP>), grid, blk, 0, s, (const bf16_t*)g, ld_g, (const bf16_t*)at, ld_at, (const bf16_t*)residual, ld_r, \
+                     (bf16_t*)out, ld_o, alpha, p, 1.0f / (1.0f - p), seed, offset, M, (int)N)
+  if (p > 0.f) LUP(true); else LUP(false);
+#undef LUP
+  VFM_LAUNCH_CHECK();
+  return VFM_OK;
+}
diff --git a/vfmseg_amd/csrc/norm.hip b/vfmseg_amd/csrc/norm.hip
--- a/vfmseg_amd/csrc/norm.hip
+++ b/vfmseg_amd/csrc/norm.hip
@@ -59,7 +59,7 @@
   *reinterpret_cast<ushort4*>(p + so.plane) = hi;
   *reinterpret_cast<ushort4*>(p + 2 * so.plane) = lo;
 }
-template <typename TO, int NV, bool DROP = false, bool SPLIT = false>
+template <typename TO, int NV, bool DROP = false, bool SPLIT = false, bool MASK = true>
 __global__ void k_ln_fwd_v4(const float* __restrict__ x, long ld_x, const float* __restrict__ w, const float* __restrict__ b,
                             float eps, TO* __restrict__ y, long ld_y, float* __restrict__ stats, long rows, int C, LnDrop dr = LnDrop(),
                             Split3Out so = Split3Out()) {
@@ -113,7 +113,7 @@
         yd.y = k1 ? f32_to_bf16(bf16_to_f32(p.y) * ksf) : f32_to_bf16(bf16_to_f32(p.y) * 0.f);
         yd.z = k2 ? f32_to_bf16(bf16_to_f32(p.z) * ksf) : f32_to_bf16(bf16_to_f32(p.z) * 0.f);
         yd.w = k3 ? f32_to_bf16(bf16_to_f32(p.w) * ksf) : f32_to_bf16(bf16_to_f32(p.w) * 0.f);
-        *reinterpret_cast<ushort4*>((bf16_t*)dr.mask + row * dr.ld_mask + c0) = mk;
+        if constexpr (MASK) *reinterpret_cast<ushort4*>((bf16_t*)dr.mask + row * dr.ld_mask + c0) = mk;
         *reinterpret_cast<ushort4*>((bf16_t*)dr.yd + row * dr.ld_yd + c0) = yd;
       }
     } else {
@@ -356,7 +356,11 @@
   hipStream_t s = (hipStream_t)stream;
   dim3 blk(256), grid(cdiv(rows, 4));
   LnDrop dr{y_drop, ld_yd, mask, ld_mask, p, 1.0f / (1.0f - p), seed, offset};
-#define LVD(NV) hipLaunchKernelGGL((k_ln_fwd_v4<bf16_t, NV, true>), grid, blk, 0, s, x, ld_x, w, b, eps, (bf16_t*)y, ld_y, stats, rows, (int)C, dr)
+#define LVD(NV)                                                                                                                        \
+  do {                                                                                                                                 \
+    if (mask) hipLaunchKernelGGL((k_ln_fwd_v4<bf16_t, NV, true, false, true>), grid, blk, 0, s, x, ld_x, w, b, eps, (bf16_t*)y, ld_y, stats, rows, (int)C, dr);  \
+    else hipLaunchKernelGGL((k_ln_fwd_v4<bf16_t, NV, true, false, false>), grid, blk, 0, s, x, ld_x, w, b, eps, (bf16_t*)y, ld_y, stats, rows, (int)C, dr);     \
+  } while (0)
   if (nv == 1) LVD(1); else if (nv == 2) LVD(2); else if (nv == 4) LVD(4); else if (nv == 5) LVD(5); else LVD(8);
 #undef LVD
   VFM_LAUNCH_CHECK();
diff --git a/vfmseg_amd/csrc/plan.hip b/vfmseg_amd/csrc/plan.hip
--- a/vfmseg_amd/csrc/plan.hip
+++ b/vfmseg_amd/csrc/plan.hip
@@ -52,6 +52,15 @@
       return vfm_strided_copy(a.src, a.src_dt, a.dst, a.dst_dt, a.n[0], a.n[1], a.n[2], a.n[3], a.ss[0], a.ss[1], a.ss[2], a.ss[3], a.ds[0],
                               a.ds[1], a.ds[2], a.ds[3], a.accumulate, s);
     }
+    case VFM_OP_LORA_DOWN: {
+      const auto& a = o.u.lora_down;
+      return vfm_lora_down(a.x, a.ld_x, a.a, a.ld_a, a.t, a.ld_t, a.alpha, a.M, a.K, a.r_live, s);
+    }
+    case VFM_OP_LORA_UP: {
+      const auto& a = o.u.lora_up;
+      return vfm_lora_up_masked(a.g, a.ld_g, a.at, a.ld_at, a.residual, a.ld_r, a.out, a.ld_o, a.alpha, a.p, seed, rng_base + a.offset, a.M,
+                                a.N, s);
+    }
     default: VFM_FAIL(VFM_E_INVAL, "vfm_run_plan: unknown op kind %d", o.kind);
   }
 }
diff --git a/vfmseg_amd/lib.py b/vfmseg_amd/lib.py
--- a/vfmseg_amd/lib.py
+++ b/vfmseg_amd/lib.py
@@ -8,7 +8,7 @@
 LIB_PATH_F16 = os.path.join(_HERE, "csrc", "libvfmseg_hip_f16.so")
 
 F32, BF16, U8, I64, SPLIT3 = 0, 1, 2, 3, 4
-ABI_VERSION = 9
+ABI_VERSION = 10
 EP_NONE, EP_GELU, EP_RELU, EP_MUL_GELU_GRAD, EP_MUL, EP_QGELU, EP_MUL_QGELU_GRAD, EP_GELU_DGELU = 0, 1, 2, 3, 4, 5, 6, 7
 ACT_NONE, ACT_GELU, ACT_RELU, ACT_QGELU = 0, 1, 2, 3
 
@@ -71,16 +71,25 @@
     _fields_ = [("src", vp), ("src_dt", ci), ("dst", vp), ("dst_dt", ci), ("n", cl * 4), ("ss", cl * 4), ("ds", cl * 4), ("accumulate", ci)]
 
 
+class _LoraDown(C.Structure):
+    _fields_ = [("x", vp), ("ld_x", cl), ("a", vp), ("ld_a", cl), ("t", vp), ("ld_t", cl), ("alpha", cf), ("r_live", ci), ("M", cl), ("K", cl)]
+
+
+class _LoraUp(C.Structure):
+    _fields_ = [("g", vp), ("ld_g", cl), ("at", vp), ("ld_at", cl), ("residual", vp), ("ld_r", cl), ("out", vp), ("ld_o", cl), ("alpha", cf),
+                ("p", cf), ("offset", u64), ("M", cl), ("N", cl)]
+
+
 class _PlanU(C.Union):
     _fields_ = [("gemm", GemmDesc), ("attn", AttnDesc), ("ln_fwd", _LnFwd), ("ln_drop", _LnDrop), ("ln_bwd", _LnBwd), ("cast", _CastOp),
-                ("copy", _CopyOp)]
+                ("copy", _CopyOp), ("lora_down", _LoraDown), ("lora_up", _LoraUp)]
 
 
 class PlanOp(C.Structure):
     _fields_ = [("kind", ci), ("prof_kind", ci), ("flops", C.c_double), ("u", _PlanU)]
 
 
-OP_GEMM, OP_LN_FWD, OP_LN_DROPOUT_FWD, OP_LN_BWD_SCALED, OP_ATTN_FWD, OP_ATTN_BWD, OP_CAST, OP_STRIDED_COPY = range(8)
+OP_GEMM, OP_LN_FWD, OP_LN_DROPOUT_FWD, OP_LN_BWD_SCALED, OP_ATTN_FWD, OP_ATTN_BWD, OP_CAST, OP_STRIDED_COPY, OP_LORA_DOWN, OP_LORA_UP = range(10)
 PROF_NONE, PROF_GEMM, PROF_GEMM_TN, PROF_ATTN_FWD, PROF_ATTN_BWD = range(5)
 PROF_NAMES = {PROF_GEMM: "gemm", PROF_GEMM_TN: "gemm_tn", PROF_ATTN_FWD: "attn_fwd", PROF_ATTN_BWD: "attn_bwd"}
 
@@ -121,6 +130,8 @@
     "vfm_layernorm_fwd": [vp, cl, vp, vp, cf, vp, ci, cl, vp, cl, cl, vp],
     "vfm_layernorm_fwd_split3": [vp, cl, vp, vp, cf, vp, cl, vp, cl, cl, vp, cl, cl, vp],
     "vfm_layernorm_dropout_fwd": [vp, cl, vp, vp, cf, vp, cl, vp, vp, cl, vp, cl, cf, u64, u64, cl, cl, vp],
+    "vfm_lora_down": [vp, cl, vp, cl, vp, cl, cf, cl, cl, ci, vp],
+    "vfm_lora_up_masked": [vp, cl, vp, cl, vp, cl, vp, cl, cf, cf, u64, u64, cl, cl, vp],
     "vfm_layernorm_bwd_scaled": [vp, ci, cl, vp, cl, vp, vp, vp, cl, ci, vp, cl, vp, cl, cl, vp],
     "vfm_layernorm_bwd": [vp, ci, cl, vp, cl, vp, vp, vp, cl, ci, vp, vp, vp, cl, cl, vp],
     "vfm_groupnorm_fwd": [vp, vp, vp, cf, ci, ci, vp, ci, vp, vp, cl, cl, cl, vp],
diff --git a/vfmseg_amd/ops.py b/vfmseg_amd/ops.py
--- a/vfmseg_amd/ops.py
+++ b/vfmseg_amd/ops.py
@@ -240,11 +240,35 @@
 def layernorm_dropout_fwd(x, w, b, eps, y, stats, y_drop, mask, p, seed, offset=0):
     lib = L.load()
     rows, c = x.shape
-    assert is_half(y.dtype) and is_half(y_drop.dtype) and is_half(mask.dtype)
+    assert is_half(y.dtype) and is_half(y_drop.dtype) and (mask is None or is_half(mask.dtype))
     L.check(lib.vfm_layernorm_dropout_fwd(L.ptr(x), _ld(x), L.ptr(w), L.ptr(b), float(eps), L.ptr(y), _ld(y), L.ptr(stats),
-                                          L.ptr(y_drop), _ld(y_drop), L.ptr(mask), _ld(mask), float(p), int(seed), int(offset),
-                                          rows, c, L.stream()), "vfm_layernorm_dropout_fwd")
+                                          L.ptr(y_drop), _ld(y_drop), L.ptr(mask), _ld(mask) if mask is not None else 0, float(p), int(seed),
+                                          int(offset), rows, c, L.stream()), "vfm_layernorm_dropout_fwd")
     return y
+
+
+def lora_down(x, a, t, alpha=1.0, r_live=64):
+    lib = L.load()
+    M, K = x.shape
+    assert is_half(x.dtype) and a.dtype == x.dtype and t.dtype == x.dtype and a.shape == (64, K) and t.shape == (M, 64)
+    fin = PROFILE("gemm", 2.0 * M * 64 * K, REGION[-1]) if PROFILE is not None else None
+    L.check(lib.vfm_lora_down(L.ptr(x), _ld(x), L.ptr(a), _ld(a), L.ptr(t), _ld(t), float(alpha), M, K, int(r_live), L.stream()), "vfm_lora_down")
+    if fin is not None:
+        fin()
+    return t
+
+
+def lora_up_masked(g, at, residual, out, alpha=1.0, p=0.0, seed=0, offset=0):
+    lib = L.load()
+    M, N = out.shape
+    assert is_half(g.dtype) and at.dtype == g.dtype and residual.dtype == g.dtype and out.dtype == g.dtype
+    assert g.shape == (M, 64) and at.shape == (N, 64) and residual.shape == (M, N)
+    fin = PROFILE("gemm", 2.0 * M * N * 64, REGION[-1]) if PROFILE is not None else None
+    L.check(lib.vfm_lora_up_masked(L.ptr(g), _ld(g), L.ptr(at), _ld(at), L.ptr(residual), _ld(residual), L.ptr(out), _ld(out), float(alpha),
+                                   float(p), int(seed), int(offset), M, N, L.stream()), "vfm_lora_up_masked")
+    if fin is not None:
+        fin()
+    return out
 
 
 def layernorm_bwd_scaled(dy, x, w, stats, dx, t_out, t_scale, accumulate_dx=False):
@@ -470,12 +494,31 @@
         return len(self.ops) - 1
 
     def layernorm_dropout_fwd(self, x, w, b, eps, y, stats, y_drop, mask, p, offset):
-        assert is_half(y.dtype) and is_half(y_drop.dtype) and is_half(mask.dtype)
+        assert is_half(y.dtype) and is_half(y_drop.dtype) and (mask is None or is_half(mask.dtype))
         op = self._new(L.OP_LN_DROPOUT_FWD, L.PROF_NONE, 0.0, x, w, b, y, stats, y_drop, mask)
         u = op.u.ln_drop
         u.x, u.ld_x, u.w, u.b, u.eps, u.y, u.ld_y, u.stats = L.ptr(x), _ld(x), L.ptr(w), L.ptr(b), float(eps), L.ptr(y), _ld(y), L.ptr(stats)
-        u.y_drop, u.ld_yd, u.mask, u.ld_mask, u.p, u.offset = L.ptr(y_drop), _ld(y_drop), L.ptr(mask), _ld(mask), float(p), int(offset)
+        u.y_drop, u.ld_yd, u.p, u.offset = L.ptr(y_drop), _ld(y_drop), float(p), int(offset)
+        u.mask, u.ld_mask = (L.ptr(mask), _ld(mask)) if mask is not None else (None, 0)
         u.rows, u.C = x.shape
+        return len(self.ops) - 1
+
+    def lora_down(self, x, a, t, alpha=1.0, r_live=64):
+        assert is_half(x.dtype) and a.dtype == x.dtype and t.dtype == x.dtype and a.shape == (64, x.shape[1]) and t.shape == (x.shape[0], 64)
+        op = self._new(L.OP_LORA_DOWN, L.PROF_GEMM, 2.0 * x.shape[0] * 64 * x.shape[1], x, a, t)
+        u = op.u.lora_down
+        u.x, u.ld_x, u.a, u.ld_a, u.t, u.ld_t, u.alpha, u.r_live = L.ptr(x), _ld(x), L.ptr(a), _ld(a), L.ptr(t), _ld(t), float(alpha), int(r_live)
+        u.M, u.K = x.shape
+        return len(self.ops) - 1
+
+    def lora_up_masked(self, g, at, residual, out, alpha=1.0, p=0.0, offset=0):
+        M, N = out.shape
+        assert is_half(g.dtype) and at.dtype == g.dtype and residual.dtype == g.dtype and out.dtype == g.dtype
+        assert g.shape == (M, 64) and at.shape == (N, 64) and residual.shape == (M, N)
+        op = self._new(L.OP_LORA_UP, L.PROF_GEMM, 2.0 * M * N * 64, g, at, residual, out)
+        u = op.u.lora_up
+        u.g, u.ld_g, u.at, u.ld_at, u.residual, u.ld_r, u.out, u.ld_o = L.ptr(g), _ld(g), L.ptr(at), _ld(at), L.ptr(residual), _ld(residual), L.ptr(out), _ld(out)
+        u.alpha, u.p, u.offset, u.M, u.N = float(alpha), float(p), int(offset), M, N
         return len(self.ops) - 1
 
     def layernorm_bwd_scaled(self, dy, x, w, stats, dx, t_out, t_scale, accumulate_dx=False):
```

Measured after the change: 138.2 images/s, median of 4. Within noise of the previous version (+0.5%).
